# spthm/grace-devel

Measured on AMD Instinct MI355X. Metric: Mrays/s SPH column-density trace, 10^7 particles, higher is better.
Workload: dtype f32

## Files before the change

### grace-devel_amd/csrc/trace.hip

```cpp
#include "kernel_tables.hpp"
#include "trace_kernel.hpp"
#include "trace_plan.hpp"

#include <cmath>

using namespace grace_hip;

namespace grace_hip {

static_assert(GRACE_SPH_KERNEL_TABLE_ROWS == GRACE_SPH_KERNEL_WENDLAND_C6 + 1, "one table per built-in kernel");
__device__ double g_sph_kernel_tables[GRACE_SPH_KERNEL_TABLE_ROWS][N_TABLE] = GRACE_SPH_KERNEL_TABLES_INIT;
static const double k_sph_kernel_tables[GRACE_SPH_KERNEL_TABLE_ROWS][N_TABLE] = GRACE_SPH_KERNEL_TABLES_INIT;

static grace_status trace_state_destroy(Context& c)
{
    if (!c.trace) return GRACE_OK;
    TraceState& ts = *c.trace;
    GRACE_TRY(plan_release(ts));
    GRACE_TRY(scene_release(ts));
    GRACE_TRY(rays_release(ts));
    if (ts.hits.chunk_counts) GRACE_TRY_HIP(hipFree(ts.hits.chunk_counts));
    if (ts.custom_table) GRACE_TRY_HIP(hipFree(ts.custom_table));
    if (ts.status) GRACE_TRY_HIP(hipFree(ts.status));
    if (ts.ev0) GRACE_TRY_HIP(hipEventDestroy(ts.ev0));
// ... 231 lines not shown

template <int MODE, bool SPLIT, bool ALT = false>
void launch_walk(const int grid, const TraceArgs& args, hipStream_t stream)
{
    trace_kernel<MODE, SPLIT, ALT, false><<<grid, TRACE_BLOCK, 0, stream>>>(args);
    if constexpr (has_lattice(MODE))
        if (args.lat_dev) trace_kernel<MODE, SPLIT, ALT, true><<<grid, TRACE_BLOCK, 0, stream>>>(args);
}

template <int MODE>
grace_status dispatch(const TraceState& ts, const TraceArgs& a, const TraceBuffers& b, const LaunchPlan& p,
                      const int* kept, const size_t n_rays, hipStream_t stream)
{
    const int grid = ceil_div(size_t(p.n_packets) * p.split, TRACE_BLOCK / 64);
    const int* const plan_k_dev = a.plan_usable ? a.plan_split_dev : nullptr;
    auto combine = [&](const int k, const int* k_dev, const int* run_if) -> grace_status {
        const int g = ceil_div(n_rays * channels(MODE), 256);
        if constexpr (double_sums(MODE))
            combine_classes_kernel<double><<<g, 256, 0, stream>>>(a.partial_d, int(n_rays), k, k_dev, a.out_sums_d, run_if);
        else if constexpr (weighted(MODE))
            combine_channel_classes_kernel<<<g, 256, 0, stream>>>(a.partial, int(n_rays), channels(MODE), k, k_dev,
                                                                  a.out_sums, a.out_stride, run_if,
                                                                  a.plan_usable, plan_k_dev);
        else if constexpr (f4_sums(MODE))
            combine_classes_kernel<float><<<g, 256, 0, stream>>>(a.partial, int(n_rays), k, k_dev, a.out_sums, run_if,
                                                                 a.plan_usable, plan_k_dev);
        else return GRACE_OK;
        GRACE_CHECK_LAUNCH();
        return GRACE_OK;
    };
    if constexpr (class_split(MODE)) {
        auto walk = [&](auto alt_tag) -> grace_status {
            constexpr bool ALT = decltype(alt_tag)::value;
            if constexpr (has_lattice(MODE)) if (p.lat_split) {
                if (output(MODE) == OUT_COUNTS)
                    GRACE_TRY_HIP(hipMemsetAsync(a.out_counts, 0, n_rays * sizeof(int), stream));
                trace_kernel<MODE, false, ALT, false><<<grid, TRACE_BLOCK, 0, stream>>>(a);
                GRACE_CHECK_LAUNCH();
                TraceArgs a_lat = a;
                a_lat.split = p.lat_split; a_lat.split_dev = nullptr;
                trace_kernel<MODE, true, ALT, true><<<ceil_div(size_t(p.n_packets) * p.lat_split, TRACE_BLOCK / 64),
                                                      TRACE_BLOCK, 0, stream>>>(a_lat);
                GRACE_CHECK_LAUNCH();
                return combine(p.lat_split, nullptr, a.lat_dev);
            }
            if constexpr (f4_sums(MODE)) if (a.plan_usable) {
                GRACE_TRY(plan_record(ts, a, stream));
                const int grid_planned = a.plan_split_dev
                    ? ceil_div(size_t(p.n_packets) * planned_split(p.n_packets), TRACE_BLOCK / 64) : grid;
                GRACE_TRY(launch_planned(MODE, ALT, grid_planned, a, stream));
                if (p.split == 1) GRACE_TRY(combine(1, nullptr, reinterpret_cast<const int*>(a.plan_usable)));
            }
            if (p.split > 1) launch_walk<MODE, true, ALT>(grid, a, stream);
            else launch_walk<MODE, false, ALT>(grid, a, stream);
            return GRACE_OK;
        };
        if constexpr (f4_sums(MODE)) GRACE_TRY(p.fast_b ? walk(std::true_type()) : walk(std::false_type()));
        else GRACE_TRY(walk(std::false_type()));
    } else if constexpr (MODE == MODE_HITS) {
        if (p.hits_split) {
            const int* counts = kept;
            if (!kept) {
                TraceArgs c = a;
                c.chunk_counts = b.chunk_counts; c.out_counts = b.scratch_counts;
                GRACE_TRY_HIP(hipMemsetAsync(b.chunk_counts, 0, n_rays * size_t(p.hit_chunks) * 4, stream));
                GRACE_TRY_HIP(hipMemsetAsync(b.scratch_counts, 0, n_rays * 4, stream));
                launch_walk<MODE_COUNT, true>(grid, c, stream);
                GRACE_CHECK_LAUNCH();
                counts = b.chunk_counts;
            }
            hits_offsets_kernel<<<ceil_div(n_rays, 4), 256, 0, stream>>>(counts, a.offsets, int(n_rays),
                                                                         p.hit_chunks, b.chunk_off);
            GRACE_CHECK_LAUNCH();
            hits_plan_kernel<<<p.n_packets, MAX_HIT_CHUNKS, 0, stream>>>(counts, a.perm, int(n_rays),
                                                                         p.hit_chunks, b.pk_prefix, b.pk_total);
            GRACE_CHECK_LAUNCH();
            hits_assign_kernel<<<1, 1024, 0, stream>>>(b.pk_total, p.n_packets, p.n_packets * p.split, p.hit_chunks,
                                                       b.pk_first, b.pk_parts, b.n_wave_map,
                                                       ts.hits_stage_split ? 200000ull : 0ull);
            GRACE_CHECK_LAUNCH();
            hits_bounds_kernel<<<p.n_packets, 64, 0, stream>>>(b.pk_prefix, b.pk_total, b.pk_first, b.pk_parts,
                                                               p.hit_chunks, b.wave_map);
            GRACE_CHECK_LAUNCH();
            TraceArgs staged = a, direct = a;
            staged.stage_dev = direct.stage_dev = b.n_wave_map + 4;
            staged.stage_want = 1; direct.stage_want = 0;
            launch_walk<MODE, true, true>(grid, staged, stream);
            GRACE_CHECK_LAUNCH();
            launch_walk<MODE, true, false>(grid, direct, stream);
        } else if (p.n_packets >= 4096) {
            launch_walk<MODE, false, true>(grid, a, stream);
        } else {
            launch_walk<MODE, false, false>(grid, a, stream);
        }
    } else {
        launch_walk<MODE, false>(grid, a, stream);
    }
    GRACE_CHECK_LAUNCH();
    GRACE_TRY(stamps_report(MODE));
    if (p.split > 1) GRACE_TRY(combine(p.split, a.split_dev, nullptr));
    return GRACE_OK;
}

template <int MODE>
grace_status launch_trace(TraceArgs a, size_t n_rays, size_t n_spheres, size_t n_nodes,
                          hipStream_t stream, const Nested nested = Nested())
{
    GRACE_REQUIRE(a.rays && a.spheres && a.nodes && a.leaves && a.root, "trace: null pointer");
    GRACE_REQUIRE(n_rays < (size_t(1) << 31), "trace: bad ray count");
    GRACE_REQUIRE(n_nodes >= 1 && n_nodes < (size_t(1) << 30), "trace: bad node count");
    GRACE_REQUIRE(n_spheres > 0 && n_spheres < (size_t(1) << 31), "trace: bad primitive count");
    TraceState* ts_ptr = nullptr;
    GRACE_TRY(trace_state(&ts_ptr));
    TraceState& ts = *ts_ptr;
    GRACE_TRY(ensure_status(ts, stream));
    a.kernel_table = ts.kernel_table;
    const LaunchPlan p = plan_launch<MODE>(ts, a.keep_chunks, n_rays, n_spheres);
    const bool reuse_chunks = p.hits_split && ts.hits.valid && ts.hits.rays == a.rays
        && ts.hits.n_rays == n_rays && ts.hits.prims == static_cast<const void*>(a.spheres)
        && ts.hits.n_prims == n_spheres && ts.hits.n_chunks == p.hit_chunks;
    if (chunked(MODE)) ts.hits.valid = false;
    const size_t need = n_rays * size_t(p.hit_chunks);
    if (p.keep_chunks && ts.hits.capacity < need) {
        if (ts.hits.chunk_counts) { GRACE_TRY_HIP(hipDeviceSynchronize()); GRACE_TRY_HIP(hipFree(ts.hits.chunk_counts)); }
        ts.hits.chunk_counts = nullptr; ts.hits.capacity = 0;
        hipError_t e = hipMalloc(reinterpret_cast<void**>(&ts.hits.chunk_counts), need * sizeof(int));
        if (e != hipSuccess) return set_error(GRACE_OUT_OF_MEMORY, __FILE__, __LINE__, hipGetErrorString(e));
        ts.hits.capacity = need;
    }
    FrameGuard frame;
    TraceBuffers b;
    GRACE_TRY(use_records<MODE>(ts, a, b, frame, p, n_rays, n_spheres, n_nodes, stream, nested));
    if (nested.measure) return GRACE_OK;
    a.width = p.width; a.split = p.split; a.treelet = p.treelet; a.treelet_axis = p.treelet_axis;
    a.n_rays = int(n_rays); a.n_nodes = int(n_nodes); a.n_prims = int(n_spheres); a.status = ts.status;
    a.group_shift = group_shift(n_spheres); a.chunk_shift = p.hit_chunk_shift; a.n_chunks = p.hit_chunks;
    a.partial = b.partial; a.partial_d = b.partial_d;
    a.chunk_off = b.chunk_off; a.wave_map = b.wave_map; a.n_wave_map = b.n_wave_map;
    if (p.split > 1 && output(MODE) == OUT_COUNTS)
        GRACE_TRY_HIP(hipMemsetAsync(a.out_counts, 0, n_rays * sizeof(int), stream));
    if (p.keep_chunks && p.split > 1) {
        a.chunk_counts = ts.hits.chunk_counts;
        GRACE_TRY_HIP(hipMemsetAsync(ts.hits.chunk_counts, 0, n_rays * size_t(p.hit_chunks) * 4, stream));
        ts.hits.valid = true; ts.hits.rays = a.rays; ts.hits.n_rays = n_rays;
        ts.hits.prims = a.spheres; ts.hits.n_prims = n_spheres; ts.hits.n_chunks = p.hit_chunks;
    }
    ts.last_lat_dev = a.lat_dev; ts.last_lat_stream = stream;
    if constexpr (f4_sums(MODE)) {
        PacketPlan& pp = ts.plan;
        if (b.plan_eligible && !(pp.key == b.plan_key && (pp.valid || pp.dead)))
            GRACE_TRY(plan_fill(ts, b.plan_key, a, stream));
        ts.last_plan_ctl = nullptr;
        if (b.plan_eligible && pp.valid && pp.key == b.plan_key) {
            a.plan_entries = pp.entries; a.plan_spans = pp.spans; a.plan_counts = pp.counts;
            a.plan_usable = &pp.ctl->usable;
            ts.last_plan_ctl = pp.ctl; ts.last_plan_stream = stream;
        }
    }
    return timed(ts, stream, [&] {
        return dispatch<MODE>(ts, a, b, p, reuse_chunks ? ts.hits.chunk_counts : nullptr, n_rays, stream);
    });
}

TraceArgs trace_args(const void* d_rays, const void* d_prims, const int* d_nodes, const int* d_leaves,
                     const int* d_root)
{
    TraceArgs a = {};
    a.rays = static_cast<const float*>(d_rays);
    a.spheres = static_cast<const float4*>(d_prims);
    a.nodes = reinterpret_cast<const float4*>(d_nodes);
    a.leaves = reinterpret_cast<const int4*>(d_leaves);
    a.root = d_root;
    return a;
}

}

namespace grace_hip {
grace_status rays_invalidate_if_written(const void* d_written)
{
    Context* c = nullptr;
    GRACE_TRY(current_context(&c));
    if (!c->trace) return GRACE_OK;
    TraceState& ts = *c->trace;
    if (ts.cache_validation) return GRACE_OK;
    if (ts.rays.valid && d_written && d_written == static_cast<const void*>(ts.rays.key.rays)) return rays_release(ts);
    return GRACE_OK;
}

grace_status scene_invalidate_if_written(const void* d_written)
{
    Context* c = nullptr;
    GRACE_TRY(current_context(&c));
    if (!c->trace) return GRACE_OK;
    TraceState& ts = *c->trace;
    if (ts.cache_validation) return GRACE_OK;
    if (ts.scene.valid && d_written
        && (d_written == ts.scene.key.prims || d_written == ts.scene.key.nodes || d_written == ts.scene.key.leaves))
        return scene_release(ts);
    return GRACE_OK;
}

grace_status trace_nested_bytes(size_t n_rays, size_t n_spheres, size_t n_nodes, size_t* bytes)
{
    TraceArgs a = trace_args(bytes, bytes, reinterpret_cast<const int*>(bytes), reinterpret_cast<const int*>(bytes),
                             reinterpret_cast<const int*>(bytes));
    size_t counts = 0, hits = 0;
    GRACE_TRY(launch_trace<MODE_COUNT>(a, n_rays, n_spheres, n_nodes, nullptr, Nested{true, &counts}));
    GRACE_TRY(launch_trace<MODE_HITS>(a, n_rays, n_spheres, n_nodes, nullptr, Nested{true, &hits}));
    *bytes = counts > hits ? counts : hits;
    return GRACE_OK;
}

grace_status trace_hitcounts_nested(const void* d_rays, size_t n_rays, const float* d_spheres, size_t n_spheres,
                                    const int* d_nodes, size_t n_nodes, const int* d_leaves, const int* d_root,
                                    int* d_hit_counts, hipStream_t stream)
{
    TraceArgs a = trace_args(d_rays, d_spheres, d_nodes, d_leaves, d_root);
    a.out_counts = d_hit_counts;
    return launch_trace<MODE_COUNT>(a, n_rays, n_spheres, n_nodes, stream, Nested{true, nullptr});
}

grace_status trace_hits_nested(const void* d_rays, size_t n_rays, const float* d_spheres, size_t n_spheres,
                               const int* d_nodes, size_t n_nodes, const int* d_leaves, const int* d_root,
                               const int* d_ray_offsets, int* d_hit_indices, float* d_hit_integrals,
                               float* d_hit_distances, hipStream_t stream)
{
    TraceArgs a = trace_args(d_rays, d_spheres, d_nodes, d_leaves, d_root);
    a.offsets = d_ray_offsets;
    a.hit_idx = d_hit_indices;
    a.hit_integral = d_hit_integrals;
    a.hit_dist = d_hit_distances;
    return launch_trace<MODE_HITS>(a, n_rays, n_spheres, n_nodes, stream, Nested{true, nullptr});
}
}

extern "C" {

grace_status grace_trace_hitcounts_f4(const void* d_rays, size_t n_rays, const float* d_spheres,
                                      size_t n_spheres, const int* d_nodes, size_t n_nodes,
                                      const int* d_leaves, const int* d_root,
                                      int* d_hit_counts, grace_stream stream)
{
    if (n_rays == 0) return GRACE_OK;
    GRACE_REQUIRE(d_hit_counts, "trace_hitcounts: null output");
    TraceArgs a = trace_args(d_rays, d_spheres, d_nodes, d_leaves, d_root);
    a.out_counts = d_hit_counts;
    return launch_trace<MODE_COUNT>(a, n_rays, n_spheres, n_nodes, as_stream(stream));
}

grace_status grace_trace_hitcounts_keep_f4(const void* d_rays, size_t n_rays, const float* d_spheres,
                                           size_t n_spheres, const int* d_nodes, size_t n_nodes,
                                           const int* d_leaves, const int* d_root,
                                           int* d_hit_counts, grace_stream stream)
{
    if (n_rays == 0) return GRACE_OK;
    GRACE_REQUIRE(d_hit_counts, "trace_hitcounts: null output");
    TraceArgs a = trace_args(d_rays, d_spheres, d_nodes, d_leaves, d_root);
    a.out_counts = d_hit_counts;
    a.keep_chunks = true;
    return launch_trace<MODE_COUNT>(a, n_rays, n_spheres, n_nodes, as_stream(stream));
}

grace_status grace_trace_cumulative_f4(const void* d_rays, size_t n_rays, const float* d_spheres,
                                       size_t n_spheres, const int* d_nodes, size_t n_nodes,
                                       const int* d_leaves, const int* d_root,
                                       float* d_cumulated, grace_stream stream)
{
    if (n_rays == 0) return GRACE_OK;
    GRACE_REQUIRE(d_cumulated, "trace_cumulative: null output");
    TraceArgs a = trace_args(d_rays, d_spheres, d_nodes, d_leaves, d_root);
    a.out_sums = d_cumulated;
    return launch_trace<MODE_CUMULATIVE>(a, n_rays, n_spheres, n_nodes, as_stream(stream));
}

grace_status grace_trace_cumulative_weighted_f4(const void* d_rays, size_t n_rays, const float* d_spheres,
                                                size_t n_spheres, const int* d_nodes, size_t n_nodes,
                                                const int* d_leaves, const int* d_root,
                                                const float* d_weights, int n_channels, float* d_out,
                                                grace_stream stream)
{
    GRACE_REQUIRE(n_channels >= 1 && n_channels <= 64, "trace_cumulative_weighted: channels must be 1..64");
    if (n_rays == 0) return GRACE_OK;
    GRACE_REQUIRE(d_weights || n_spheres == 0, "trace_cumulative_weighted: null weights");
    GRACE_REQUIRE(d_out, "trace_cumulative_weighted: null output");
    GRACE_REQUIRE(n_rays * size_t(n_channels) < (size_t(1) << 31), "trace_cumulative_weighted: too many outputs");
    for (int g = 0; g < n_channels; g += MAX_LAUNCH_CHANNELS) {
        TraceArgs a = trace_args(d_rays, d_spheres, d_nodes, d_leaves, d_root);
        a.weights = d_weights + g;
        a.w_stride = n_channels;
        a.out_sums = d_out + g;
        a.out_stride = n_channels;
        const hipStream_t s = as_stream(stream);
        switch (n_channels - g < MAX_LAUNCH_CHANNELS ? n_channels - g : MAX_LAUNCH_CHANNELS) {
        case 1: GRACE_TRY(launch_trace<MODE_WCUM1>(a, n_rays, n_spheres, n_nodes, s)); break;
        case 2: GRACE_TRY(launch_trace<MODE_WCUM2>(a, n_rays, n_spheres, n_nodes, s)); break;
        case 3: GRACE_TRY(launch_trace<MODE_WCUM3>(a, n_rays, n_spheres, n_nodes, s)); break;
        default: GRACE_TRY(launch_trace<MODE_WCUM4>(a, n_rays, n_spheres, n_nodes, s)); break;
        }
    }
    return GRACE_OK;
}

grace_status grace_trace_hits_f4(const void* d_rays, size_t n_rays, const float* d_spheres,
                                 size_t n_spheres, const int* d_nodes, size_t n_nodes,
                                 const int* d_leaves, const int* d_root,
                                 const int* d_ray_offsets, int* d_hit_indices,
                                 float* d_hit_integrals, float* d_hit_distances,
                                 grace_stream stream)
// ... 97 lines not shown
                                     int* d_hit_indices, double* d_hit_integrals,
                                     double* d_hit_distances, grace_stream stream)
{
    if (n_rays == 0) return GRACE_OK;
    GRACE_REQUIRE(d_ray_offsets && d_hit_indices && d_hit_integrals && d_hit_distances,
                  "trace_hits (float4, double): null output");
    TraceArgs a = trace_args(d_rays, d_spheres, d_nodes, d_leaves, d_root);
    a.offsets = d_ray_offsets;
    a.hit_idx = d_hit_indices;
    a.hit_integral_d = d_hit_integrals;
    a.hit_dist_d = d_hit_distances;
    return launch_trace<MODE_HITS_F4D>(a, n_rays, n_spheres, n_nodes, as_stream(stream));
}

grace_status grace_trace_stats_f4(const void* d_rays, size_t n_rays, const float* d_spheres,
                                  size_t n_spheres, const int* d_nodes, size_t n_nodes,
                                  const int* d_leaves, const int* d_root,
                                  uint32_t* d_stats4, grace_stream stream)
{
    if (n_rays == 0) return GRACE_OK;
    GRACE_REQUIRE(d_stats4, "trace_stats: null output");
    TraceArgs a = trace_args(d_rays, d_spheres, d_nodes, d_leaves, d_root);
    a.stats = d_stats4;
    return launch_trace<MODE_STATS>(a, n_rays, n_spheres, n_nodes, as_stream(stream));
}

grace_status grace_hit_integrals_f32(const float* d_b2, const float* d_h, size_t n, float* d_out,
                                     grace_stream stream)
{
    GRACE_REQUIRE(n == 0 || (d_b2 && d_h && d_out), "hit_integrals: null pointer");
    if (n == 0) return GRACE_OK;
    TraceState* ts = nullptr;
    GRACE_TRY(trace_state(&ts));
    hit_integrals_kernel<<<stream_grid(n, 256), 256, 0, as_stream(stream)>>>(d_b2, d_h, n, d_out,
                                                                             ts->kernel_table);
    GRACE_CHECK_LAUNCH();
    return GRACE_OK;
}

grace_status grace_sph_kernel_table(int kind, double* h_out51)
{
    GRACE_REQUIRE(kind >= GRACE_SPH_KERNEL_CUBIC && kind <= GRACE_SPH_KERNEL_WENDLAND_C6,
                  "sph_kernel_table: kind must be a built-in GRACE_SPH_KERNEL_* (0..5)");
    GRACE_REQUIRE(h_out51, "sph_kernel_table: null output");
    for (int i = 0; i < N_TABLE; ++i) h_out51[i] = k_sph_kernel_tables[kind][i];
    return GRACE_OK;
}

#define GRACE_TRACE_STATE()                                                                      \
    TraceState* ts_ptr_ = nullptr;                                                               \
    GRACE_TRY(trace_state(&ts_ptr_));                                                            \
    TraceState& ts = *ts_ptr_

grace_status grace_trace_prepare_f4(const float* d_spheres, size_t n_spheres, const int* d_nodes,
                                    size_t n_nodes, const int* d_leaves, grace_stream stream)
{
    GRACE_TRACE_STATE();
    return scene_prepare(ts, PRIM_F4, d_spheres, n_spheres, d_nodes, n_nodes, d_leaves, as_stream(stream));
}

grace_status grace_trace_prepare_tri(const float* d_tris, size_t n_tris, const int* d_nodes,
                                     size_t n_nodes, const int* d_leaves, grace_stream stream)
{
    GRACE_TRACE_STATE();
    return scene_prepare(ts, PRIM_TRI, d_tris, n_tris, d_nodes, n_nodes, d_leaves, as_stream(stream));
}

grace_status grace_trace_prepare_rays(const void* d_rays, size_t n_rays, grace_stream stream)
{
    GRACE_TRACE_STATE();
    return rays_prepare(ts, static_cast<const float*>(d_rays), n_rays, as_stream(stream));
}

grace_status grace_trace_release_rays(void)
{
    GRACE_TRACE_STATE();
    GRACE_TRY(plan_release(ts));
    return rays_release(ts);
}

grace_status grace_trace_release(void)
{
    GRACE_TRACE_STATE();
    if (ts.hits.chunk_counts) {
        GRACE_TRY_HIP(hipDeviceSynchronize());
        GRACE_TRY_HIP(hipFree(ts.hits.chunk_counts));
    }
    ts.hits = HitsCache();
    GRACE_TRY(plan_release(ts));
    return scene_release(ts);
}

grace_status grace_trace_enable_timing(int enabled)
{
    GRACE_TRACE_STATE();
    ts.timing = enabled != 0;
    ts.ev_valid = false;
    return GRACE_OK;
}

grace_status grace_trace_last_kernel_ms(float* h_ms)
{
    GRACE_REQUIRE(h_ms, "null output");
    GRACE_TRACE_STATE();
    GRACE_REQUIRE(ts.timing && ts.ev_valid, "no timed traversal launch recorded");
    GRACE_TRY_HIP(hipEventSynchronize(ts.ev1));
    GRACE_TRY_HIP(hipEventElapsedTime(h_ms, ts.ev0, ts.ev1));
    return GRACE_OK;
}

grace_status grace_trace_last_lattice(int* h_lattice)
{
    GRACE_REQUIRE(h_lattice, "null output");
    *h_lattice = 0;
    GRACE_TRACE_STATE();
    if (ts.last_lat_dev) {
        GRACE_TRY_HIP(hipStreamSynchronize(ts.last_lat_stream));
        GRACE_TRY_HIP(hipMemcpy(h_lattice, ts.last_lat_dev, sizeof(int), hipMemcpyDeviceToHost));
    }
    return GRACE_OK;
}

grace_status grace_trace_last_plan_used(int* h_used)
{
    GRACE_REQUIRE(h_used, "null output");
    *h_used = 0;
    GRACE_TRACE_STATE();
    if (ts.last_plan_ctl) {
        PlanCtl h = {};
        GRACE_TRY_HIP(hipStreamSynchronize(ts.last_plan_stream));
        GRACE_TRY_HIP(hipMemcpy(&h, ts.last_plan_ctl, sizeof(h), hipMemcpyDeviceToHost));
        *h_used = h.usable != 0u ? 1 : 0;
    }
    return GRACE_OK;
}

grace_status grace_trace_plan_stats(unsigned long long* h_stats)
{
    GRACE_REQUIRE(h_stats, "null output");
    for (int k = 0; k < 7; ++k) h_stats[k] = 0;
    GRACE_TRACE_STATE();
    if (ts.last_plan_ctl) {
        PlanCtl h = {};
        GRACE_TRY_HIP(hipStreamSynchronize(ts.last_plan_stream));
        GRACE_TRY_HIP(hipMemcpy(&h, ts.last_plan_ctl, sizeof(h), hipMemcpyDeviceToHost));
        if (h.usable != 0u) {
            for (int k = 0; k < 6; ++k) h_stats[k] = h.stats[k];
            h_stats[6] = h.largest_round;
        }
    }
    return GRACE_OK;
}

grace_status grace_trace_set_plan(int on)
{
    GRACE_TRACE_STATE();
    ts.plan_on = on != 0;
    if (!ts.plan_on) GRACE_TRY(plan_release(ts));
    return GRACE_OK;
}

grace_status grace_trace_set_plan_budget(size_t bytes)
{
    GRACE_TRACE_STATE();
    ts.plan_budget = bytes;
    GRACE_TRY(plan_release(ts));
    return GRACE_OK;
}

grace_status grace_trace_plan_bytes(size_t* h_bytes)
{
    GRACE_REQUIRE(h_bytes, "null output");
    GRACE_TRACE_STATE();
    const PacketPlan& pp = ts.plan;
    *h_bytes = pp.valid ? (pp.n_entries + 4) * sizeof(uint4) + pp.n_lists * (sizeof(int) + sizeof(int2)) + sizeof(PlanCtl) : 0;
    return GRACE_OK;
}

grace_status grace_trace_set_packet_split(int waves_per_packet)
{
    GRACE_REQUIRE(waves_per_packet == -1 || waves_per_packet == 1 || waves_per_packet == 2
                      || waves_per_packet == 4 || waves_per_packet == 8,
                  "packet split must be 1, 2, 4, 8 or -1 (automatic)");
    GRACE_TRACE_STATE();
    ts.split = waves_per_packet;
    return GRACE_OK;
}

grace_status grace_trace_set_packet_width(int rays_per_packet)
{
    GRACE_REQUIRE(rays_per_packet == -1 || rays_per_packet == 16 || rays_per_packet == 32
                      || rays_per_packet == 64,
                  "packet width must be 16, 32, 64 or -1 (automatic)");
    GRACE_TRACE_STATE();
    ts.width = rays_per_packet;
    return GRACE_OK;
}

grace_status grace_trace_set_exact_integrals(int enabled)
{
    GRACE_TRACE_STATE();
    ts.exact_integrals = enabled != 0;
    return GRACE_OK;
}

grace_status grace_trace_set_sph_kernel(int kind)
{
    GRACE_REQUIRE(kind >= GRACE_SPH_KERNEL_CUBIC && kind <= GRACE_SPH_KERNEL_WENDLAND_C6,
                  "set_sph_kernel: kind must be a built-in GRACE_SPH_KERNEL_* (0..5); a custom table is "
                  "set with grace_trace_set_sph_kernel_table");
    GRACE_TRACE_STATE();
    ts.sph_kernel = kind;
    ts.kernel_table = ts.builtin_tables + kind * N_TABLE;
    return GRACE_OK;
}

grace_status grace_trace_set_sph_kernel_table(const double* h_table, int n)
{
    GRACE_REQUIRE(h_table && n == N_TABLE, "set_sph_kernel_table: the table must hold 51 values");
    for (int i = 0; i < N_TABLE; ++i)
        GRACE_REQUIRE(std::isfinite(h_table[i]) && h_table[i] >= 0.0,
                      "set_sph_kernel_table: every value must be finite and >= 0");
    GRACE_REQUIRE(h_table[N_TABLE - 1] == 0.0, "set_sph_kernel_table: the last value (b = H) must be 0");
    GRACE_TRACE_STATE();
    GRACE_TRY_HIP(hipDeviceSynchronize());
    if (!ts.custom_table)
        GRACE_TRY_HIP(hipMalloc(reinterpret_cast<void**>(&ts.custom_table), N_TABLE * sizeof(double)));
    GRACE_TRY_HIP(hipMemcpy(ts.custom_table, h_table, N_TABLE * sizeof(double), hipMemcpyHostToDevice));
    for (int i = 0; i < N_TABLE; ++i) ts.custom_host[i] = h_table[i];
    ts.sph_kernel = GRACE_SPH_KERNEL_CUSTOM;
    ts.kernel_table = ts.custom_table;
    return GRACE_OK;
}

grace_status grace_trace_get_sph_kernel(int* h_kind, double* h_table51)
{
    GRACE_TRACE_STATE();
    if (h_kind) *h_kind = ts.sph_kernel;
    if (h_table51) {
        const double* t = ts.sph_kernel == GRACE_SPH_KERNEL_CUSTOM ? ts.custom_host
                                                                   : k_sph_kernel_tables[ts.sph_kernel];
        for (int i = 0; i < N_TABLE; ++i) h_table51[i] = t[i];
    }
    return GRACE_OK;
}

grace_status grace_trace_set_treelet_size(int max_primitives)
{
    GRACE_REQUIRE(max_primitives >= -1, "treelet size must be >= 0 (or -1 for automatic)");
    GRACE_TRACE_STATE();
    ts.treelet = max_primitives;
    return GRACE_OK;
}

grace_status grace_trace_set_ray_reorder(int enabled)
{
    GRACE_TRACE_STATE();
    ts.ray_reorder = enabled != 0;
    return GRACE_OK;
}

grace_status grace_trace_set_cache_validation(int enabled)
{
    GRACE_TRACE_STATE();
    ts.cache_validation = enabled != 0;
    return GRACE_OK;
}

grace_status grace_trace_set_cache_auto(int enabled)
{
    GRACE_TRACE_STATE();
    ts.cache_auto = enabled != 0;
    if (!ts.cache_auto) {
        if ((ts.scene.valid && !ts.scene.pinned) || (ts.rays.valid && !ts.rays.pinned)) GRACE_TRY(plan_release(ts));
        if (ts.scene.valid && !ts.scene.pinned) GRACE_TRY(scene_release(ts));
        if (ts.rays.valid && !ts.rays.pinned) GRACE_TRY(rays_release(ts));
        ts.scene.seen = SceneKey();
        ts.rays.seen = RayKey();
    }
    return GRACE_OK;
}

grace_status grace_trace_set_lattice_split(int waves_per_packet)
{
    GRACE_REQUIRE(waves_per_packet == 0 || waves_per_packet == 2 || waves_per_packet == 4
                      || waves_per_packet == 8,
                  "lattice split must be 0 (one wave per packet), 2, 4 or 8");
    GRACE_TRACE_STATE();
    ts.lat_split = waves_per_packet;
    return GRACE_OK;
}

grace_status grace_trace_set_hits_staging(int enabled)
{
    GRACE_TRACE_STATE();
    ts.hits_stage_split = enabled != 0;
    return GRACE_OK;
}

grace_status grace_trace_status(grace_stream stream)
{
    GRACE_TRACE_STATE();
    if (!ts.status) return GRACE_OK;
    int h = 0;
    GRACE_TRY_HIP(hipMemcpyAsync(&h, ts.status, sizeof(int), hipMemcpyDeviceToHost,
                                 as_stream(stream)));
    GRACE_TRY_HIP(hipStreamSynchronize(as_stream(stream)));
    if (h != 0) {
        GRACE_TRY_HIP(hipMemsetAsync(ts.status, 0, sizeof(int), as_stream(stream)));
        if (h == GRACE_INVALID_ARGUMENT)
            return set_error(GRACE_INVALID_ARGUMENT, __FILE__, __LINE__,
                             "range_neighbours: a row of d_offsets does not have the length of its list");
        return set_error(GRACE_STACK_OVERFLOW, __FILE__, __LINE__,
                         "trace: packet stack (128 entries) exhausted");
    }
    return GRACE_OK;
}

}
```

### grace-devel_amd/csrc/trace_coherence.hip

```cpp
#include "trace_state.hpp"

using namespace grace_hip;

namespace {

__device__ __forceinline__ uint32_t f2ord_u(float f)
{
    const uint32_t u = __float_as_uint(f);
    return (u & 0x80000000u) ? ~u : (u | 0x80000000u);
}

__device__ __forceinline__ float ord2f_u(uint32_t u)
{
    return __uint_as_float((u & 0x80000000u) ? (u & 0x7fffffffu) : ~u);
}

__global__ void ray_ext_init_kernel(uint32_t* __restrict__ ext16)
{
    if (threadIdx.x < 16) ext16[threadIdx.x] = threadIdx.x < 6 ? 0xFFFFFFFFu : 0u;
}

__global__ __launch_bounds__(1024) void ray_extents_kernel(const float* __restrict__ rays, int n,
                                                          uint32_t* __restrict__ ext12,
                                                          const uint32_t* __restrict__ run_if)
// ... 14 lines not shown
        len_hi = fmaxf(len_hi, r[6]);
    }
#pragma unroll
    for (int off = 32; off > 0; off >>= 1) len_hi = fmaxf(len_hi, __shfl_xor(len_hi, off));
#pragma unroll
    for (int k = 0; k < 6; ++k) {
#pragma unroll
        for (int off = 32; off > 0; off >>= 1) {
            lo[k] = fminf(lo[k], __shfl_xor(lo[k], off));
            hi[k] = fmaxf(hi[k], __shfl_xor(hi[k], off));
        }
    }
    __shared__ float s_lo[16][6], s_hi[16][6], s_len[16];
    const int wave = threadIdx.x >> 6;
    if ((threadIdx.x & 63) == 0) {
#pragma unroll
        for (int k = 0; k < 6; ++k) { s_lo[wave][k] = lo[k]; s_hi[wave][k] = hi[k]; }
        s_len[wave] = len_hi;
    }
    __syncthreads();
    const int n_waves = int(blockDim.x >> 6);
    if (threadIdx.x < 6) {
        const int k = threadIdx.x;
        float l = s_lo[0][k], h = s_hi[0][k];
        for (int w = 1; w < n_waves; ++w) { l = fminf(l, s_lo[w][k]); h = fmaxf(h, s_hi[w][k]); }
        atomicMin(&ext12[k], f2ord_u(l));
        atomicMax(&ext12[6 + k], f2ord_u(h));
    } else if (threadIdx.x == 6) {
        float l = s_len[0];
        for (int w = 1; w < n_waves; ++w) l = fmaxf(l, s_len[w]);
        if (l > -INFINITY) atomicMax(&ext12[15], f2ord_u(l));
    }
}

__device__ int choose_split(const uint32_t* __restrict__ ext12, int n_packets, int launched_arg, bool lattice)
{
    const bool one_direction = ext12[0] == ext12[6] && ext12[1] == ext12[7] && ext12[2] == ext12[8];
    const int launched = launched_arg & 0xFF;
    const int budget = (launched_arg & SPLIT_WIDE_BUDGET) ? 32768 : 16384;
    int k = launched;
    if (one_direction && !lattice) {
        k = 1;
        while (k < launched && n_packets * k < 8192) k *= 2;
        if (k < launched && n_packets >= 6144 && n_packets * k * 2 <= budget) k *= 2;
    } else if (!lattice) {
        k = 1;
        while (k < launched && n_packets * k < 16384) k *= 2;
    }
    return k;
}

__device__ __forceinline__ uint32_t hilbert2d_15(uint32_t x, uint32_t y)
{
    uint32_t d = 0;
    for (uint32_t s = 1u << 14; s > 0; s >>= 1) {
        const uint32_t rx = (x & s) ? 1u : 0u, ry = (y & s) ? 1u : 0u;
        d = (d << 2) | ((3u * rx) ^ ry);
        if (ry == 0) {
            if (rx) { x = 32767u - x; y = 32767u - y; }
            const uint32_t t = x; x = y; y = t;
        }
    }
    return d;
}

__global__ __launch_bounds__(256) void ray_lattice_kernel(const float* __restrict__ rays, int n,
                                                          const uint32_t* __restrict__ ext12,
                                                          uint32_t* __restrict__ flag,
                                                          const uint32_t* __restrict__ run_if)
{
    if (run_if && *run_if == 0u) return;
    int dims[2] = { 0, 0 }, nvar = 0;
    float lo[2] = { 0.f, 0.f }, span[2] = { 0.f, 0.f };
    for (int k = 5; k >= 0; --k) {
        const float l = ord2f_u(ext12[k]), sp = ord2f_u(ext12[6 + k]) - l;
        if (sp > 0.f && sp < INFINITY) {
            if (nvar < 2) { dims[nvar] = k; lo[nvar] = l; span[nvar] = sp; }
            ++nvar;
        }
    }
    bool fit = nvar == 2 && n >= 64 && (n & (n - 1)) == 0;
    float m1 = 0.f, m2 = 0.f;
    if (fit) {
        int log_n = 0;
        while ((1 << log_n) < n) ++log_n;
        fit = false;
        const float ratio = span[0] / span[1];
        for (int a = 3; a <= log_n - 3; ++a) {
            const float c1 = float((1 << a) - 1), c2 = float((1 << (log_n - a)) - 1);
            if (fabsf(c1 / c2 - ratio) <= 1e-3f * ratio) { fit = true; m1 = c1; m2 = c2; break; }
        }
    }
    if (!fit) {
        if (blockIdx.x == 0 && threadIdx.x == 0) atomicOr(flag, 1u);
        return;
    }
    const float s1 = m1 / span[0], s2 = m2 / span[1];
    bool off = false;
    for (int i = blockIdx.x * blockDim.x + threadIdx.x; i < n; i += gridDim.x * blockDim.x) {
        const float* r = rays + 7 * size_t(i);
        const float u1 = (r[dims[0]] - lo[0]) * s1, u2 = (r[dims[1]] - lo[1]) * s2;
        off = off || !(fabsf(u1 - rintf(u1)) <= 0.01f) || !(fabsf(u2 - rintf(u2)) <= 0.01f);
    }
    if (__builtin_amdgcn_ballot_w64(off) != 0ull && (threadIdx.x & 63) == 0) atomicOr(flag, 1u);
}

__device__ void choose_variants(const uint32_t* __restrict__ ext12, int n, const float4* __restrict__ scene_min,
                                uint32_t* __restrict__ lat_flag, int split_packets, int split_launched,
                                int* __restrict__ split_dev)
{
    if (lat_flag) {
        int n_dir = 0;
        bool one_dir = true;
        float e1 = 0.f, e2 = 0.f;
        for (int k = 0; k < 3; ++k) {
            const float dl = ord2f_u(ext12[k]), dh = ord2f_u(ext12[6 + k]);
            one_dir = one_dir && dl == dh;
            n_dir += dl != 0.f ? 1 : 0;
            const float e = ord2f_u(ext12[9 + k]) - ord2f_u(ext12[3 + k]);
            if (e > e1) { e2 = e1; e1 = e; } else if (e > e2) e2 = e;
        }
        const float spacing2 = e1 * e2 / float(n);
        const float r2_min = scene_min->x;
        bool lat = one_dir && n_dir == 1 && spacing2 > 0.f && r2_min < 2.0f * spacing2;
        if (!lat && e1 == 0.f && ext12[15] != 0u) {
            const float len = ord2f_u(ext12[15]);
            if (len > 0.f && len < INFINITY) lat = r2_min < 2.0f * (12.566371f * len * len / float(n));
        }
        *lat_flag = lat ? 1u : 0u;
    }
    if (split_dev)
        *split_dev = choose_split(ext12, split_packets, split_launched, lat_flag ? *lat_flag != 0u : false);
}

__global__ void choose_variants_kernel(const uint32_t* __restrict__ ext12, int n, const float4* __restrict__ scene_min,
                                       uint32_t* __restrict__ lat_flag, int split_packets, int split_launched,
                                       int* __restrict__ split_dev, const PlanGate gate,
                                       int* __restrict__ plan_split_dev)
{
    if (lat_flag || split_dev)
        choose_variants(ext12, n, scene_min, lat_flag, split_packets, split_launched, split_dev);
    if (plan_split_dev) *plan_split_dev = planned_split(split_packets);
    if (gate.ctl) {
        PlanCtl& pc = *gate.ctl;
        const bool stale = pc.sig[0] != gate.scene->sig[0] || pc.sig[1] != gate.scene->sig[1]
            || pc.sig[2] != gate.rays->sig[0] || pc.sig[3] != gate.rays->sig[1];
        pc.record = stale ? 1u : 0u;
        if (stale) {
            pc.unusable = 0u; pc.usable = 1u;
            pc.sig[0] = gate.scene->sig[0]; pc.sig[1] = gate.scene->sig[1];
            pc.sig[2] = gate.rays->sig[0]; pc.sig[3] = gate.rays->sig[1];
            for (int k = 0; k < 6; ++k) pc.stats[k] = 0ull;
            pc.largest_round = 0u;
        }
    }
}

__global__ __launch_bounds__(256) void ray_keys_kernel(const float* __restrict__ rays, int n,
                                                       const uint32_t* __restrict__ ext12,
                                                       uint32_t* __restrict__ keys,
                                                       const float4* __restrict__ scene_min,
                                                       uint32_t* __restrict__ lat_flag,
                                                       int split_packets, int split_launched,
                                                       int* __restrict__ split_dev,
                                                       const uint32_t* __restrict__ not_grid,
                                                       const uint32_t* __restrict__ run_if)
{
    if (run_if && *run_if == 0u) return;
    const bool z_order_2d = not_grid && *not_grid == 0u;
    if (blockIdx.x == 0 && threadIdx.x == 0)
        choose_variants(ext12, n, scene_min, lat_flag, split_packets, split_launched, split_dev);
    float lo[6], scale[6], span[6];
    int nvar = 0;
    float span_d = 0.f, span_o = 0.f;
#pragma unroll
    for (int k = 0; k < 6; ++k) {
        lo[k] = ord2f_u(ext12[k]);
        span[k] = ord2f_u(ext12[6 + k]) - lo[k];
        const bool varies = span[k] > 0.f && span[k] < INFINITY;
        if (varies) { if (k < 3) span_d = fmaxf(span_d, span[k]); else span_o = fmaxf(span_o, span[k]); }
    }
#pragma unroll
    for (int k = 0; k < 6; ++k) {
        const bool varies = span[k] > 0.f && span[k] < INFINITY;
        scale[k] = varies ? 1.0f / (k < 3 ? span_d : span_o) : 0.f;
        nvar += varies ? 1 : 0;
    }
    const int bits = nvar ? min(15, 30 / nvar) : 0;
    const float qmax = float((1 << bits) - 1);
    const bool pencil = scale[3] == 0.f && scale[4] == 0.f && scale[5] == 0.f && nvar > 0;
    for (int i = blockIdx.x * blockDim.x + threadIdx.x; i < n; i += gridDim.x * blockDim.x) {
        const float* r = rays + 7 * size_t(i);
        if (pencil) {
            const float l1 = fabsf(r[0]) + fabsf(r[1]) + fabsf(r[2]);
            float u = r[0] / l1, v = r[1] / l1;
            if (r[2] < 0.f) {
                const float fu = (1.f - fabsf(v)) * (u >= 0.f ? 1.f : -1.f);
                const float fv = (1.f - fabsf(u)) * (v >= 0.f ? 1.f : -1.f);
                u = fu; v = fv;
            }
            const uint32_t qu = uint32_t(fminf(32767.f, fmaxf(0.f, (u * 0.5f + 0.5f) * 32767.f + 0.5f)));
            const uint32_t qv = uint32_t(fminf(32767.f, fmaxf(0.f, (v * 0.5f + 0.5f) * 32767.f + 0.5f)));
            keys[i] = hilbert2d_15(qu, qv);
            continue;
        }
        uint32_t q[6];
#pragma unroll
        for (int k = 0; k < 6; ++k) q[k] = uint32_t(fminf(qmax, (r[k] - lo[k]) * scale[k] * qmax + 0.5f));
#ifndef GRACE_MORTON2D
        if (nvar == 2 && !z_order_2d) {
            uint32_t xy[2] = {0, 0};
            int m = 0;
#pragma unroll
            for (int k = 5; k >= 0; --k)
                if (scale[k] > 0.f) { if (m < 2) xy[m] = q[k]; ++m; }
            keys[i] = hilbert2d_15(xy[1], xy[0]);
            continue;
        }
#endif
        uint32_t key = 0;
        for (int b = bits - 1; b >= 0; --b) {
#pragma unroll
            for (int k = 5; k >= 0; --k)
                if (scale[k] > 0.f) key = (key << 1) | ((q[k] >> b) & 1u);
        }
        keys[i] = key << (30 - bits * nvar);
    }
}

}

namespace grace_hip {

grace_status launch_choose_variants(const uint32_t* ext12, int n, const float4* scene_min, uint32_t* lat_flag,
                                    int split_packets, int split_launched, int* split_dev, hipStream_t stream,
                                    const PlanGate* gate, int* plan_split_dev)
{
    choose_variants_kernel<<<1, 1, 0, stream>>>(ext12, n, scene_min, lat_flag, split_packets, split_launched,
                                                split_dev, gate ? *gate : PlanGate(), plan_split_dev);
    GRACE_CHECK_LAUNCH();
    return GRACE_OK;
}

static grace_status rays_free_buffers(RayOrder& ro)
{
    if (ro.perm || ro.ext || ro.ctl) GRACE_TRY_HIP(hipDeviceSynchronize());
    if (ro.perm) GRACE_TRY_HIP(hipFree(ro.perm));
    if (ro.ext) GRACE_TRY_HIP(hipFree(ro.ext));
    if (ro.ctl) GRACE_TRY_HIP(hipFree(ro.ctl));
    ro.perm = nullptr; ro.ext = nullptr; ro.ctl = nullptr;
    ro.valid = false;
    ro.pinned = false;
    return GRACE_OK;
}

grace_status rays_release(TraceState& ts)
{
    GRACE_TRY(rays_free_buffers(ts.rays));
    ts.rays = RayOrder();
    return GRACE_OK;
}

grace_status rays_cache_alloc(TraceState& ts, const RayKey& key)
{
    RayOrder& ro = ts.rays;
    GRACE_TRY(rays_free_buffers(ro));
    if (hipMalloc(reinterpret_cast<void**>(&ro.perm), key.n * 4) != hipSuccess
        || hipMalloc(reinterpret_cast<void**>(&ro.ext), 64) != hipSuccess
        || hipMalloc(reinterpret_cast<void**>(&ro.ctl), sizeof(CacheCtl)) != hipSuccess) {
        (void)hipGetLastError();
        (void)rays_free_buffers(ro);
        return set_error(GRACE_OUT_OF_MEMORY, __FILE__, __LINE__, "ray order cache: out of device memory");
    }
    ro.key = key;
    ro.gen = ++ts.cache_gen;
    return GRACE_OK;
}

grace_status ray_order(const float* d_rays, size_t n_rays, uint32_t* ext, uint32_t* keys, uint32_t* perm,
                       const float4* scene_min, uint32_t* lat_flag, int n_packets, int split, int* split_dev,
                       hipStream_t stream, const uint32_t* run_if)
{
    if (!run_if) {
        ray_ext_init_kernel<<<1, 64, 0, stream>>>(ext);
        GRACE_CHECK_LAUNCH();
    }
    const int grid_small = stream_grid(n_rays, 256, 4) < 1024 ? stream_grid(n_rays, 256, 4) : 1024;
    const int grid_ext = stream_grid(n_rays, 1024, 4) < 128 ? stream_grid(n_rays, 1024, 4) : 128;
    ray_extents_kernel<<<grid_ext, 1024, 0, stream>>>(d_rays, int(n_rays), ext, run_if);
    GRACE_CHECK_LAUNCH();
    ray_lattice_kernel<<<grid_small, 256, 0, stream>>>(d_rays, int(n_rays), ext, ext + 14, run_if);
    GRACE_CHECK_LAUNCH();
    ray_keys_kernel<<<stream_grid(n_rays, 256), 256, 0, stream>>>(d_rays, int(n_rays), ext, keys, scene_min,
                                                                 lat_flag, n_packets, split, split_dev, ext + 14,
                                                                 run_if);
    GRACE_CHECK_LAUNCH();
    const size_t packets64 = ceil_div(n_rays, size_t(64));
    int want_bits = 2;
    while ((size_t(1) << (want_bits - 2)) < packets64 && want_bits < 30) ++want_bits;
    want_bits = ((want_bits + 7) / 8) * 8;
    const int begin_bit = want_bits >= 30 ? 0 : 30 - want_bits;
    return sort_pairs_u32_nested(keys, nullptr, n_rays, 0, begin_bit, 30, perm, stream, run_if);
}

grace_status rays_prepare(TraceState& ts, const float* d_rays, size_t n_rays, hipStream_t stream)
{
// ... 31 lines not shown
```

### grace-devel_amd/csrc/trace_kernel.hpp

```cpp
#pragma once

#include "trace_diag.hpp"
#include "trace_packet.hpp"
#include "trace_state.hpp"

#include <type_traits>

namespace {

using namespace grace_hip;

__device__ __forceinline__ bool any_lane(bool p) { return __builtin_amdgcn_ballot_w64(p) != 0ull; }

__device__ __forceinline__ int imin(int a, int b) { return a < b ? a : b; }
__device__ __forceinline__ int imax(int a, int b) { return a > b ? a : b; }

__device__ __forceinline__ void aabbs_hit(const float ix, const float iy, const float iz,
                                          const float ox, const float oy, const float oz,
                                          const float len, const float4 L, const float4 R,
                                          const float4 Z, bool& hit_l, bool& hit_r)
{
    const float bx_L = (L.x - ox) * ix, tx_L = (L.y - ox) * ix;
    const float by_L = (L.z - oy) * iy, ty_L = (L.w - oy) * iy;
    const float bz_L = (Z.x - oz) * iz, tz_L = (Z.y - oz) * iz;
// ... 45 lines not shown
    integral *= ir2;
    return integral;
}

__device__ __forceinline__ float hit_integral_fast(const float b2, const float ir50,
                                                   const float2* lutf)
{
    const float b = __builtin_amdgcn_sqrtf(b2) * ir50;
    const float2 y = lutf[static_cast<int>(b)];
    return __builtin_fmaf(y.y, b, y.x);
}

__device__ __forceinline__ bool tri_intersect(const double ddx, const double ddy, const double ddz,
                                              const float ox, const float oy, const float oz,
                                              const double* __restrict__ tri, float* t_out)
{
    const double vx = tri[0], vy = tri[1], vz = tri[2];
    const double e1x = tri[3], e1y = tri[4], e1z = tri[5];
    const double e2x = tri[6], e2y = tri[7], e2z = tri[8];
    const float Px = float(ddy * e2z - ddz * e2y);
    const float Py = float(ddz * e2x - ddx * e2z);
    const float Pz = float(ddx * e2y - ddy * e2x);
    const float det = float((e1x * double(Px) + e1y * double(Py)) + e1z * double(Pz));
    bool reject = det < 1E-14f;
    const float inv_det = 1.0f / det;
    const float OVx = ox - float(vx), OVy = oy - float(vy), OVz = oz - float(vz);
    const double dOVx = OVx, dOVy = OVy, dOVz = OVz;
    const float u = float(((dOVx * double(Px) + dOVy * double(Py)) + dOVz * double(Pz)) * double(inv_det));
    reject = reject || (u < 0.f || u > 1.f);
    const float Qx = float(dOVy * e1z - dOVz * e1y);
    const float Qy = float(dOVz * e1x - dOVx * e1z);
    const float Qz = float(dOVx * e1y - dOVy * e1x);
    const float v = float(((ddx * double(Qx) + ddy * double(Qy)) + ddz * double(Qz)) * double(inv_det));
    reject = reject || (v < 0.f || u + v > 1.f);
    *t_out = float(((e2x * double(Qx) + e2y * double(Qy)) + e2z * double(Qz)) * double(inv_det));
    return !reject;
}

__global__ __launch_bounds__(256) void hit_integrals_kernel(const float* __restrict__ b2,
                                                            const float* __restrict__ h, size_t n,
                                                            float* __restrict__ out,
                                                            const double* __restrict__ table)
{
    __shared__ double2 s_lut[N_TABLE];
    if (threadIdx.x < N_TABLE) {
        const double y0 = table[threadIdx.x];
        const double y1 = threadIdx.x + 1 < N_TABLE ? table[threadIdx.x + 1] : y0;
        s_lut[threadIdx.x] = make_double2(y0, y1 - y0);
    }
    __syncthreads();
    for (size_t i = blockIdx.x * size_t(blockDim.x) + threadIdx.x; i < n;
         i += size_t(gridDim.x) * blockDim.x) {
        const float ir = 1.f / h[i];
        out[i] = hit_integral(b2[i], ir, ir * ir, s_lut);
    }
}

__device__ __forceinline__ bool beam_may_hit(const float4 s, const Beam& bm,
                                             const float margin = 3.814697265625e-06f )
{
    float p2_lo = 0.f, p2_hi = 0.f, t_lo = 0.f, t_hi = 0.f;
    const float c[3] = { s.x, s.y, s.z };
#pragma unroll
    for (int k = 0; k < 3; ++k) {
        const float plo = c[k] - bm.ohi[k], phi = c[k] - bm.olo[k];
        const float a2 = plo * plo, b2 = phi * phi;
        p2_hi += fmaxf(a2, b2);
        p2_lo += (plo <= 0.f && phi >= 0.f) ? 0.f : fminf(a2, b2);
        const float q0 = plo * bm.dlo[k], q1 = plo * bm.dhi[k];
        const float q2 = phi * bm.dlo[k], q3 = phi * bm.dhi[k];
        t_lo += fminf(fminf(q0, q1), fminf(q2, q3));
        t_hi += fmaxf(fmaxf(q0, q1), fmaxf(q2, q3));
    }
    const float t2_hi = fmaxf(t_lo * t_lo, t_hi * t_hi);
    const float b2_lo = p2_lo - t2_hi - margin * p2_hi;
    return !(b2_lo >= s.w);
}

struct Pencil {
    float ox, oy, oz;
    float ax, ay, az;
    float sin_t, cos_t;
    float nx[4], ny[4], nz[4];
};

__device__ __forceinline__ bool pencil_may_hit(const float4 s, const Pencil& pc)
{
    const float vx = s.x - pc.ox, vy = s.y - pc.oy, vz = s.z - pc.oz;
    const float d2 = __builtin_fmaf(vx, vx, __builtin_fmaf(vy, vy, vz * vz));
    const float va = __builtin_fmaf(vx, pc.ax, __builtin_fmaf(vy, pc.ay, vz * pc.az));
    const float inv = __builtin_amdgcn_rsqf(d2);
    const float sin_a = fminf(1.0f, __builtin_amdgcn_sqrtf(s.w) * inv * 1.00001f);
    const float cos_a = __builtin_amdgcn_sqrtf(fmaxf(0.0f, __builtin_fmaf(-sin_a, sin_a, 1.0f)));
    const float cos_limit = __builtin_fmaf(pc.cos_t, cos_a, -pc.sin_t * sin_a) - 1e-5f;
    const float h = __builtin_amdgcn_sqrtf(s.w) * 1.00001f + 1e-6f * __builtin_amdgcn_sqrtf(d2);
    float out = -1.0f;
#pragma unroll
    for (int k = 0; k < 4; ++k)
        out = fmaxf(out, __builtin_fmaf(vx, pc.nx[k], __builtin_fmaf(vy, pc.ny[k], vz * pc.nz[k])) - h);
    return !(d2 > s.w * 1.00001f) || (!(va * inv < cos_limit) && !(out > 0.0f));
}

template <int AX, bool FUSED = false>
__device__ __forceinline__ bool axis_beam_may_hit(const float4 s, const Beam& bm)
{
    constexpr int D1 = AX == 0 ? 1 : 0, D2 = AX == 2 ? 1 : 2;
    const float s1 = AX == 0 ? s.y : s.x;
    const float s2 = AX == 2 ? s.y : s.z;
    const float q1 = s1 - __builtin_amdgcn_fmed3f(s1, bm.olo[D1], bm.ohi[D1]);
    const float q2 = s2 - __builtin_amdgcn_fmed3f(s2, bm.olo[D2], bm.ohi[D2]);
    const float b2_lo = FUSED ? __builtin_fmaf(q1, q1, q2 * q2) : q1 * q1 + q2 * q2;
    return !(b2_lo >= s.w);
}

__device__ __forceinline__ float4 cluster_sphere(const float4 blo, const float4 bhi)
{
    const float cx = 0.5f * (blo.x + bhi.x), cy = 0.5f * (blo.y + bhi.y), cz = 0.5f * (blo.z + bhi.z);
    const float ex = bhi.x - cx, ey = bhi.y - cy, ez = bhi.z - cz;
    const float fx = cx - blo.x, fy = cy - blo.y, fz = cz - blo.z;
    const float rx = fmaxf(ex, fx), ry = fmaxf(ey, fy), rz = fmaxf(ez, fz);
    return make_float4(cx, cy, cz, (rx * rx + ry * ry + rz * rz) * 1.001f);
}

template <int AX>
__device__ __forceinline__ bool cluster_may_hit(const float4 blo, const float4 bhi, const Beam& bm,
                                                const Pencil* pc)
{
    if constexpr (AX >= 0) {
        constexpr int D1 = AX == 0 ? 1 : 0, D2 = AX == 2 ? 1 : 2;
        const float lo1 = AX == 0 ? blo.y : blo.x, hi1 = AX == 0 ? bhi.y : bhi.x;
        const float lo2 = AX == 2 ? blo.y : blo.z, hi2 = AX == 2 ? bhi.y : bhi.z;
        return !(lo1 > bm.ohi[D1]) && !(hi1 < bm.olo[D1]) && !(lo2 > bm.ohi[D2]) && !(hi2 < bm.olo[D2]);
    } else if constexpr (AX == -2) {
        const float lx = blo.x - pc->ox, ly = blo.y - pc->oy, lz = blo.z - pc->oz;
        const float hx = bhi.x - pc->ox, hy = bhi.y - pc->oy, hz = bhi.z - pc->oz;
        const float scale = fmaxf(fmaxf(fmaxf(fabsf(lx), fabsf(hx)), fmaxf(fabsf(ly), fabsf(hy))),
                                  fmaxf(fabsf(lz), fabsf(hz)));
        const float slack = 1e-5f * scale;
        float worst = -1.0f;
#pragma unroll
        for (int k = 0; k < 4; ++k) {
            const float m = fminf(pc->nx[k] * lx, pc->nx[k] * hx) + fminf(pc->ny[k] * ly, pc->ny[k] * hy)
                + fminf(pc->nz[k] * lz, pc->nz[k] * hz);
            worst = fmaxf(worst, m);
        }
        const float front = fmaxf(pc->ax * lx, pc->ax * hx) + fmaxf(pc->ay * ly, pc->ay * hy)
            + fmaxf(pc->az * lz, pc->az * hz);
        return !(worst > slack) && !(front < -slack) && pencil_may_hit(cluster_sphere(blo, bhi), *pc);
    } else {
        return beam_may_hit(cluster_sphere(blo, bhi), bm, 1.52587890625e-05f );
    }
}

typedef uint32_t plan_u32x4 __attribute__((ext_vector_type(4)));
typedef int plan_i32x2 __attribute__((ext_vector_type(2)));
template <typename T>
__device__ __forceinline__ const __attribute__((address_space(4))) T* plan_const(const void* p)
{
    return (const __attribute__((address_space(4))) T*)(uintptr_t)p;
}

template <int N>
struct WeightedB {
    float x, y;
    float w[N + 1];
    __device__ WeightedB(const float2 b) : x(b.x), y(b.y), w{} {}
};

template <int MODE, bool SPLIT, bool ALT = false, bool LAT = false, bool PLANNED = false>
__global__ __launch_bounds__(TRACE_BLOCK, !f4_class_split(MODE) ? 1
                                          : weighted(MODE) ? (channels(MODE) == 1 ? 6 : 7 - channels(MODE))
                                          : (SPLIT ? 8 : 6))
void trace_kernel(const TraceArgs a)
{
    static_assert(!ALT || f4_integrals(MODE), "no alternative path for this mode");
    static_assert(!LAT || has_lattice(MODE), "no lattice cull for this mode");
    static_assert(!PLANNED || (SPLIT && !LAT && f4_sums(MODE)), "planned: class-split column densities only");
    if constexpr (PLANNED) {
        if (*plan_const<uint32_t>(a.plan_usable) == 0u) return;
    } else if (has_lattice(MODE)) {
        if (a.plan_usable && *a.plan_usable != 0u) return;
        if (a.lat_dev ? (*a.lat_dev != 0) != LAT : LAT) return;
        if (a.stage_dev && *a.stage_dev != a.stage_want) return;
    }
    constexpr bool FAST = ALT && f4_sums(MODE);
    constexpr bool WEIGHTED = weighted(MODE);
    constexpr int NW = channels(MODE), WP = WEIGHTED ? (NW + 1) / 2 : 0;
    using BRec = std::conditional_t<WEIGHTED, WeightedB<NW>, float2>;
    __shared__ double2 s_lut[FAST ? 1 : N_TABLE];
    constexpr int LUTF_N = 256;
    __shared__ float2 s_lutf[FAST ? LUTF_N : 1];
    constexpr bool D4 = primitive(MODE) == PRIM_D4, F4D = primitive(MODE) == PRIM_F4D;
    constexpr bool LDS_TILE = primitive(MODE) == PRIM_F4;
    __shared__ __align__(16) float2 s_tile[LDS_TILE ? TRACE_BLOCK / 64 : 1][LDS_TILE ? 3 + WP : 1][LDS_TILE ? 66 : 1];
    __shared__ double s_tile_d[D4 ? TRACE_BLOCK / 64 : 1][D4 ? 64 : 1][D4 ? 6 : 1];
    __shared__ float4 s_tile_f[F4D ? TRACE_BLOCK / 64 : 1][F4D ? 64 : 1][F4D ? 2 : 1];
    const int lane = threadIdx.x & 63;
    static_assert(!SPLIT || class_split(MODE) || MODE == MODE_HITS, "triangle and stats walks do not split");
    constexpr bool RANGE_SPLIT = SPLIT && MODE == MODE_HITS;
    const int split_ordinary = !SPLIT ? 1 : (!RANGE_SPLIT && a.split_dev) ? *a.split_dev : a.split;
    int split_planned = 0;
    if constexpr (PLANNED)
        if (a.plan_split_dev) split_planned = *plan_const<int>(a.plan_split_dev);
    const int split = PLANNED && split_planned > 0 ? split_planned : split_ordinary;
    const int n_packets = (a.n_rays + a.width - 1) / a.width;
    const int nb = (n_packets * split + TRACE_BLOCK / 64 - 1) / (TRACE_BLOCK / 64);
    const int q = nb >> 3, r8 = nb & 7, xcd = blockIdx.x & 7, slot = blockIdx.x >> 3;
    if (slot >= q + (xcd < r8 ? 1 : 0)) return;
    const int vblock = (xcd < r8 ? xcd * (q + 1) : r8 * (q + 1) + (xcd - r8) * q) + slot;
    const int wave_id = __builtin_amdgcn_readfirstlane(vblock * (TRACE_BLOCK / 64)
                                                       + (threadIdx.x >> 6));
    if (integrates(MODE)) {
        if (FAST) {
            static_assert(TRACE_BLOCK >= 256, "one table entry per thread");
            float2 e = make_float2(0.f, 0.f);
            if (threadIdx.x < N_TABLE - 1) {
                const double y0 = a.kernel_table[threadIdx.x], dy = a.kernel_table[threadIdx.x + 1] - y0;
                e = make_float2(float(y0 - double(threadIdx.x) * dy), float(dy));
            }
            if (threadIdx.x < LUTF_N) s_lutf[threadIdx.x] = e;
        } else if (threadIdx.x < N_TABLE) {
            const int i0 = threadIdx.x;
            const double y0 = a.kernel_table[i0];
            const double y1 = i0 + 1 < N_TABLE ? a.kernel_table[i0 + 1] : y0;
            s_lut[threadIdx.x] = make_double2(y0, y1 - y0);
        }
        __syncthreads();
    }
    int packet = wave_id / split, part = wave_id - packet * split;
    int prim_lo = 0, prim_hi = 0x7fffffff;
    if (RANGE_SPLIT) {
        if (wave_id >= *a.n_wave_map) return;
        const int4 wm = a.wave_map[wave_id];
        packet = wm.x; part = 0;
        prim_lo = wm.y << a.chunk_shift;
        prim_hi = wm.z << a.chunk_shift;
        if (prim_lo >= prim_hi) return;
    }
    const int first_ray = packet * a.width;
    if (first_ray >= a.n_rays) return;
    const int classes_per_part = SUM_CLASSES / split;
    const int own_lo = part * classes_per_part, own_hi = own_lo + classes_per_part;
    auto owns_granule = [&](const int g) {
        if (RANGE_SPLIT) { const int p = g << GRANULE_SHIFT; return p >= prim_lo && p < prim_hi; }
        const int c = g & (SUM_CLASSES - 1);
        return c >= own_lo && c < own_hi;
    };
    auto foreign_range = [&](const int first, const int count) {
        if (RANGE_SPLIT) return first + count <= prim_lo || first >= prim_hi;
        const int g0 = first >> GRANULE_SHIFT, g1 = (first + count - 1) >> GRANULE_SHIFT;
        return g1 - g0 <= 1 && !owns_granule(g0) && !owns_granule(g1);
    };
    const PacketRay ray = load_packet_ray(a, first_ray, lane);
    const bool valid = ray.valid;
    const int ray_index = ray.index;
    const float dx = ray.dx, dy = ray.dy, dz = ray.dz;
    const float ox = ray.ox, oy = ray.oy, oz = ray.oz;
    const float len = ray.len;
    const float ix = 1.f / dx, iy = 1.f / dy, iz = 1.f / dz;
    const Beam beam = packet_beam(ray);
    int axis = -1;
    if (!ordered(MODE)) axis = packet_axis(dx, dy, dz);
    __shared__ Pencil s_pencil[TRACE_BLOCK / 64];
    Pencil pencil;
    bool is_pencil = false;
    if (!PLANNED && axis < 0 && MODE != MODE_STATS && beam.olo[0] == beam.ohi[0] && beam.olo[1] == beam.ohi[1]
        && beam.olo[2] == beam.ohi[2]) {
        float sx = dx, sy = dy, sz = dz;
#pragma unroll
        for (int off = 32; off > 0; off >>= 1) {
            sx += __shfl_xor(sx, off); sy += __shfl_xor(sy, off); sz += __shfl_xor(sz, off);
        }
        const float inv = 1.0f / sqrtf(sx * sx + sy * sy + sz * sz);
        const float ax = sx * inv, ay = sy * inv, az = sz * inv;
        const float cx = ay * dz - az * dy, cy = az * dx - ax * dz, cz = ax * dy - ay * dx;
        const float sin_t = wave_max(sqrtf(cx * cx + cy * cy + cz * cz)) + 2e-6f;
        const float cos_min = wave_min(ax * dx + ay * dy + az * dz);
        if (cos_min > 0.5f && sin_t < 0.8660254f) {
            is_pencil = true;
            pencil.ox = beam.olo[0]; pencil.oy = beam.olo[1]; pencil.oz = beam.olo[2];
            pencil.ax = ax; pencil.ay = ay; pencil.az = az;
            pencil.sin_t = sin_t;
            pencil.cos_t = sqrtf(1.0f - sin_t * sin_t);
            float ux, uy, uz;
            if (fabsf(ax) <= fabsf(ay) && fabsf(ax) <= fabsf(az)) { ux = 0.f; uy = -az; uz = ay; }
            else if (fabsf(ay) <= fabsf(az)) { ux = az; uy = 0.f; uz = -ax; }
            else { ux = -ay; uy = ax; uz = 0.f; }
            const float un = 1.0f / sqrtf(ux * ux + uy * uy + uz * uz);
            ux *= un; uy *= un; uz *= un;
            const float vx = ay * uz - az * uy, vy = az * ux - ax * uz, vz = ax * uy - ay * ux;
            const float da_ = ax * dx + ay * dy + az * dz;
            const float tu = (ux * dx + uy * dy + uz * dz) / da_, tv = (vx * dx + vy * dy + vz * dz) / da_;
            const float m = 4e-6f;
            const float tu_lo = wave_min(tu) - m, tu_hi = wave_max(tu) + m;
            const float tv_lo = wave_min(tv) - m, tv_hi = wave_max(tv) + m;
            auto plane = [&](int k, float cu, float cv, float ca) {
                float px = cu * ux + cv * vx + ca * ax, py = cu * uy + cv * vy + ca * ay,
                      pz = cu * uz + cv * vz + ca * az;
                const float pn = 1.0f / sqrtf(px * px + py * py + pz * pz);
                pencil.nx[k] = px * pn; pencil.ny[k] = py * pn; pencil.nz[k] = pz * pn;
            };
            plane(0, 1.f, 0.f, -tu_hi);
            plane(1, -1.f, 0.f, tu_lo);
            plane(2, 0.f, 1.f, -tv_hi);
            plane(3, 0.f, -1.f, tv_lo);
            if (lane == 0) s_pencil[threadIdx.x >> 6] = pencil;
        }
    }
    const AxisRay ar = axis_ray(axis, ray);
    const float oa = ar.oa, da = ar.da, noda = ar.noda, o1 = ar.o1, o2 = ar.o2;
    float noda_lo = 0.f, noda_hi = 0.f, len_lo = 0.f, da0 = 0.f;
    bool same_sense = false;
    if (axis >= 0) axis_extremes(ar, len, noda_lo, noda_hi, len_lo, da0, same_sense);
    const float fat_r2 = FAST && axis >= 0 ? fat_radius2(axis, beam) : INFINITY;
    const int treelet = axis >= 0 ? a.treelet_axis : a.treelet;
    constexpr bool LATTICE = LAT;
    __shared__ float s_lat[LATTICE ? TRACE_BLOCK / 64 : 1][2][8];
    __shared__ float s_lat_r2[LATTICE ? TRACE_BLOCK / 64 : 1];
    if (LATTICE && lane == 0) s_lat_r2[threadIdx.x >> 6] = 0.f;
    if (LATTICE && axis >= 0) {
        bool ok;
        float cell2;
        build_origin_lattice(o1, o2, lane, s_lat, ok, cell2);
        if (lane == 0) s_lat_r2[threadIdx.x >> 6] = ok ? cell2 : 0.f;
    }

    int count = 0;
    constexpr bool CHUNKED = SPLIT && chunked(MODE);
    int cur_chunk = -1;
    int count_at_chunk = 0;
    float sum = 0.f;
    float wsum[NW] = {};
    constexpr bool CLASSES_F = f4_sums(MODE), CLASSES_D = double_sums(MODE);
    constexpr bool CLASSES = output(MODE) == OUT_SUMS || WEIGHTED;
    __shared__ float s_class[CLASSES_F ? TRACE_BLOCK / 64 : 1][CLASSES_F ? SUM_CLASSES * NW : 1][CLASSES_F ? 64 : 1];
    __shared__ double s_class_d[CLASSES_D ? TRACE_BLOCK / 64 : 1][CLASSES_D ? SUM_CLASSES : 1][CLASSES_D ? 64 : 1];
    const int wv_acc = threadIdx.x >> 6;
    if (CLASSES_F) {
#pragma unroll
        for (int c = 0; c < SUM_CLASSES * NW; ++c) s_class[wv_acc][c][lane] = 0.f;
    }
    if (CLASSES_D) {
#pragma unroll
        for (int c = 0; c < SUM_CLASSES; ++c) s_class_d[wv_acc][c][lane] = 0.0;
    }
    double sum_d = 0.0;
    int cur_granule = -1;
// ... 12 lines not shown
        cur_granule = prim >> GRANULE_SHIFT;
        cur_granule_end = (cur_granule + 1) << GRANULE_SHIFT;
        cur_owned = !SPLIT || owns_granule(cur_granule);
        if constexpr (WEIGHTED) {
#pragma unroll
            for (int c = 0; c < NW; ++c) wsum[c] = s_class[wv_acc][(cur_granule & (SUM_CLASSES - 1)) * NW + c][lane];
        } else {
        if (CLASSES_D) sum_d = s_class_d[wv_acc][cur_granule & (SUM_CLASSES - 1)][lane];
        else sum = s_class[wv_acc][cur_granule & (SUM_CLASSES - 1)][lane];
        }
    };
    int write_at = 0;
    auto leave_chunk = [&]() {
        if (MODE == MODE_COUNT && cur_chunk >= 0 && valid && count != count_at_chunk)
            atomicAdd(&a.chunk_counts[size_t(ray_index) * a.n_chunks + cur_chunk],
                      count - count_at_chunk);
        count_at_chunk = count;
    };
    int tri_data = -1;
    float tri_tmin = len * (1.f + 0.000001f);
    const double ddx = dx, ddy = dy, ddz = dz;
    if (output(MODE) == OUT_HITS) write_at = a.offsets[ray_index];
    const double rdx = dx, rdy = dy, rdz = dz;
    constexpr int HIT_CAP = 8;
    constexpr bool STAGE_HITS = ALT && MODE == MODE_HITS;
    __shared__ float s_hits[STAGE_HITS ? TRACE_BLOCK / 64 : 1][STAGE_HITS ? 3 : 1]
                           [STAGE_HITS ? HIT_CAP : 1][STAGE_HITS ? 65 : 1];
    int staged = 0;
    auto drain_hits = [&]() {
        const int wvh = threadIdx.x >> 6;
        constexpr int RAYS_PER_PASS = 64 / HIT_CAP;
        const int g = lane / HIT_CAP, e = lane % HIT_CAP;
#pragma unroll 1
        for (int pass = 0; pass < HIT_CAP; ++pass) {
            const int src = pass * RAYS_PER_PASS + g;
            const int n_src = __shfl(staged, src);
            const int first = __shfl(write_at - staged, src);
            if (e < n_src) {
                a.hit_idx[first + e] = __float_as_int(s_hits[wvh][0][e][src]);
                a.hit_integral[first + e] = s_hits[wvh][STAGE_HITS ? 1 : 0][e][src];
                a.hit_dist[first + e] = s_hits[wvh][STAGE_HITS ? 2 : 0][e][src];
            }
        }
        staged = 0;
    };
    auto enter_chunk = [&](const int chunk) {
        leave_chunk();
        cur_chunk = chunk;
        if (MODE == MODE_HITS) {
            if (STAGE_HITS && __builtin_amdgcn_ballot_w64(staged != 0) != 0ull) drain_hits();
            write_at = a.chunk_off[size_t(ray_index) * a.n_chunks + chunk];
        }
    };
    uint32_t st_nodes = 0, st_leaves = 0, st_tested = 0;

    int stk0 = 0, stk1 = 0;
    int ml0 = 0, mh0 = 0, ml1 = 0, mh1 = 0;
    int sp = -1;
    int junk = 0;
    bool overflow = false;

    auto push = [&](const int value, const unsigned long long alive) {
        if (sp >= 127) { overflow = true; return; }
        ++sp;
        if (sp < 64) {
            const bool me = lane == sp;
            stk0 = me ? value : stk0;
            if (MODE == MODE_STATS) {
                ml0 = me ? int(uint32_t(alive)) : ml0;
                mh0 = me ? int(uint32_t(alive >> 32)) : mh0;
            }
        } else {
            const bool me = lane == sp - 64;
            stk1 = me ? value : stk1;
            if (MODE == MODE_STATS) {
                ml1 = me ? int(uint32_t(alive)) : ml1;
                mh1 = me ? int(uint32_t(alive >> 32)) : mh1;
            }
        }
    };

    constexpr bool FLAT_OK = class_split(MODE);
    bool flat = FLAT_OK && !PLANNED && (axis >= 0 || is_pencil);
    int groups_kept = 0;
    const float4* const group_boxes = a.C + 2 * ((size_t(a.n_prims) + 63) >> 6) + 1;
    const int covered = FLAT_OK ? min(__float_as_int(group_boxes[-1].y), a.n_prims) : 0;
    if (covered < 0) flat = false;
    const int n_groups = FLAT_OK ? int((size_t(max(covered, 0)) + (size_t(1) << a.group_shift) - 1) >> a.group_shift) : 0;
    unsigned long long group_mask = 0ull;
    int group_next = 0;
    __shared__ unsigned long long s_group_mask[FLAT_OK && !PLANNED ? TRACE_BLOCK / 64 : 1][FLAT_OK && !PLANNED ? 64 : 1];
    if (flat && axis < 0) {
        const int wvg = threadIdx.x >> 6;
        for (int g0 = 0; g0 < n_groups; g0 += 128) {
            float4 lo[2], hi[2];
#pragma unroll
            for (int k = 0; k < 2; ++k) {
                const int gj = min(g0 + 64 * k + lane, n_groups - 1);
                lo[k] = group_boxes[2 * size_t(gj)];
                hi[k] = group_boxes[2 * size_t(gj) + 1];
            }
#pragma unroll
            for (int k = 0; k < 2; ++k) {
                const int gk = g0 + 64 * k;
                if (gk < n_groups) {
                    const bool may = cluster_may_hit<-2>(lo[k], hi[k], beam, &s_pencil[wvg]);
                    const int n_g = n_groups - gk;
                    const unsigned long long m = __builtin_amdgcn_ballot_w64(may)
                        & (n_g >= 64 ? ~0ull : ((1ull << n_g) - 1ull));
                    if (lane == 0) s_group_mask[wvg][gk >> 6] = m;
                    groups_kept += __builtin_popcountll(m);
                }
            }
        }
    } else if (flat) {
        const int d1 = axis == 0 ? 1 : 0, d2 = axis == 2 ? 1 : 2;
        const float flat_lo1 = d1 == 0 ? beam.olo[0] : beam.olo[1], flat_hi1 = d1 == 0 ? beam.ohi[0] : beam.ohi[1];
        const float flat_lo2 = d2 == 1 ? beam.olo[1] : beam.olo[2], flat_hi2 = d2 == 1 ? beam.ohi[1] : beam.ohi[2];
        const float oa = axis == 0 ? ox : axis == 1 ? oy : oz;
        const float da = axis == 0 ? dx : axis == 1 ? dy : dz;
        const float ea = oa + da * len;
        const float flat_alo = wave_min(fminf(oa, ea));
        const float flat_ahi = wave_max(fmaxf(oa, ea));
        const int wvg = threadIdx.x >> 6;
        auto group_test = [&](const float4 glo, const float4 ghi, const int g0) {
            const float l1 = axis == 0 ? glo.y : glo.x, h1 = axis == 0 ? ghi.y : ghi.x;
            const float l2 = axis == 2 ? glo.y : glo.z, h2 = axis == 2 ? ghi.y : ghi.z;
            const float la = axis == 0 ? glo.x : axis == 1 ? glo.y : glo.z;
            const float ha = axis == 0 ? ghi.x : axis == 1 ? ghi.y : ghi.z;
            const bool may = !(l1 > flat_hi1) && !(h1 < flat_lo1) && !(l2 > flat_hi2) && !(h2 < flat_lo2)
                && !(la > flat_ahi) && !(ha < flat_alo);
            const int n_g = n_groups - g0;
            const unsigned long long m = __builtin_amdgcn_ballot_w64(may)
                & (n_g >= 64 ? ~0ull : n_g <= 0 ? 0ull : ((1ull << n_g) - 1ull));
            if (lane == 0) s_group_mask[wvg][g0 >> 6] = m;
            groups_kept += __builtin_popcountll(m);
        };
        for (int g0 = 0; g0 < n_groups; g0 += 256) {
            float4 lo[4], hi[4];
#pragma unroll
            for (int k = 0; k < 4; ++k) {
                const int gj = min(g0 + 64 * k + lane, n_groups - 1);
                lo[k] = group_boxes[2 * size_t(gj)];
                hi[k] = group_boxes[2 * size_t(gj) + 1];
            }
#pragma unroll
            for (int k = 0; k < 4; ++k)
                if (g0 + 64 * k < n_groups) group_test(lo[k], hi[k], g0 + 64 * k);
        }
    }
    constexpr int FLAT_MAX_GROUPS = 256;
    if (flat && groups_kept > FLAT_MAX_GROUPS) flat = false;
    if (!flat && !PLANNED) push(*a.root, ~0ull);
    const __attribute__((address_space(4))) plan_u32x4* plan_at = nullptr;
    int plan_n = 0, plan_cls = own_lo;
    (void)plan_at; (void)plan_n; (void)plan_cls;
    unsigned long long st_walk = 0, st_cluster = 0, st_cull = 0, st_surv = 0, st_rounds = 0, st_nsurv = 0;
    const unsigned long long st_begin = STAMP_NOW();
    (void)st_walk; (void)st_cluster; (void)st_cull; (void)st_surv; (void)st_rounds; (void)st_nsurv; (void)st_begin;

    for (;;) {
        const unsigned long long st_t0 = STAMP_NOW(); (void)st_t0;
        int sweep_first = 0, sweep_count = 0;
        bool sweep = false;
        if constexpr (PLANNED) {
            if (plan_cls >= own_hi) break;
            const int list = packet * SUM_CLASSES + plan_cls++;
            plan_n = plan_const<int>(a.plan_counts)[list];
            if (plan_n <= 0) continue;
            plan_at = plan_const<plan_u32x4>(a.plan_entries) + plan_const<plan_i32x2>(a.plan_spans)[list].x;
            enter_granule((plan_cls - 1) << GRANULE_SHIFT);
            sweep = true; sweep_count = a.n_prims;
        } else if (flat) {
            while (group_mask == 0ull && group_next < n_groups) {
                group_mask = s_group_mask[threadIdx.x >> 6][group_next >> 6];
                group_mask = (unsigned long long)uint32_t(__builtin_amdgcn_readfirstlane(int(uint32_t(group_mask))))
                    | ((unsigned long long)uint32_t(__builtin_amdgcn_readfirstlane(int(uint32_t(group_mask >> 32)))) << 32);
                group_next += 64;
            }
            if (group_mask == 0ull) break;
            const int g = group_next - 64 + __builtin_ctzll(group_mask);
            group_mask &= group_mask - 1ull;
            sweep_first = g << a.group_shift;
            sweep_count = min(1 << a.group_shift, covered - sweep_first);
            if (SPLIT) {
                bool mine = false;
                for (int gr = sweep_first >> GRANULE_SHIFT; gr <= (sweep_first + sweep_count - 1) >> GRANULE_SHIFT
                         && gr < (sweep_first >> GRANULE_SHIFT) + SUM_CLASSES; ++gr)
                    mine = mine || owns_granule(gr);
                if (!mine) continue;
            }
            sweep = true;
        } else {
        if (sp < 0) break;
        int idx;
        unsigned long long alive_mask = ~0ull;
        if (sp < 64) {
            idx = __builtin_amdgcn_readlane(stk0, sp);
            if (MODE == MODE_STATS)
                alive_mask = (unsigned long long)uint32_t(__builtin_amdgcn_readlane(ml0, sp))
                    | ((unsigned long long)uint32_t(__builtin_amdgcn_readlane(mh0, sp)) << 32);
        } else {
            idx = __builtin_amdgcn_readlane(stk1, sp - 64);
            if (MODE == MODE_STATS)
                alive_mask = (unsigned long long)uint32_t(__builtin_amdgcn_readlane(ml1, sp - 64))
                    | ((unsigned long long)uint32_t(__builtin_amdgcn_readlane(mh1, sp - 64)) << 32);
        }
        --sp;
        const bool alive = (alive_mask >> lane) & 1ull;

        if (idx < a.n_nodes) {
            const float4* np = a.nodes + 4 * size_t(idx);
            const float4 n0 = np[0];
            const float4 L = np[1];
            const float4 R = np[2];
            const float4 Z = np[3];
            int2 span = make_int2(0, 0x7fffffff);
#ifdef GRACE_PACKET_STATS
            if (treelet > 0) span = a.node_prims[idx];
#else
            if (MODE != MODE_STATS && (treelet > 0 || SPLIT)) span = a.node_prims[idx];
#endif
            if (SPLIT && foreign_range(span.x, span.y)) continue;
            if (span.y <= treelet) {
                sweep = true; sweep_first = span.x; sweep_count = span.y;
            } else {
            bool hit_l, hit_r;
            if constexpr (fp64(MODE) || MODE == MODE_TRI) {
                auto widen = [](const float4 b) {
                    const float s0 = (fabsf(b.x) + fabsf(b.y)) * 4.76837158203125e-07f;
                    const float s1 = (fabsf(b.z) + fabsf(b.w)) * 4.76837158203125e-07f;
                    return make_float4(b.x - s0, b.y + s0, b.z - s1, b.w + s1);
                };
                aabbs_hit(ix, iy, iz, ox, oy, oz, len, widen(L), widen(R), widen(Z), hit_l, hit_r);
            } else {
                aabbs_hit(ix, iy, iz, ox, oy, oz, len, L, R, Z, hit_l, hit_r);
            }
            const unsigned long long vote_r = __builtin_amdgcn_ballot_w64(hit_r);
            const unsigned long long vote_l = __builtin_amdgcn_ballot_w64(hit_l);
#ifdef GRACE_PACKET_STATS
#else
            if (MODE == MODE_STATS && alive) ++st_nodes;
#endif
            if (vote_r) push(__float_as_int(n0.y),
                             MODE == MODE_STATS ? __builtin_amdgcn_ballot_w64(hit_r && alive) : 0ull);
            if (vote_l) push(__float_as_int(n0.x),
                             MODE == MODE_STATS ? __builtin_amdgcn_ballot_w64(hit_l && alive) : 0ull);
            }
        } else {
            const int4 lf = a.leaves[idx - a.n_nodes];
            if (SPLIT && foreign_range(lf.x, lf.y)) continue;
            sweep = true; sweep_first = lf.x; sweep_count = lf.y;
#ifndef GRACE_PACKET_STATS
            if (MODE == MODE_STATS && alive) { ++st_leaves; st_tested += uint32_t(lf.y); }
#endif
        }
        }
        STAMP_ADD(st_walk, st_t0);
        if (sweep) {
            const int2 leaf = make_int2(sweep_first, sweep_count);
            int warm = 0;
            if (sp >= 0) {
                const int nxt = sp < 64 ? __builtin_amdgcn_readlane(stk0, sp)
                                        : __builtin_amdgcn_readlane(stk1, sp - 64);
                warm = nxt < a.n_nodes
                    ? reinterpret_cast<const int*>(a.nodes)[16 * size_t(nxt)]
                    : reinterpret_cast<const int*>(a.leaves)[4 * size_t(nxt - a.n_nodes)];
            }
            auto sweep_range = [&](auto ax_tag) {
                constexpr int AX = decltype(ax_tag)::value;
            constexpr bool NEED_B = f4_integrals(MODE);
            constexpr bool LEAN4 = FAST && AX >= 0;
            const int wv = threadIdx.x >> 6;
            float4* const tile4 = reinterpret_cast<float4*>(&s_tile[wv][0][0]);
            const int r_lo = leaf.x, r_hi = leaf.x + leaf.y;
            const int c_first = r_lo >> 6, c_last = (r_hi - 1) >> 6;
            double4 mined_next = make_double4(0., 0., 0., 0.);
            float mw_next[NW] = {};
            auto load_cluster = [&](const int c, float4& m4, float2& m2) {
                const int pj = PLANNED ? int(min(uint32_t(c << 6) + uint32_t(lane), uint32_t(r_hi - 1)))
                                       : min(max((c << 6) + lane, r_lo), r_hi - 1);
                m4 = a.A[pj];
                if (LDS_TILE && NEED_B) m2 = a.B[pj];
                if (D4) mined_next = reinterpret_cast<const double4*>(a.spheres_d)[pj];
                if (F4D) {
                    const float4 f = a.spheres[pj];
                    mined_next = make_double4(f.x, f.y, f.z, f.w);
                }
                if constexpr (WEIGHTED) {
#pragma unroll
                    for (int c = 0; c < NW; ++c) mw_next[c] = a.weights[size_t(pj) * a.w_stride + c];
                }
            };
            for (int cg = c_first; cg <= (PLANNED ? c_first : c_last); cg += 64) {
                const unsigned long long st_t1 = STAMP_NOW(); (void)st_t1;
                unsigned long long cmask = 1ull;
                unsigned long long small_mask = ~0ull;
                if (!PLANNED && c_last != c_first) {
                    const int cj = min(cg + lane, c_last);
                    const float4 blo = a.C[2 * size_t(cj)], bhi = a.C[2 * size_t(cj) + 1];
                    const bool c_may = cluster_may_hit<AX>(blo, bhi, beam, &s_pencil[wv]);
                    if (LATTICE && AX >= 0) small_mask = __builtin_amdgcn_ballot_w64(blo.w < s_lat_r2[wv]);
                    const int n_c = min(64, c_last - cg + 1);
                    cmask = __builtin_amdgcn_ballot_w64(c_may)
                        & (n_c >= 64 ? ~0ull : ((1ull << n_c) - 1ull));
                    if (SPLIT) cmask &= __builtin_amdgcn_ballot_w64(owns_granule(cj >> (GRANULE_SHIFT - 6)));
#ifdef GRACE_PACKET_STATS
                    if (MODE == MODE_STATS) st_leaves += 1;
#endif
                }
                STAMP_ADD(st_cluster, st_t1);
                if (cmask == 0ull) continue;
                int cnext = cg + __builtin_ctzll(cmask);
                cmask &= cmask - 1ull;
                plan_u32x4 e0 = { 0u, 0u, 0u, 0u }, e1 = e0, e2 = e0, e3 = e0;
                int plan_i = 0;
                (void)plan_i;
                if constexpr (PLANNED) { e0 = plan_at[0]; e1 = plan_at[1]; e2 = plan_at[2]; e3 = plan_at[3]; }
                float4 mine_next;
                float2 mineb_next = make_float2(0.f, 0.f);
                int round_n_next = 0;
                uint32_t round_bits_next = 0u;
                (void)round_n_next; (void)round_bits_next;
                auto gather_round = [&]() {
                    if constexpr (PLANNED) {
                        float* const idx = &s_tile[wv][0][0].x;
                        int p = 0;
                        round_bits_next = e0.w;
                        auto take = [&](const plan_u32x4 ent) {
                            const uint32_t m_lo = uint32_t(__builtin_amdgcn_readfirstlane(int(ent.y)));
                            const uint32_t m_hi = uint32_t(__builtin_amdgcn_readfirstlane(int(ent.z)));
                            const unsigned long long m = (unsigned long long)m_lo | ((unsigned long long)m_hi << 32);
                            const int n_e = __builtin_popcountll(m);
                            if (p + n_e > 64) return false;
                            if (__builtin_amdgcn_inverse_ballot_w64(m))
                                idx[p + int(__builtin_amdgcn_mbcnt_hi(m_hi, __builtin_amdgcn_mbcnt_lo(m_lo, 0u)))] =
                                    __uint_as_float((uint32_t(__builtin_amdgcn_readfirstlane(int(ent.x))) << 6) + uint32_t(lane));
                            p += n_e;
                            ++plan_i;
                            return (uint32_t(__builtin_amdgcn_readfirstlane(int(ent.w))) & 4u) == 0u && plan_i < plan_n;
                        };
                        while (take(e0) && take(e1) && take(e2) && take(e3)) {
                            e0 = plan_at[plan_i]; e1 = plan_at[plan_i + 1]; e2 = plan_at[plan_i + 2]; e3 = plan_at[plan_i + 3];
                        }
                        e0 = plan_at[plan_i]; e1 = plan_at[plan_i + 1]; e2 = plan_at[plan_i + 2]; e3 = plan_at[plan_i + 3];
                        round_n_next = p;
                        const int pj = int(min(__float_as_uint(idx[lane]), uint32_t(r_hi - 1)));
                        mine_next = a.A[pj];
                        if (NEED_B) mineb_next = a.B[pj];
                        if constexpr (WEIGHTED) {
#pragma unroll
                            for (int c = 0; c < NW; ++c) mw_next[c] = a.weights[size_t(pj) * a.w_stride + c];
                        }
                    }
                };
                if constexpr (PLANNED) gather_round();
                else load_cluster(cnext, mine_next, mineb_next);
                for (;;) {
                    const unsigned long long st_t2 = STAMP_NOW(); (void)st_t2;
                    const int pbase = cnext << 6;
                    const float4 mine = mine_next;
                    const float2 mineb = mineb_next;
                    const double4 mined = mined_next;
                    float mw[NW];
                    if constexpr (WEIGHTED) {
#pragma unroll
                        for (int c = 0; c < NW; ++c) mw[c] = mw_next[c];
                    }
                    bool more = cmask != 0ull;
                    const int round_n = round_n_next;
                    const uint32_t round_bits = round_bits_next;
                    (void)round_n; (void)round_bits;
                    if constexpr (PLANNED) {
                        more = plan_i < plan_n;
                        if (more) gather_round();
                    } else if (more) {
                        cnext = cg + __builtin_ctzll(cmask);
                        cmask &= cmask - 1ull;
                        load_cluster(cnext, mine_next, mineb_next);
                    }
                    const int lo_bit = max(r_lo - pbase, 0), hi_bit = min(r_hi - pbase, 64);
                    const unsigned long long m_mask =
                        (hi_bit >= 64 ? ~0ull : ((1ull << hi_bit) - 1ull)) & (~0ull << lo_bit);
                bool may_hit = false;
                if constexpr (PLANNED) { }
                else if constexpr (AX >= 0) may_hit = axis_beam_may_hit<AX, FAST>(mine, beam);
                else if constexpr (AX == -2) may_hit = pencil_may_hit(mine, s_pencil[wv]);
                else may_hit = beam_may_hit(mine, beam);
                unsigned long long rest = PLANNED
                    ? (round_n >= 64 ? ~0ull : ((1ull << round_n) - 1ull))
                    : (__builtin_amdgcn_ballot_w64(may_hit) & m_mask);
                bool keep = __builtin_amdgcn_inverse_ballot_w64(rest);
                bool lean_round = PLANNED && (__builtin_amdgcn_readfirstlane(int(round_bits)) & 1) != 0;
                if constexpr (!PLANNED && AX >= 0 && f4_class_split(MODE)) {
                    const float sa = AX == 0 ? mine.x : AX == 1 ? mine.y : mine.z;
                    const unsigned long long inside =
                        __builtin_amdgcn_ballot_w64(__builtin_fmaf(sa, da0, noda_lo) >= 0.0f)
                        & __builtin_amdgcn_ballot_w64(__builtin_fmaf(sa, da0, noda_hi) < len_lo);
                    lean_round = same_sense & ((rest & ~inside) == 0ull);
                }
                bool fat_round = PLANNED && (__builtin_amdgcn_readfirstlane(int(round_bits)) & 2) != 0;
                if constexpr (LEAN4 && !PLANNED)
                    fat_round = (rest & ~__builtin_amdgcn_ballot_w64(mine.w >= fat_r2)) == 0ull;
                if constexpr (LATTICE && AX >= 0) {
                    if (((small_mask >> ((pbase >> 6) - cg)) & 1ull) && rest != 0ull
                        && __builtin_amdgcn_ballot_w64(keep && mine.w < s_lat_r2[wv]) != 0ull) {
                        const float s1 = AX == 0 ? mine.y : mine.x;
                        const float s2 = AX == 2 ? mine.y : mine.z;
                        float q1 = INFINITY, q2 = INFINITY;
#pragma unroll 1
                        for (int k = 0; k < 8; ++k) {
                            q1 = fminf(q1, fabsf(s1 - s_lat[wv][0][k]));
                            q2 = fminf(q2, fabsf(s2 - s_lat[wv][1][k]));
                        }
                        const float nan_if_nan = (s1 + s2) * 0.0f;
                        const float b2_lo = (FAST ? __builtin_fmaf(q1, q1, q2 * q2) : q1 * q1 + q2 * q2) + nan_if_nan;
                        keep = keep && !(b2_lo >= mine.w);
                        rest = __builtin_amdgcn_ballot_w64(keep);
                    }
                }
#ifdef GRACE_PACKET_STATS
                if (MODE == MODE_STATS) { st_tested += __builtin_popcountll(rest); }
#endif
                constexpr bool COMPACT = f4_class_split(MODE);
                bool skip_round = rest == 0ull;
                if (!PLANNED && !skip_round && (CLASSES || SPLIT)) {
                    const int pf = pbase + __builtin_ctzll(rest);
                    if (CLASSES && pf >= cur_granule_end) enter_granule(pf);
                    if (SPLIT && !(CLASSES ? cur_owned : owns_granule(pf >> GRANULE_SHIFT)))
                        skip_round = true;
                    else if (CHUNKED && (MODE == MODE_HITS || a.chunk_counts) && (pf >> a.chunk_shift) != cur_chunk)
                        enter_chunk(pf >> a.chunk_shift);
                }
                if (!skip_round) {
                if (LDS_TILE) {
                    const int slot = PLANNED ? lane : COMPACT
                        ? int(__builtin_amdgcn_mbcnt_hi(uint32_t(rest >> 32),
                                                        __builtin_amdgcn_mbcnt_lo(uint32_t(rest), 0u)))
                        : lane;
                    float sw[NW + 3] = {};
                    if constexpr (WEIGHTED) {
#pragma unroll
                        for (int c = 0; c < NW; ++c) sw[c] = FAST ? mw[c] * mineb.y : mw[c];
                    }
                    if (LEAN4 && lean_round) {
                        const float s1 = AX == 0 ? mine.y : mine.x;
                        const float s2 = AX == 2 ? mine.y : mine.z;
                        if constexpr (WEIGHTED) {
                            if (keep) tile4[slot] = make_float4(s1, s2, mineb.x, sw[0]);
                            if (NW > 1 && keep) tile4[66 + slot] = make_float4(sw[1], sw[2], sw[3], 0.f);
                        } else {
                        if (keep) tile4[slot] = make_float4(s1, s2, mineb.x, mineb.y);
                        }
                    } else if (!COMPACT || keep) {
                        s_tile[wv][0][slot] = make_float2(mine.x, mine.y);
                        s_tile[wv][LDS_TILE ? 1 : 0][slot] = make_float2(mine.z, mine.w);
                        if (NEED_B) s_tile[wv][LDS_TILE ? 2 : 0][slot] = mineb;
                        if constexpr (WEIGHTED) {
#pragma unroll
                            for (int p = 0; p < WP; ++p) s_tile[wv][3 + p][slot] = make_float2(sw[2 * p], sw[2 * p + 1]);
                        }
                    }
                }
                if (D4) {
                    double* t = s_tile_d[wv][lane];
                    const double ir = 1.f / mined.w;
                    t[0] = mined.x; t[1] = mined.y; t[2] = mined.z;
                    t[3] = mined.w * mined.w;
                    t[4] = ir; t[5] = ir * ir;
                }
                if (F4D) {
                    const float4 f = make_float4(float(mined.x), float(mined.y), float(mined.z), float(mined.w));
                    const float ir = 1.f / f.w;
                    s_tile_f[wv][lane][0] = make_float4(f.x, f.y, f.z, f.w * f.w);
                    s_tile_f[wv][lane][F4D ? 1 : 0] = make_float4(ir, ir * ir, 0.f, 0.f);
                }
                const unsigned long long todo = rest;
                STAMP_ADD(st_cull, st_t2);
                const unsigned long long st_t3 = STAMP_NOW(); (void)st_t3;
#ifdef GRACE_STAMPS
                st_rounds += 1; st_nsurv += __builtin_popcountll(todo);
#endif
                auto process = [&](auto lean_tag, const float4 s, const BRec sb, const int jj) {
                    constexpr bool LEAN = decltype(lean_tag)::value;
                    if constexpr (D4) {
                        const double* sp = s_tile_d[wv][jj - pbase];
                        const double sx = sp[0], sy = sp[1], sz = sp[2], sw2 = sp[3];
                        double dot_p, b2;
                        if (AX >= 0) {
                            const double sa = AX == 0 ? sx : AX == 1 ? sy : sz;
                            const double s1 = AX == 0 ? sy : sx;
                            const double s2 = AX == 2 ? sy : sz;
                            const double q1 = s1 - double(o1), q2 = s2 - double(o2);
                            dot_p = (sa - double(oa)) * double(da);
                            b2 = q1 * q1 + q2 * q2;
                        } else {
                            const double px = sx - ox, py = sy - oy, pz = sz - oz;
                            dot_p = px * rdx + py * rdy + pz * rdz;
                            const double bx = px - dot_p * rdx, by = py - dot_p * rdy, bz = pz - dot_p * rdz;
                            b2 = bx * bx + by * by + bz * bz;
                        }
                        const bool hit = !(b2 >= sw2) && !(dot_p < 0.0f) && !(dot_p >= len);
                        if (output(MODE) == OUT_COUNTS) {
                            count += hit ? 1 : 0;
                        } else if (hit) {
                            const double ir = sp[4];
                            double x = (N_TABLE - 1) * (sqrt(b2) * ir);
                            int x_idx = static_cast<int>(x);
                            if (x_idx >= N_TABLE - 1) { x = double(N_TABLE - 1); x_idx = N_TABLE - 2; }
                            const double2 y = s_lut[x_idx];
                            double integral = __builtin_fma(x - x_idx, y.y, y.x);
                            integral *= sp[5];
                            if (output(MODE) == OUT_SUMS) {
                                sum_d += integral;
                            } else if (valid) {
                                a.hit_idx[write_at] = jj;
                                a.hit_integral_d[write_at] = integral;
                                a.hit_dist_d[write_at] = dot_p;
                                ++write_at;
                            }
                        }
                    } else if constexpr (F4D) {
                        const float4 r0 = s_tile_f[wv][jj - pbase][0], r1 = s_tile_f[wv][jj - pbase][F4D ? 1 : 0];
                        double dot_p, b2;
                        if (AX >= 0) {
                            const float sa = AX == 0 ? r0.x : AX == 1 ? r0.y : r0.z;
                            const float s1 = AX == 0 ? r0.y : r0.x;
                            const float s2 = AX == 2 ? r0.y : r0.z;
                            const double q1 = s1 - o1, q2 = s2 - o2;
                            dot_p = double(sa - oa) * double(da);
                            b2 = q1 * q1 + q2 * q2;
                        } else {
                            const double px = r0.x - ox, py = r0.y - oy, pz = r0.z - oz;
                            dot_p = px * rdx + py * rdy + pz * rdz;
                            const double bx = px - dot_p * rdx, by = py - dot_p * rdy, bz = pz - dot_p * rdz;
                            b2 = bx * bx + by * by + bz * bz;
                        }
                        const bool hit = !(b2 >= double(r0.w)) && !(dot_p < 0.0f) && !(dot_p >= len);
                        if (output(MODE) == OUT_COUNTS) {
                            count += hit ? 1 : 0;
                        } else if (hit && output(MODE) == OUT_SUMS) {
                            const float b = float((N_TABLE - 1) * (sqrt(b2) * double(r1.x)));
                            int x_idx = static_cast<int>(b);
                            float t = b - static_cast<float>(x_idx);
                            if (x_idx >= N_TABLE - 1) { t = 1.0f; x_idx = N_TABLE - 2; }
                            const double2 y = s_lut[x_idx];
                            float integral = static_cast<float>(__builtin_fma(double(t), y.y, y.x));
                            integral *= r1.y;
                            sum_d += integral;
                        } else if (hit && valid) {
                            const double ir = r1.x;
                            double x = (N_TABLE - 1) * (sqrt(b2) * ir);
                            int x_idx = static_cast<int>(x);
                            if (x_idx >= N_TABLE - 1) { x = double(N_TABLE - 1); x_idx = N_TABLE - 2; }
                            const double2 y = s_lut[x_idx];
                            double integral = __builtin_fma(x - x_idx, y.y, y.x);
                            integral *= ir * ir;
                            a.hit_idx[write_at] = jj;
                            a.hit_integral_d[write_at] = integral;
                            a.hit_dist_d[write_at] = dot_p;
                            ++write_at;
                        }
                    } else if (MODE == MODE_TRI) {
                        float t;
                        if (tri_intersect(ddx, ddy, ddz, ox, oy, oz, a.T64 + 9 * size_t(jj), &t)) {
                            if (t <= tri_tmin && t >= 1E-14f) {
                                tri_tmin = t;
                                tri_data = jj;
                            }
                        }
                    } else {
                        float b2, dot_p;
                        if (AX >= 0) {
                            const float sa = AX == 0 ? s.x : AX == 1 ? s.y : s.z;
                            const float s1 = AX == 0 ? s.y : s.x;
                            const float s2 = AX == 2 ? s.y : s.z;
                            const float q1 = s1 - o1, q2 = s2 - o2;
                            dot_p = LEAN ? 0.0f : __builtin_fmaf(sa, da, noda);
                            b2 = FAST ? __builtin_fmaf(q1, q1, q2 * q2) : q1 * q1 + q2 * q2;
                        } else {
                            const float px = s.x - ox, py = s.y - oy, pz = s.z - oz;
                            dot_p = px * dx + py * dy + pz * dz;
                            const float bx = px - dot_p * dx;
                            const float by = py - dot_p * dy;
                            const float bz = pz - dot_p * dz;
                            b2 = FAST ? __builtin_fmaf(bx, bx, __builtin_fmaf(by, by, bz * bz))
                                      : bx * bx + by * by + bz * bz;
                        }
                        if constexpr (FAST && LEAN) {
                            const float b = fminf(__builtin_amdgcn_sqrtf(b2) * sb.x, float(N_TABLE - 1));
                            const float2 y = s_lutf[static_cast<int>(b)];
                            if constexpr (WEIGHTED) {
                                const float t = __builtin_fmaf(y.y, b, y.x);
#pragma unroll
                                for (int c = 0; c < NW; ++c) wsum[c] = __builtin_fmaf(t, sb.w[c], wsum[c]);
                            } else {
                                sum = __builtin_fmaf(__builtin_fmaf(y.y, b, y.x), sb.y, sum);
                            }
                            return;
                        }
                        const bool hit = LEAN ? !(b2 >= s.w)
                                              : !(b2 >= s.w) && !(dot_p < 0.0f) && !(dot_p >= len);
#ifdef GRACE_PACKET_STATS
                        if (MODE == MODE_STATS && __builtin_amdgcn_ballot_w64(hit) != 0ull) ++st_nodes;
#endif
                        if (!integrates(MODE)) {
                            count += hit ? 1 : 0;
                        } else if (hit) {
                            const float w = FAST ? hit_integral_fast(b2, sb.x, s_lutf)
                                                 : hit_integral(b2, sb.x, sb.y, s_lut);
                            if constexpr (WEIGHTED) {
#pragma unroll
                                for (int c = 0; c < NW; ++c)
                                    wsum[c] = FAST ? __builtin_fmaf(w, sb.w[c], wsum[c]) : wsum[c] + sb.w[c] * w;
                            } else {
                            if (FAST) {
                                sum = __builtin_fmaf(w, sb.y, sum);
                            } else if (MODE == MODE_CUMULATIVE) {
                                sum += w;
                            } else if (valid && !STAGE_HITS) {
                                a.hit_idx[write_at] = jj;
                                a.hit_integral[write_at] = w;
                                a.hit_dist[write_at] = dot_p;
                                ++write_at;
                            } else if (valid) {
                                const int wvh = threadIdx.x >> 6;
                                s_hits[wvh][0][staged][lane] = __int_as_float(jj);
                                s_hits[wvh][STAGE_HITS ? 1 : 0][staged][lane] = w;
                                s_hits[wvh][STAGE_HITS ? 2 : 0][staged][lane] = dot_p;
                                ++staged;
                                ++write_at;
                            }
                            }
                        }
                        if (STAGE_HITS && __builtin_amdgcn_ballot_w64(staged == HIT_CAP) != 0ull)
                            drain_hits();
                    }
                };
                auto fetch = [&](unsigned long long& td, int& k, float4& c, BRec& cb, int& jj) {
                    int at;
                    if (COMPACT) {
                        at = k++;
                        jj = 0;
                    } else {
                        at = __builtin_ctzll(td);
                        td = (td & ~(1ull << at)) | 0x8000000000000000ull;
                        jj = min(pbase + at, r_hi - 1);
                    }
                    if (LDS_TILE) {
                        const float2 xy = s_tile[wv][0][at];
                        const float2 zw = s_tile[wv][LDS_TILE ? 1 : 0][at];
                        c = make_float4(xy.x, xy.y, zw.x, zw.y);
                        if constexpr (WEIGHTED) {
                            const float2 b = s_tile[wv][2][at];
                            cb.x = b.x; cb.y = b.y;
#pragma unroll
                            for (int p = 0; p < WP; ++p) {
                                const float2 wp = s_tile[wv][3 + p][at];
                                cb.w[2 * p] = wp.x;
                                cb.w[2 * p + 1] = wp.y;
                            }
                        } else {
                        if (NEED_B) cb = s_tile[wv][LDS_TILE ? 2 : 0][at];
                        }
                        __builtin_amdgcn_sched_barrier(0);
                    } else if (!fp64(MODE)) {
                        c = a.A[jj];
                    }
                };
                auto run = [&](auto lean_tag) {
                    float4 c0, c1, c2;
                    BRec b0 = make_float2(0.f, 0.f), b1 = b0, b2 = b0;
                    int j0, j1 = 0, j2 = 0;
                    int left = __builtin_popcountll(todo);
                    unsigned long long td = todo | 0x8000000000000000ull;
                    int k = 0;
                    fetch(td, k, c0, b0, j0);
                    fetch(td, k, c1, b1, j1);
                    for (;;) {
                        fetch(td, k, c2, b2, j2);
                        process(lean_tag, c0, b0, j0);
                        if (--left == 0) break;
                        fetch(td, k, c0, b0, j0);
                        process(lean_tag, c1, b1, j1);
                        if (--left == 0) break;
                        fetch(td, k, c1, b1, j1);
                        process(lean_tag, c2, b2, j2);
                        if (--left == 0) break;
                    }
                };
                auto run_lean4 = [&](auto fat_tag) {
                    constexpr bool FAT = decltype(fat_tag)::value;
                    float4 c0, c1, c2;
                    int left = __builtin_popcountll(todo);
                    const float4* t4 = tile4;
                    if constexpr (WEIGHTED && NW > 1) {
                        float4 x0, x1;
                        auto procw = [&](const float4 c, const float4 x) {
                            const float q1 = c.x - o1, q2 = c.y - o2;
                            float b = __builtin_amdgcn_sqrtf(__builtin_fmaf(q1, q1, q2 * q2)) * c.z;
                            if (!FAT) b = fminf(b, float(N_TABLE - 1));
                            const float2 y = s_lutf[static_cast<int>(b)];
                            const float t = __builtin_fmaf(y.y, b, y.x);
                            const float xw[4] = { c.w, x.x, x.y, x.z };
#pragma unroll
                            for (int ch = 0; ch < NW; ++ch) wsum[ch] = __builtin_fmaf(t, xw[ch], wsum[ch]);
                        };
                        c0 = t4[0]; x0 = t4[66]; __builtin_amdgcn_sched_barrier(0);
                        for (;;) {
                            c1 = t4[1]; x1 = t4[67]; __builtin_amdgcn_sched_barrier(0);
                            procw(c0, x0);
                            if (--left == 0) break;
                            c0 = t4[2]; x0 = t4[68]; __builtin_amdgcn_sched_barrier(0);
                            procw(c1, x1);
                            if (--left == 0) break;
                            t4 += 2;
                        }
                        return;
                    }
                    auto proc = [&](const float4 c) {
                        const float q1 = c.x - o1, q2 = c.y - o2;
                        float b = __builtin_amdgcn_sqrtf(__builtin_fmaf(q1, q1, q2 * q2)) * c.z;
                        if (!FAT) b = fminf(b, float(N_TABLE - 1));
                        const float2 y = s_lutf[static_cast<int>(b)];
                        if constexpr (WEIGHTED) wsum[0] = __builtin_fmaf(__builtin_fmaf(y.y, b, y.x), c.w, wsum[0]);
                        else sum = __builtin_fmaf(__builtin_fmaf(y.y, b, y.x), c.w, sum);
                    };
                    c0 = t4[0]; __builtin_amdgcn_sched_barrier(0);
                    c1 = t4[1]; __builtin_amdgcn_sched_barrier(0);
                    for (;;) {
                        c2 = t4[2]; __builtin_amdgcn_sched_barrier(0);
                        proc(c0);
                        if (--left == 0) break;
                        c0 = t4[3]; __builtin_amdgcn_sched_barrier(0);
                        proc(c1);
                        if (--left == 0) break;
                        c1 = t4[4]; __builtin_amdgcn_sched_barrier(0);
                        proc(c2);
                        if (--left == 0) break;
                        t4 += 3;
                    }
                };
                if constexpr (LEAN4) {
                    if (lean_round) {
                        if (fat_round) run_lean4(std::true_type());
                        else run_lean4(std::false_type());
                    } else run(std::false_type());
                } else {
                    if (lean_round) run(std::true_type());
                    else run(std::false_type());
                }
                STAMP_ADD(st_surv, st_t3);
                }
                    if (!more) break;
                }
            }
            };
            switch (axis) {
            case 0: sweep_range(std::integral_constant<int, 0>()); break;
            case 1: sweep_range(std::integral_constant<int, 1>()); break;
            case 2: sweep_range(std::integral_constant<int, 2>()); break;
            default:
                if constexpr (!PLANNED) {
                    if (is_pencil) sweep_range(std::integral_constant<int, -2>());
                    else sweep_range(std::integral_constant<int, -1>());
                }
                break;
            }
            junk |= warm;
        }
    }

#ifdef GRACE_STAMPS
    if (lane == 0) {
        atomicAdd(&g_stamp_acc[0], __builtin_amdgcn_s_memtime() - st_begin);
        atomicAdd(&g_stamp_acc[1], st_walk); atomicAdd(&g_stamp_acc[2], st_cluster);
        atomicAdd(&g_stamp_acc[3], st_cull); atomicAdd(&g_stamp_acc[4], st_surv);
        atomicAdd(&g_stamp_acc[5], st_rounds); atomicAdd(&g_stamp_acc[6], st_nsurv);
        atomicAdd(&g_stamp_acc[7], 1ull);
        {
            const unsigned slot = atomicAdd(&g_stamp_n, 1u) & 0xffffu;
            g_stamp_log[slot][0] = st_begin; g_stamp_log[slot][1] = __builtin_amdgcn_s_memtime();
            g_stamp_log[slot][2] = st_nsurv; g_stamp_log[slot][3] = st_walk;
        }
    }
#endif
    if (STAGE_HITS) drain_hits();
    if (CHUNKED && MODE == MODE_COUNT && a.chunk_counts) leave_chunk();
    if ((overflow || junk < 0) && lane == 0) *a.status = GRACE_STACK_OVERFLOW;
    if (!valid) return;
    if (output(MODE) == OUT_COUNTS) {
        if (!SPLIT) a.out_counts[ray_index] = count;
        else if (count) atomicAdd(&a.out_counts[ray_index], count);
    }
    if (MODE == MODE_TRI) a.out_counts[ray_index] = tri_data;
    if (double_sums(MODE)) {
        if (cur_granule >= 0) s_class_d[wv_acc][cur_granule & (SUM_CLASSES - 1)][lane] = sum_d;
        const int c_lo = SPLIT ? own_lo : 0, c_n = SPLIT ? classes_per_part : SUM_CLASSES;
        for (int w = 1; w < c_n; w *= 2)
            for (int c = c_lo; c < c_lo + c_n; c += 2 * w) {
                const double x = s_class_d[wv_acc][c][lane], y = s_class_d[wv_acc][c + w][lane];
                s_class_d[wv_acc][c][lane] = x + y;
            }
        if (!SPLIT) a.out_sums_d[ray_index] = s_class_d[wv_acc][0][lane];
        else a.partial_d[size_t(ray_index) * split + part] = s_class_d[wv_acc][c_lo][lane];
    }
    if (MODE == MODE_CUMULATIVE) {
        if (cur_granule >= 0) s_class[wv_acc][cur_granule & (SUM_CLASSES - 1)][lane] = sum;
        float t[SUM_CLASSES];
#pragma unroll
        for (int c = 0; c < SUM_CLASSES; ++c) t[c] = s_class[wv_acc][c][lane];
        float result = 0.f;
        if (!SPLIT) {
#pragma unroll
            for (int w = 1; w < SUM_CLASSES; w *= 2)
#pragma unroll
                for (int c = 0; c < SUM_CLASSES; c += 2 * w) t[c] = t[c] + t[c + w];
            result = t[0];
            a.out_sums[ray_index] = result;
        } else {
            for (int w = 1; w < classes_per_part; w *= 2)
                for (int c = own_lo; c < own_hi; c += 2 * w) {
                    const float x = s_class[wv_acc][c][lane], y = s_class[wv_acc][c + w][lane];
                    s_class[wv_acc][c][lane] = x + y;
                }
            a.partial[size_t(ray_index) * split + part] = s_class[wv_acc][own_lo][lane];
        }
    }
    if constexpr (WEIGHTED) {
        if (cur_granule >= 0) {
#pragma unroll
            for (int c = 0; c < NW; ++c) s_class[wv_acc][(cur_granule & (SUM_CLASSES - 1)) * NW + c][lane] = wsum[c];
        }
#pragma unroll
        for (int ch = 0; ch < NW; ++ch) {
            if (!SPLIT) {
                float t[SUM_CLASSES];
#pragma unroll
                for (int c = 0; c < SUM_CLASSES; ++c) t[c] = s_class[wv_acc][c * NW + ch][lane];
#pragma unroll
                for (int w = 1; w < SUM_CLASSES; w *= 2)
#pragma unroll
                    for (int c = 0; c < SUM_CLASSES; c += 2 * w) t[c] = t[c] + t[c + w];
                a.out_sums[size_t(ray_index) * a.out_stride + ch] = t[0];
            } else {
                for (int w = 1; w < classes_per_part; w *= 2)
                    for (int c = own_lo; c < own_hi; c += 2 * w) {
// ... 15 lines not shown
```

### grace-devel_amd/csrc/trace_planned.hip

```cpp
#include "trace_kernel.hpp"

#include <vector>

using namespace grace_hip;

namespace {

struct PlanRef {
    uint4* entries;
    const int2* spans;
    int* counts;
    PlanCtl* ctl;
    int force;
};

template <bool FUSED>
__global__ __launch_bounds__(TRACE_BLOCK) void plan_record_kernel(const TraceArgs a, const PlanRef pl)
{
    __shared__ float s_lat[TRACE_BLOCK / 64][2][8];
    if (pl.spans && !pl.force && pl.ctl->record == 0u) return;
    const int lane = threadIdx.x & 63, wv = threadIdx.x >> 6;
    const int n_packets = (a.n_rays + a.width - 1) / a.width;
    const int packet = blockIdx.x * (TRACE_BLOCK / 64) + wv;
    if (packet >= n_packets) return;
    const PacketRay ray = load_packet_ray(a, packet * a.width, lane);
    const int axis = packet_axis(ray.dx, ray.dy, ray.dz);
    const float4* const group_boxes = a.C + 2 * ((size_t(a.n_prims) + 63) >> 6) + 1;
    const int covered = min(__float_as_int(group_boxes[-1].y), a.n_prims);
    int cnt = 0;
    int round_n = 0, round_bits = 0;
    int t_surv = 0, t_rounds = 0, t_full = 0, t_cap = 0, t_flag = 0, t_max = 0;
    bool failed = axis < 0 || covered < 0;
    if (!failed) {
        const AxisRay ar = axis_ray(axis, ray);
        float noda_lo, noda_hi, len_lo, da0;
        bool same_sense;
        axis_extremes(ar, ray.len, noda_lo, noda_hi, len_lo, da0, same_sense);
        const float lo1 = wave_min(ar.o1), hi1 = wave_max(ar.o1), lo2 = wave_min(ar.o2), hi2 = wave_max(ar.o2);
        const float ea = ar.oa + ar.da * ray.len;
        const float alo = wave_min(fminf(ar.oa, ea)), ahi = wave_max(fmaxf(ar.oa, ea));
        const float fat_r2 = fat_radius2(hi1 - lo1, hi2 - lo2);
        bool lat_ok;
        float cell2;
        build_origin_lattice(ar.o1, ar.o2, lane, s_lat, lat_ok, cell2);
        const float lat_r2 = lat_ok ? cell2 : 0.f;

        auto box_may_hit = [&](const float4 blo, const float4 bhi, const bool along) {
            const float l1 = axis == 0 ? blo.y : blo.x, h1 = axis == 0 ? bhi.y : bhi.x;
            const float l2 = axis == 2 ? blo.y : blo.z, h2 = axis == 2 ? bhi.y : bhi.z;
            const float la = axis == 0 ? blo.x : axis == 1 ? blo.y : blo.z;
            const float ha = axis == 0 ? bhi.x : axis == 1 ? bhi.y : bhi.z;
            return !(l1 > hi1) && !(h1 < lo1) && !(l2 > hi2) && !(h2 < lo2)
                && (!along || (!(la > ahi) && !(ha < alo)));
        };
        const int n_groups = int((size_t(covered) + (size_t(1) << a.group_shift) - 1) >> a.group_shift);
        for (int g0 = 0; g0 < n_groups; g0 += 64) {
            const int gj = min(g0 + lane, n_groups - 1);
            const bool g_may = box_may_hit(group_boxes[2 * size_t(gj)], group_boxes[2 * size_t(gj) + 1], true);
            const int n_g = min(64, n_groups - g0);
            unsigned long long gmask = __builtin_amdgcn_ballot_w64(g_may) & (n_g >= 64 ? ~0ull : ((1ull << n_g) - 1ull));
            while (gmask != 0ull) {
                const int g = g0 + __builtin_ctzll(gmask);
                gmask &= gmask - 1ull;
                const int r_lo = g << a.group_shift;
                const int r_hi = r_lo + min(1 << a.group_shift, covered - r_lo);
                const int c_first = r_lo >> 6, c_last = (r_hi - 1) >> 6;
                for (int cg = c_first; cg <= c_last; cg += 64) {
                    const int cj = min(cg + lane, c_last);
                    const bool c_may = box_may_hit(a.C[2 * size_t(cj)], a.C[2 * size_t(cj) + 1], false);
                    const int n_c = min(64, c_last - cg + 1);
                    unsigned long long cmask = __builtin_amdgcn_ballot_w64(c_may)
                        & (n_c >= 64 ? ~0ull : ((1ull << n_c) - 1ull));
                    while (cmask != 0ull) {
                        const int c = cg + __builtin_ctzll(cmask);
                        cmask &= cmask - 1ull;
                        const int pbase = c << 6;
                        const int pj = min(max(pbase + lane, r_lo), r_hi - 1);
                        const float4 mine = a.A[pj];
                        const int lo_bit = max(r_lo - pbase, 0), hi_bit = min(r_hi - pbase, 64);
                        const unsigned long long m_mask =
                            (hi_bit >= 64 ? ~0ull : ((1ull << hi_bit) - 1ull)) & (~0ull << lo_bit);
                        const float s1 = axis == 0 ? mine.y : mine.x;
                        const float s2 = axis == 2 ? mine.y : mine.z;
                        const float sa = axis == 0 ? mine.x : axis == 1 ? mine.y : mine.z;
                        const float q1 = s1 - __builtin_amdgcn_fmed3f(s1, lo1, hi1);
                        const float q2 = s2 - __builtin_amdgcn_fmed3f(s2, lo2, hi2);
                        const float b2_lo = FUSED ? __builtin_fmaf(q1, q1, q2 * q2) : q1 * q1 + q2 * q2;
                        bool keep = !(b2_lo >= mine.w);
                        unsigned long long rest = __builtin_amdgcn_ballot_w64(keep) & m_mask;
                        keep = __builtin_amdgcn_inverse_ballot_w64(rest);
                        if (rest != 0ull && __builtin_amdgcn_ballot_w64(keep && mine.w < lat_r2) != 0ull) {
                            float p1 = INFINITY, p2 = INFINITY;
                            for (int k = 0; k < 8; ++k) {
                                p1 = fminf(p1, fabsf(s1 - s_lat[wv][0][k]));
                                p2 = fminf(p2, fabsf(s2 - s_lat[wv][1][k]));
                            }
                            const float nan_if_nan = (s1 + s2) * 0.0f;
                            const float l2 = (FUSED ? __builtin_fmaf(p1, p1, p2 * p2) : p1 * p1 + p2 * p2) + nan_if_nan;
                            keep = keep && !(l2 >= mine.w);
                            rest = __builtin_amdgcn_ballot_w64(keep);
                        }
                        if (rest == 0ull) continue;
                        const unsigned long long inside =
                            __builtin_amdgcn_ballot_w64(__builtin_fmaf(sa, da0, noda_lo) >= 0.0f)
                            & __builtin_amdgcn_ballot_w64(__builtin_fmaf(sa, da0, noda_hi) < len_lo);
                        const bool lean = same_sense && (rest & ~inside) == 0ull;
                        const bool fat = FUSED && (rest & ~__builtin_amdgcn_ballot_w64(mine.w >= fat_r2)) == 0ull;
                        const int cls = (c >> (GRANULE_SHIFT - 6)) & (SUM_CLASSES - 1);
                        const int n = __builtin_amdgcn_readlane(cnt, cls);
                        const int bits = (lean ? 1 : 0) | (fat ? 2 : 0);
                        const int n_surv = __builtin_popcountll(rest);
                        const int open_n = __builtin_amdgcn_readlane(round_n, cls);
                        const int open_bits = __builtin_amdgcn_readlane(round_bits, cls);
                        const bool close_cap = n > 0 && open_n + n_surv > 64;
                        const bool close_flag = n > 0 && !close_cap && open_bits != bits;
                        const bool close = close_cap || close_flag;
                        if (pl.spans) {
                            const int2 span = pl.spans[packet * SUM_CLASSES + cls];
                            if (n < span.y) {
                                if (lane == 0) {
                                    if (close) pl.entries[size_t(span.x) + n - 1].w = uint32_t(open_bits) | PLAN_ROUND_END;
                                    pl.entries[size_t(span.x) + n] =
                                        make_uint4(uint32_t(c), uint32_t(rest), uint32_t(rest >> 32), uint32_t(bits));
                                }
                            } else {
                                failed = true;
                            }
                        }
                        if (lane == cls) {
                            if (close) {
                                t_rounds += 1; t_full += open_n == 64 ? 1 : 0;
                                t_cap += close_cap ? 1 : 0; t_flag += close_flag ? 1 : 0;
                                t_max = max(t_max, open_n);
                                round_n = 0;
                            }
                            round_n += n_surv; round_bits = bits;
                            t_surv += n_surv;
                            cnt += 1;
                        }
                    }
                }
            }
        }
    }
    if (failed) {
        cnt = 0;
        if (lane == 0) { pl.ctl->unusable = 1u; pl.ctl->usable = 0u; }
    }
    if (lane < SUM_CLASSES) pl.counts[packet * SUM_CLASSES + lane] = cnt;
    if (pl.spans && !failed) {
        for (int cls = 0; cls < SUM_CLASSES; ++cls) {
            const int n = __builtin_amdgcn_readlane(cnt, cls);
            const int open_bits = __builtin_amdgcn_readlane(round_bits, cls);
            if (n > 0 && lane == 0)
                pl.entries[size_t(pl.spans[packet * SUM_CLASSES + cls].x) + n - 1].w = uint32_t(open_bits) | PLAN_ROUND_END;
        }
        if (lane < SUM_CLASSES && cnt > 0) {
            t_rounds += 1; t_full += round_n == 64 ? 1 : 0;
            t_max = max(t_max, round_n);
        }
        if (lane >= SUM_CLASSES) cnt = 0;
        int tally[6] = { cnt, t_surv, t_rounds, t_full, t_cap, t_flag };
#pragma unroll
        for (int off = 1; off < SUM_CLASSES; off <<= 1) {
#pragma unroll
            for (int k = 0; k < 6; ++k) tally[k] += __shfl_xor(tally[k], off);
            t_max = max(t_max, __shfl_xor(t_max, off));
        }
        if (lane == 0) {
#pragma unroll
            for (int k = 0; k < 6; ++k)
                if (tally[k]) atomicAdd(&pl.ctl->stats[k], (unsigned long long)tally[k]);
            atomicMax(&pl.ctl->largest_round, uint32_t(t_max));
        }
    }
}

grace_status launch_record(const bool fast, const TraceArgs& a, const PlanRef& pl, hipStream_t stream)
{
    const int n_packets = (a.n_rays + a.width - 1) / a.width;
    const int grid = ceil_div(size_t(n_packets), size_t(TRACE_BLOCK / 64));
    if (fast) plan_record_kernel<true><<<grid, TRACE_BLOCK, 0, stream>>>(a, pl);
    else plan_record_kernel<false><<<grid, TRACE_BLOCK, 0, stream>>>(a, pl);
    GRACE_CHECK_LAUNCH();
    return GRACE_OK;
}

grace_status plan_free_buffers(PacketPlan& pp)
{
    void* bufs[] = { pp.entries, pp.spans, pp.counts, pp.ctl };
    bool any = false;
    for (void* b : bufs) any = any || b;
    if (any) GRACE_TRY_HIP(hipDeviceSynchronize());
    for (void* b : bufs)
        if (b) GRACE_TRY_HIP(hipFree(b));
    pp.entries = nullptr; pp.spans = nullptr; pp.counts = nullptr; pp.ctl = nullptr;
    pp.valid = false;
    pp.n_lists = pp.n_entries = pp.recorded = 0;
    return GRACE_OK;
}

}

namespace grace_hip {

grace_status plan_release(TraceState& ts)
{
    GRACE_TRY(plan_free_buffers(ts.plan));
    ts.plan = PacketPlan();
    ts.last_plan_ctl = nullptr;
    return GRACE_OK;
}

grace_status plan_fill(TraceState& ts, const PlanKey& key, const TraceArgs& a, hipStream_t stream)
{
    PacketPlan& pp = ts.plan;
    GRACE_TRY(plan_free_buffers(pp));
    ts.last_plan_ctl = nullptr;
    pp.key = key;
    pp.dead = true;
    const int n_packets = (a.n_rays + a.width - 1) / a.width;
    const size_t n_lists = size_t(n_packets) * SUM_CLASSES;
    auto alloc = [&](auto*& ptr, const size_t bytes) {
        if (hipMalloc(reinterpret_cast<void**>(&ptr), bytes) == hipSuccess) return true;
        (void)hipGetLastError();
        ptr = nullptr;
        return false;
    };
    if (n_lists * (sizeof(int) + sizeof(int2)) > ts.plan_budget) return GRACE_OK;
    if (!alloc(pp.counts, n_lists * sizeof(int)) || !alloc(pp.spans, n_lists * sizeof(int2))
        || !alloc(pp.ctl, sizeof(PlanCtl)))
        return plan_free_buffers(pp);
    GRACE_TRY_HIP(hipMemsetAsync(pp.ctl, 0, sizeof(PlanCtl), stream));
    GRACE_TRY(launch_record(key.fast, a, PlanRef{ nullptr, nullptr, pp.counts, pp.ctl, 1 }, stream));
    std::vector<int> counts(n_lists);
    PlanCtl seen = {};
    GRACE_TRY_HIP(hipMemcpyAsync(counts.data(), pp.counts, n_lists * sizeof(int), hipMemcpyDeviceToHost, stream));
    GRACE_TRY_HIP(hipMemcpyAsync(&seen, pp.ctl, sizeof(seen), hipMemcpyDeviceToHost, stream));
    GRACE_TRY_HIP(hipStreamSynchronize(stream));
    if (seen.unusable) return plan_free_buffers(pp);
    std::vector<int2> spans(n_lists);
    size_t total = 0, used = 0;
    for (size_t l = 0; l < n_lists; ++l) {
        const size_t room = size_t(counts[l]) + size_t(counts[l]) / 8 + 2;
        spans[l] = make_int2(int(total), int(room));
        total += room;
        used += size_t(counts[l]);
        if (total >= (size_t(1) << 31)) return plan_free_buffers(pp);
    }
    const size_t bytes = (total + 4) * sizeof(uint4) + n_lists * (sizeof(int) + sizeof(int2));
    if (bytes > ts.plan_budget || !alloc(pp.entries, (total + 4) * sizeof(uint4))) return plan_free_buffers(pp);
    GRACE_TRY_HIP(hipMemcpy(pp.spans, spans.data(), n_lists * sizeof(int2), hipMemcpyHostToDevice));
    GRACE_TRY_HIP(hipMemsetAsync(pp.entries + total, 0, 4 * sizeof(uint4), stream));
    pp.n_lists = n_lists; pp.n_entries = total; pp.recorded = used;
    GRACE_TRY_HIP(hipMemsetD32Async(reinterpret_cast<hipDeviceptr_t>(&pp.ctl->usable), 1, 1, stream));
    GRACE_TRY_HIP(hipMemcpyAsync(&pp.ctl->sig[0], ts.scene.ctl->sig, 16, hipMemcpyDeviceToDevice, stream));
    GRACE_TRY_HIP(hipMemcpyAsync(&pp.ctl->sig[2], ts.rays.ctl->sig, 16, hipMemcpyDeviceToDevice, stream));
    GRACE_TRY(launch_record(key.fast, a, PlanRef{ pp.entries, pp.spans, pp.counts, pp.ctl, 1 }, stream));
    pp.valid = true;
    pp.dead = false;
    return GRACE_OK;
}

grace_status plan_record(const TraceState& ts, const TraceArgs& a, hipStream_t stream)
{
    const PacketPlan& pp = ts.plan;
    return launch_record(pp.key.fast, a, PlanRef{ pp.entries, pp.spans, pp.counts, pp.ctl, 0 }, stream);
}

grace_status launch_planned(const int mode, const bool fast, const int grid, const TraceArgs& a, hipStream_t stream)
{
    auto go = [&](auto mode_tag) {
        constexpr int MODE = decltype(mode_tag)::value;
        if (fast) trace_kernel<MODE, true, true, false, true><<<grid, TRACE_BLOCK, 0, stream>>>(a);
        else trace_kernel<MODE, true, false, false, true><<<grid, TRACE_BLOCK, 0, stream>>>(a);
    };
    switch (mode) {
    case MODE_CUMULATIVE: go(std::integral_constant<int, MODE_CUMULATIVE>()); break;
    case MODE_WCUM1: go(std::integral_constant<int, MODE_WCUM1>()); break;
    case MODE_WCUM2: go(std::integral_constant<int, MODE_WCUM2>()); break;
    case MODE_WCUM3: go(std::integral_constant<int, MODE_WCUM3>()); break;
    case MODE_WCUM4: go(std::integral_constant<int, MODE_WCUM4>()); break;
    default: return set_error(GRACE_INVALID_ARGUMENT, __FILE__, __LINE__, "no planned kernel for this mode");
    }
    GRACE_CHECK_LAUNCH();
    return GRACE_OK;
}

}
```

### grace-devel_amd/csrc/trace_state.hpp

```cpp
#pragma once

#include "common.hpp"

namespace grace_hip {

constexpr int TRACE_BLOCK = 256;
constexpr int N_TABLE = 51;
constexpr int SPLIT_WIDE_BUDGET = 0x100;

inline int group_shift(size_t n_prims)
{
    int s = 12;
    while (((n_prims + (size_t(1) << s) - 1) >> s) > 4096) ++s;
    return s;
}
inline size_t group_count(size_t n_prims)
{
    const int s = group_shift(n_prims);
    return (n_prims + (size_t(1) << s) - 1) >> s;
}
inline size_t cluster_record_count(size_t n_prims)
{
    return 2 * ((n_prims + 63) / 64) + 1 + 2 * group_count(n_prims);
}
constexpr int MAX_HIT_CHUNKS = 256;
constexpr int SUM_CLASSES = 8;
constexpr int GRANULE_SHIFT = 10;


enum { MODE_COUNT = 0, MODE_CUMULATIVE = 1, MODE_HITS = 2, MODE_STATS = 3, MODE_TRI = 4,
       MODE_COUNT_D4 = 5, MODE_CUM_D4 = 6, MODE_HITS_D4 = 7,
       MODE_COUNT_F4D = 8, MODE_CUM_F4D = 9, MODE_HITS_F4D = 10,
       MODE_WCUM1 = 11, MODE_WCUM2 = 12, MODE_WCUM3 = 13, MODE_WCUM4 = 14 };

enum Primitive { PRIM_F4 = 0,
                 PRIM_TRI = 1,
                 PRIM_D4 = 2,
                 PRIM_F4D = 3 };
enum Output { OUT_COUNTS, OUT_SUMS, OUT_HITS, OUT_STATS, OUT_CLOSEST,
              OUT_WSUMS };

struct ModeParts { Primitive prim; Output out; int channels = 1; };
constexpr ModeParts mode_parts(const int mode)
{
    switch (mode) {
    case MODE_COUNT:      return { PRIM_F4, OUT_COUNTS };
    case MODE_CUMULATIVE: return { PRIM_F4, OUT_SUMS };
    case MODE_HITS:       return { PRIM_F4, OUT_HITS };
    case MODE_STATS:      return { PRIM_F4, OUT_STATS };
    case MODE_TRI:        return { PRIM_TRI, OUT_CLOSEST };
    case MODE_COUNT_D4:   return { PRIM_D4, OUT_COUNTS };
    case MODE_CUM_D4:     return { PRIM_D4, OUT_SUMS };
    case MODE_HITS_D4:    return { PRIM_D4, OUT_HITS };
    case MODE_COUNT_F4D:  return { PRIM_F4D, OUT_COUNTS };
    case MODE_CUM_F4D:    return { PRIM_F4D, OUT_SUMS };
    case MODE_HITS_F4D:   return { PRIM_F4D, OUT_HITS };
    case MODE_WCUM1:      return { PRIM_F4, OUT_WSUMS, 1 };
    case MODE_WCUM2:      return { PRIM_F4, OUT_WSUMS, 2 };
    case MODE_WCUM3:      return { PRIM_F4, OUT_WSUMS, 3 };
    case MODE_WCUM4:      return { PRIM_F4, OUT_WSUMS, 4 };
    }
    __builtin_unreachable();
}
constexpr Primitive primitive(const int mode) { return mode_parts(mode).prim; }
constexpr Output output(const int mode) { return mode_parts(mode).out; }
constexpr int channels(const int mode) { return mode_parts(mode).channels; }
constexpr int MAX_LAUNCH_CHANNELS = 4;
constexpr bool weighted(const int mode) { return output(mode) == OUT_WSUMS; }

constexpr bool fp64(const int mode) { return primitive(mode) == PRIM_D4 || primitive(mode) == PRIM_F4D; }
constexpr bool class_split(const int mode)
{
    return output(mode) == OUT_COUNTS || output(mode) == OUT_SUMS || output(mode) == OUT_WSUMS;
}
constexpr bool f4_class_split(const int mode) { return class_split(mode) && primitive(mode) == PRIM_F4; }
constexpr bool f4_sums(const int mode)
{
    return primitive(mode) == PRIM_F4 && (output(mode) == OUT_SUMS || output(mode) == OUT_WSUMS);
}
constexpr bool double_sums(const int mode) { return output(mode) == OUT_SUMS && fp64(mode); }
constexpr bool ordered(const int mode) { return output(mode) == OUT_HITS || output(mode) == OUT_CLOSEST; }
constexpr bool integrates(const int mode)
{
    return output(mode) == OUT_SUMS || output(mode) == OUT_WSUMS || output(mode) == OUT_HITS;
}
constexpr bool f4_integrals(const int mode) { return integrates(mode) && primitive(mode) == PRIM_F4; }
constexpr bool has_lattice(const int mode) { return primitive(mode) == PRIM_F4 && output(mode) != OUT_STATS; }
constexpr bool chunked(const int mode)
{
    return primitive(mode) == PRIM_F4 && (output(mode) == OUT_COUNTS || output(mode) == OUT_HITS);
}

struct TraceArgs {
    const float* rays;
    const uint32_t* perm;
    int n_rays;
    const float4* spheres;
    const int2* node_prims;
    int treelet;
    int treelet_axis;
    const float4* A;
    const float2* B;
    int group_shift;
    const float4* C;
    const double* T64;
    const double* spheres_d;
    double* out_sums_d;
    double* hit_integral_d;
    double* hit_dist_d;
    int split;
    int n_prims;
    float* partial;
    double* partial_d;
    const int* split_dev;
    const int* lat_dev;
    const int* stage_dev;
    int stage_want;
    int* chunk_counts;
    const int* chunk_off;
    const int4* wave_map;
    const int* n_wave_map;
    bool keep_chunks;
    int chunk_shift, n_chunks;
    int width;
    const float4* nodes;
    int n_nodes;
    const int4* leaves;
    const int* root;
    int* out_counts;
    float* out_sums;
    const int* offsets;
    int* hit_idx;
    float* hit_integral;
    float* hit_dist;
    uint32_t* stats;
    int* status;
    const float* weights;
    int w_stride;
    int out_stride;
    const double* kernel_table;
    const uint4* plan_entries;
    const int2* plan_spans;
    const int* plan_counts;
    const uint32_t* plan_usable;
    const int* plan_split_dev;
};


struct CacheCtl {
    unsigned long long sig[2];
    uint32_t stale;
    uint32_t pad;
};

struct SceneKey {
    Primitive kind = PRIM_F4;
    const void* prims = nullptr; const void* nodes = nullptr; const void* leaves = nullptr;
    size_t n_prims = 0, n_nodes = 0;
    bool operator==(const SceneKey& o) const
    {
        return kind == o.kind && prims == o.prims && nodes == o.nodes && leaves == o.leaves
            && n_prims == o.n_prims && n_nodes == o.n_nodes;
    }
};

struct Scene {
    bool valid = false;
    SceneKey key;
    SceneKey seen;
    float4* A = nullptr; float2* B1 = nullptr; float2* B50 = nullptr; double* T64 = nullptr;
    int2* node_prims = nullptr; float4* C = nullptr;
    CacheCtl* ctl = nullptr;
    bool pinned = false;
    unsigned long long gen = 0;
};

struct RayKey {
    const float* rays = nullptr;
    size_t n = 0;
    bool operator==(const RayKey& o) const { return rays == o.rays && n == o.n; }
};

struct RayOrder {
    bool valid = false;
    RayKey key, seen;
    uint32_t* perm = nullptr;
    uint32_t* ext = nullptr;
    CacheCtl* ctl = nullptr;
    bool pinned = false;
    unsigned long long gen = 0;
};

struct PlanCtl {
    uint32_t record;
    uint32_t unusable;
    uint32_t usable;
    uint32_t largest_round;
    unsigned long long sig[4];
    unsigned long long stats[6];
};
constexpr uint32_t PLAN_ROUND_END = 4u;
constexpr int PLAN_FORMAT = 2;

struct PlanKey {
    int format = PLAN_FORMAT;
    bool fast = false;
    int group_shift = 0, width = 0;
    bool reorder = false;
    size_t n_rays = 0, n_prims = 0;
    unsigned long long scene_gen = 0, rays_gen = 0;
    bool operator==(const PlanKey& o) const
    {
        return format == o.format && fast == o.fast && group_shift == o.group_shift && width == o.width && reorder == o.reorder
            && n_rays == o.n_rays && n_prims == o.n_prims && scene_gen == o.scene_gen && rays_gen == o.rays_gen;
    }
};

struct PacketPlan {
    bool valid = false;
    bool dead = false;
    PlanKey key;
    uint4* entries = nullptr;
    int2* spans = nullptr;
    int* counts = nullptr;
    PlanCtl* ctl = nullptr;
    size_t n_lists = 0, n_entries = 0;
    size_t recorded = 0;
};

struct PlanGate {
    const CacheCtl* scene = nullptr;
    const CacheCtl* rays = nullptr;
    PlanCtl* ctl = nullptr;
};

__host__ __device__ inline int planned_split(const int n_packets)
{
    return n_packets <= 8192 ? SUM_CLASSES : SUM_CLASSES / 2;
}

struct HitsCache {
    int* chunk_counts = nullptr;
    size_t capacity = 0;
    bool valid = false;
    const void* rays = nullptr; const void* prims = nullptr;
    size_t n_rays = 0, n_prims = 0;
    int n_chunks = 0;
};

struct TraceState {
    int* status = nullptr;
    const int* last_lat_dev = nullptr;
    hipStream_t last_lat_stream = nullptr;
    bool timing = false;
    hipEvent_t ev0 = nullptr, ev1 = nullptr;
    bool ev_valid = false;
    bool ray_reorder = true;
    int treelet = -1;
    int split = -1;
    int lat_split = 4;
    int width = -1;
    bool exact_integrals = false;
    bool hits_stage_split = true;
    bool cache_validation = true;
    bool cache_auto = true;
    int sph_kernel = 0;
    const double* builtin_tables = nullptr;
    const double* kernel_table = nullptr;
    double* custom_table = nullptr;
    double custom_host[N_TABLE] = {};
    bool plan_on = true;
    size_t plan_budget = size_t(512) << 20;
    Scene scene;
    RayOrder rays;
    HitsCache hits;
    unsigned long long cache_gen = 0;
    PacketPlan plan;
    const PlanCtl* last_plan_ctl = nullptr;
    hipStream_t last_plan_stream = nullptr;
};

grace_status trace_state(TraceState** out);

inline grace_status ensure_status(TraceState& ts, hipStream_t stream)
{
    if (!ts.status) {
        GRACE_TRY_HIP(hipMalloc(reinterpret_cast<void**>(&ts.status), sizeof(int)));
        GRACE_TRY_HIP(hipMemsetAsync(ts.status, 0, sizeof(int), stream));
    }
    return GRACE_OK;
}

template <typename Launches>
grace_status timed(TraceState& ts, hipStream_t stream, Launches launches)
{
    if (ts.timing) {
        if (!ts.ev0) { GRACE_TRY_HIP(hipEventCreate(&ts.ev0)); GRACE_TRY_HIP(hipEventCreate(&ts.ev1)); }
        GRACE_TRY_HIP(hipEventRecord(ts.ev0, stream));
    }
    GRACE_TRY(launches());
    if (ts.timing) {
        GRACE_TRY_HIP(hipEventRecord(ts.ev1, stream));
        ts.ev_valid = true;
    }
    return GRACE_OK;
}

size_t sig_partial_words();
struct SigRequest {
    const void* prims = nullptr; size_t prims_bytes = 0;
    const void* nodes = nullptr; size_t nodes_bytes = 0;
    const void* leaves = nullptr; size_t leaves_bytes = 0;
    CacheCtl* scene_ctl = nullptr; bool scene_force = false;
    const void* rays = nullptr; size_t rays_bytes = 0;
    CacheCtl* rays_ctl = nullptr; bool rays_force = false;
    uint32_t* rays_ext = nullptr;
};
grace_status launch_signatures(const SigRequest& rq, unsigned long long* partial, hipStream_t stream);

grace_status scene_release(TraceState& ts);
grace_status scene_cache_alloc(TraceState& ts, const SceneKey& key);
grace_status scene_fill(Primitive kind, const void* prims, size_t n_prims, const float4* nodes,
                        size_t n_nodes, const int4* leaves, float4* A, float2* B1, float2* B50,
                        double* T64, int2* node_prims, float4* C, hipStream_t stream,
                        const uint32_t* run_if = nullptr);
grace_status scene_prepare(TraceState& ts, Primitive kind, const void* prims, size_t n_prims,
                           const int* d_nodes, size_t n_nodes, const int* d_leaves, hipStream_t stream);

grace_status rays_release(TraceState& ts);
grace_status rays_cache_alloc(TraceState& ts, const RayKey& key);
grace_status ray_order(const float* d_rays, size_t n_rays, uint32_t* ext, uint32_t* keys, uint32_t* perm,
                       const float4* scene_min, uint32_t* lat_flag, int n_packets, int split, int* split_dev,
                       hipStream_t stream, const uint32_t* run_if = nullptr);
grace_status rays_prepare(TraceState& ts, const float* d_rays, size_t n_rays, hipStream_t stream);
grace_status launch_choose_variants(const uint32_t* ext12, int n, const float4* scene_min, uint32_t* lat_flag,
                                    int split_packets, int split_launched, int* split_dev, hipStream_t stream,
                                    const PlanGate* gate = nullptr, int* plan_split_dev = nullptr);

grace_status plan_release(TraceState& ts);
grace_status plan_fill(TraceState& ts, const PlanKey& key, const TraceArgs& a, hipStream_t stream);
grace_status plan_record(const TraceState& ts, const TraceArgs& a, hipStream_t stream);
grace_status launch_planned(int mode, bool fast, int grid, const TraceArgs& a, hipStream_t stream);

}
```

### grace-devel_amd/grace_hip/__init__.py

```python
import collections
import ctypes as C
import os

import numpy as np
import torch

_HERE = os.path.dirname(os.path.abspath(__file__))
LIB_PATH = os.path.join(os.path.dirname(_HERE), "lib", "libgrace_hip.so")

if not os.path.exists(LIB_PATH):
    raise ImportError(
        "libgrace_hip.so is not built (%s). Run __graft_entry__.build() or "
        "`make -C grace-devel_amd`. There is no CPU fallback." % LIB_PATH)

_lib = C.CDLL(LIB_PATH)
_lib.grace_last_error.restype = C.c_char_p
_lib.grace_version.restype = C.c_int

GRACE_OK = 0
GRACE_INVALID_ARGUMENT = 1
GRACE_HIP_ERROR = 2
GRACE_OUT_OF_MEMORY = 3
GRACE_STACK_OVERFLOW = 4

# ... 187 lines not shown
def build_ALBVH(tree, prims, deltas, prim_kind=PRIM_SPHERE_F4, delta_comp=COMP_LESS):
    n = len(prims)
    assert tree.leaves.shape[0] >= n and len(deltas) == n + 1
    if deltas.dtype not in _DELTA_CODES:
        raise ValueError("deltas must be float32/float64 or 32/64-bit XOR deltas")
    n_leaves = C.c_size_t(0)
    _check(_lib.grace_albvh_build_ex(C.c_int(prim_kind), _ptr(prims), C.c_size_t(n),
                                     C.c_int(_DELTA_CODES[deltas.dtype]), _ptr(deltas), C.c_int(delta_comp),
                                     C.c_int(tree.max_per_leaf), _ptr(tree.nodes), _ptr(tree.leaves),
                                     _ptr(tree.root_index), C.byref(n_leaves), _stream()))
    tree.leaves = tree.leaves[: n_leaves.value]
    tree.nodes = tree.nodes[: n_leaves.value - 1]
    return tree


def min_max_components(data, n_comp, first=0):
    code = {torch.float32: 0, torch.float64: 1, torch.int32: 2}[data.dtype]
    assert data.dim() == 2 and data.is_contiguous() and first + n_comp <= data.shape[1]
    npdt = {0: np.float32, 1: np.float64, 2: np.int32}[code]
    lo = np.zeros(n_comp, npdt); hi = np.zeros(n_comp, npdt)
    elem = data.element_size()
    _check(_lib.grace_minmax_components(C.c_void_p(data.data_ptr() + first * elem), C.c_size_t(len(data)),
                                        C.c_int(code), C.c_int(n_comp), C.c_size_t(data.shape[1] * elem),
                                        lo.ctypes.data_as(C.c_void_p), hi.ctypes.data_as(C.c_void_p), _stream()))
    return lo, hi


def build_tree(spheres, tree, low=None, high=None, want_perm=False):
    deltas = torch.empty(len(spheres) + 1, dtype=torch.float32, device=spheres.device)
    keys = torch.empty(len(spheres), dtype=torch.int32, device=spheres.device)
    morton_keys_sph(spheres, keys, low, high)
    perm = sort_by_key(keys, spheres, 0, 30, want_perm=want_perm)
    euclidean_deltas_sph(spheres, deltas)
    ALBVH_sph(spheres, deltas, tree)
    return (tree, perm) if want_perm else tree


def _check_rays(rays):
    _rays(rays)
    if len(rays) % 32 != 0:
        raise ValueError("Number of rays must be a multiple of the warp size (32).")


def _trace_args(rays, spheres, tree):
    return (_ptr(rays), C.c_size_t(len(rays)), _ptr(_spheres(spheres)), C.c_size_t(len(spheres)),
            _ptr(tree.nodes), C.c_size_t(tree.n_nodes), _ptr(tree.leaves), _ptr(tree.root_index))


def hit_integrals(b2, h):
    out = torch.empty_like(b2)
    _check(_lib.grace_hit_integrals_f32(_ptr(b2), _ptr(h), C.c_size_t(len(b2)), _ptr(out), _stream()))
    return out


def enable_kernel_timing(enabled=True):
    _check(_lib.grace_trace_enable_timing(C.c_int(1 if enabled else 0)))


def last_kernel_ms():
    ms = C.c_float(0)
    _check(_lib.grace_trace_last_kernel_ms(C.byref(ms)))
    return ms.value


def last_lattice():
    v = C.c_int(0)
    _check(_lib.grace_trace_last_lattice(C.byref(v)))
    return v.value


def set_packet_split(k):
    _check(_lib.grace_trace_set_packet_split(C.c_int(int(k))))


def set_packet_width(w):
    _check(_lib.grace_trace_set_packet_width(C.c_int(int(w))))


def set_exact_integrals(enabled):
    _check(_lib.grace_trace_set_exact_integrals(C.c_int(1 if enabled else 0)))


SPH_KERNELS = ("cubic", "quartic", "quintic", "wendland_c2", "wendland_c4", "wendland_c6")
SPH_KERNEL_CUSTOM = -1


def _kernel_kind(name):
    if name not in SPH_KERNELS:
        raise ValueError("unknown SPH kernel %r (one of %s)" % (name, ", ".join(SPH_KERNELS)))
    return SPH_KERNELS.index(name)


def sph_kernel_table(name):
    out = (C.c_double * N_TABLE)()
    _check(_lib.grace_sph_kernel_table(C.c_int(_kernel_kind(name)), out))
    return np.array(out, np.float64)


def set_sph_kernel(kernel):
    if isinstance(kernel, str):
        _check(_lib.grace_trace_set_sph_kernel(C.c_int(_kernel_kind(kernel))))
        return
    t = np.asarray(kernel)
    if t.dtype.kind not in "fiu" or t.ndim != 1:
        raise ValueError("an SPH kernel table must be a 1-D array of 51 numbers")
    t = np.ascontiguousarray(t, dtype=np.float64)
    _check(_lib.grace_trace_set_sph_kernel_table(t.ctypes.data_as(C.POINTER(C.c_double)), C.c_int(len(t))))


def sph_kernel():
    kind = C.c_int(0)
    out = (C.c_double * N_TABLE)()
    _check(_lib.grace_trace_get_sph_kernel(C.byref(kind), out))
    name = "custom" if kind.value == SPH_KERNEL_CUSTOM else SPH_KERNELS[kind.value]
    return name, np.array(out, np.float64)


def set_cache_validation(enabled):
    _check(_lib.grace_trace_set_cache_validation(C.c_int(1 if enabled else 0)))


def set_cache_auto(enabled):
    _check(_lib.grace_trace_set_cache_auto(C.c_int(1 if enabled else 0)))


def set_plan(enabled):
    _check(_lib.grace_trace_set_plan(C.c_int(1 if enabled else 0)))


def set_plan_budget(n_bytes):
    _check(_lib.grace_trace_set_plan_budget(C.c_size_t(int(n_bytes))))


def plan_bytes():
    v = C.c_size_t(0)
    _check(_lib.grace_trace_plan_bytes(C.byref(v)))
    return v.value


def last_plan_used():
    v = C.c_int(0)
    _check(_lib.grace_trace_last_plan_used(C.byref(v)))
    return v.value


PlanStats = collections.namedtuple(
    "PlanStats", "entries survivors rounds full_rounds closed_by_capacity closed_by_flags largest_round")


def plan_stats():
    v = (C.c_ulonglong * 7)()
    _check(_lib.grace_trace_plan_stats(v))
    return PlanStats(*[int(x) for x in v])


def set_lattice_split(k):
    _check(_lib.grace_trace_set_lattice_split(C.c_int(k)))


def set_hits_staging(enabled):
    _check(_lib.grace_trace_set_hits_staging(C.c_int(1 if enabled else 0)))


class Context:

    def __init__(self):
        self._h = C.c_void_p(0)
        _check(_lib.grace_context_create(C.byref(self._h)))

    def make_current(self):
        _check(_lib.grace_context_set_current(self._h))

    @staticmethod
    def reset_current():
        _check(_lib.grace_context_set_current(C.c_void_p(0)))

    def destroy(self):
        if self._h:
            _check(_lib.grace_context_destroy(self._h))
            self._h = C.c_void_p(0)

    def __enter__(self):
        self.make_current()
        return self

    def __exit__(self, *exc):
        Context.reset_current()
        self.destroy()
        return False


def set_treelet_size(n):
    _check(_lib.grace_trace_set_treelet_size(C.c_int(int(n))))


def set_ray_reorder(enabled):
    _check(_lib.grace_trace_set_ray_reorder(C.c_int(1 if enabled else 0)))


def trace_status():
    _check(_lib.grace_trace_status(_stream()))


_prepared = {}


def trace_prepare(spheres, tree):
    _check(_lib.grace_trace_prepare_f4(_ptr(_spheres(spheres)), C.c_size_t(len(spheres)),
                                       _ptr(tree.nodes), C.c_size_t(tree.n_nodes),
                                       _ptr(tree.leaves), _stream()))
    _prepared["scene"] = (spheres, tree.nodes, tree.leaves)


def trace_prepare_tri(tris, tree):
    _check(_lib.grace_trace_prepare_tri(_ptr(_tris(tris)), C.c_size_t(len(tris)),
                                        _ptr(tree.nodes), C.c_size_t(tree.n_nodes),
                                        _ptr(tree.leaves), _stream()))
    _prepared["scene"] = (tris, tree.nodes, tree.leaves)


def trace_prepare_rays(rays):
    _check(_lib.grace_trace_prepare_rays(_ptr(_rays(rays)), C.c_size_t(len(rays)), _stream()))
    _prepared["rays"] = rays


def trace_release_rays():
    _check(_lib.grace_trace_release_rays())
    _prepared.pop("rays", None)


def trace_release():
    _check(_lib.grace_trace_release())
    _prepared.pop("scene", None)


def _trace_hitcounts_keep(rays, spheres, tree, hit_counts, real=torch.float32):
    _check_rays(rays)
    fn = _lib.grace_trace_hitcounts_f4_f64 if real == torch.float64 else _lib.grace_trace_hitcounts_keep_f4
    _check(fn(*_trace_args(rays, spheres, tree), _ptr(hit_counts), _stream()))
    return hit_counts


def _real_of(real):
    assert real in (torch.float32, torch.float64), "real: torch.float32 or torch.float64"
    return real


def trace_hitcounts_f4_f64(rays, spheres, tree, hit_counts, check=False):
    _check_rays(rays)
    assert hit_counts.dtype == torch.int32 and len(hit_counts) == len(rays)
    _check(_lib.grace_trace_hitcounts_f4_f64(*_trace_args(rays, spheres, tree), _ptr(hit_counts), _stream()))
    if check:
        trace_status()
    return hit_counts


def trace_hitcounts_sph(rays, spheres, tree, hit_counts, check=False):
    _check_rays(rays)
    assert hit_counts.dtype == torch.int32 and len(hit_counts) == len(rays)
    _check(_lib.grace_trace_hitcounts_f4(*_trace_args(rays, spheres, tree), _ptr(hit_counts),
                                         _stream()))
    if check:
        trace_status()
    return hit_counts


def trace_cumulative_sph(rays, spheres, tree, cumulated, check=False):
    _check_rays(rays)
    assert cumulated.dtype in (torch.float32, torch.float64) and len(cumulated) == len(rays)
    fn = _lib.grace_trace_cumulative_f4_f64 if cumulated.dtype == torch.float64 else _lib.grace_trace_cumulative_f4
    _check(fn(*_trace_args(rays, spheres, tree), _ptr(cumulated), _stream()))
    if check:
        trace_status()
    return cumulated


def trace_cumulative_weighted_sph(rays, spheres, tree, weights, out=None, check=False):
    _check_rays(rays)
    if weights.dtype != torch.float32:
        raise ValueError("weights must be float32")
    if weights.dim() not in (1, 2) or weights.shape[0] != len(spheres):
        raise ValueError("weights must have shape [n_spheres] or [n_spheres, C]")
    n_ch = 1 if weights.dim() == 1 else weights.shape[1]
    if not 1 <= n_ch <= 64:
        raise ValueError("weights must have 1..64 channels")
    shape = (len(rays),) if weights.dim() == 1 else (len(rays), n_ch)
    if out is None:
        out = torch.empty(shape, dtype=torch.float32, device=rays.device)
    if out.dtype != torch.float32 or tuple(out.shape) != shape:
        raise ValueError("out must be float32 of shape %s" % (shape,))
    _check(_lib.grace_trace_cumulative_weighted_f4(*_trace_args(rays, spheres, tree), _ptr(weights),
                                                   C.c_int(n_ch), _ptr(out), _stream()))
    if check:
        trace_status()
    return out


def trace_emission_absorption_sph(rays, spheres, tree, emission, absorption, out=None, tau=None,
                                  check=False):
    _check_rays(rays)
    if emission.dtype != torch.float32 or absorption.dtype != torch.float32:
        raise ValueError("emission and absorption must be float32")
    if emission.dim() not in (1, 2) or emission.shape[0] != len(spheres):
        raise ValueError("emission must have shape [n_spheres] or [n_spheres, C]")
    if tuple(absorption.shape) != (len(spheres),):
        raise ValueError("absorption must have shape [n_spheres]")
# ... 1002 lines not shown
```

### include/grace_hip.h

```cpp
#ifndef GRACE_HIP_H
#define GRACE_HIP_H

#include <stddef.h>
#include <stdint.h>

#ifdef __cplusplus
extern "C" {
#endif

typedef enum grace_status {
    GRACE_OK = 0,
    GRACE_INVALID_ARGUMENT = 1,
    GRACE_HIP_ERROR = 2,
    GRACE_OUT_OF_MEMORY = 3,
    GRACE_STACK_OVERFLOW = 4
} grace_status;

typedef void* grace_stream;

int grace_version(void);
const char* grace_last_error(void);

grace_status grace_device_malloc(void** d_ptr, size_t bytes);
grace_status grace_device_free(void* d_ptr);
// ... 65 lines not shown
grace_status grace_sort_last_stats(grace_sort_stats* h_stats);

grace_status grace_deltas_euclid_f4(const float* d_spheres, size_t n, float* d_deltas,
                                    grace_stream stream);
grace_status grace_deltas_area_f4(const float* d_spheres, size_t n, float* d_deltas,
                                  grace_stream stream);
grace_status grace_deltas_xor_u32(const uint32_t* d_keys, size_t n, uint32_t* d_deltas,
                                  grace_stream stream);
grace_status grace_deltas_xor_u64(const uint64_t* d_keys, size_t n, uint64_t* d_deltas,
                                  grace_stream stream);

grace_status grace_albvh_build_f4(const float* d_spheres, size_t n, const float* d_deltas,
                                  int max_per_leaf, int* d_nodes, int* d_leaves, int* d_root,
                                  size_t* h_n_leaves, grace_stream stream);
grace_status grace_albvh_build_f4_u32(const float* d_spheres, size_t n, const uint32_t* d_deltas,
                                      int max_per_leaf, int* d_nodes, int* d_leaves,
                                      int* d_root, size_t* h_n_leaves, grace_stream stream);

grace_status grace_centroid_bounds_tri(const float* d_tris, size_t n, float* h_bot, float* h_top,
                                       grace_stream stream);
grace_status grace_morton_keys30_tri(const float* d_tris, size_t n, const float* h_bot,
                                     const float* h_top, uint32_t* d_keys, grace_stream stream);
grace_status grace_albvh_build_tri_u32(const float* d_tris, size_t n, const uint32_t* d_deltas,
                                       int max_per_leaf, int* d_nodes, int* d_leaves, int* d_root,
                                       size_t* h_n_leaves, grace_stream stream);

enum { GRACE_PRIM_SPHERE_F4 = 0, GRACE_PRIM_TRIANGLE = 1, GRACE_PRIM_SPHERE_D4 = 2, GRACE_PRIM_BOX = 3 };
enum { GRACE_DELTA_F32 = 0, GRACE_DELTA_F64 = 1, GRACE_DELTA_U32 = 2, GRACE_DELTA_U64 = 3 };
enum { GRACE_COMP_LESS = 0, GRACE_COMP_GREATER = 1 };
grace_status grace_albvh_build_ex(int prim_kind, const void* d_prims, size_t n, int delta_type,
                                  const void* d_deltas, int delta_comp, int max_per_leaf,
                                  int* d_nodes, int* d_leaves, int* d_root, size_t* h_n_leaves,
                                  grace_stream stream);

grace_status grace_albvh_enable_timing(int enabled);
grace_status grace_albvh_last_phase_ms(float* h_leaves_ms, float* h_nodes_ms);
grace_status grace_trace_closest_tri(const void* d_rays, size_t n_rays, const float* d_tris,
                                     size_t n_tris, const int* d_nodes, size_t n_nodes,
                                     const int* d_leaves, const int* d_root, int* d_closest,
                                     grace_stream stream);

grace_status grace_trace_hitcounts_f4(const void* d_rays, size_t n_rays, const float* d_spheres,
                                      size_t n_spheres, const int* d_nodes, size_t n_nodes,
                                      const int* d_leaves, const int* d_root,
                                      int* d_hit_counts, grace_stream stream);
grace_status grace_trace_hitcounts_keep_f4(const void* d_rays, size_t n_rays, const float* d_spheres,
                                           size_t n_spheres, const int* d_nodes, size_t n_nodes,
                                           const int* d_leaves, const int* d_root,
                                           int* d_hit_counts, grace_stream stream);
grace_status grace_trace_cumulative_f4(const void* d_rays, size_t n_rays, const float* d_spheres,
                                       size_t n_spheres, const int* d_nodes, size_t n_nodes,
                                       const int* d_leaves, const int* d_root,
                                       float* d_cumulated, grace_stream stream);
grace_status grace_trace_cumulative_weighted_f4(const void* d_rays, size_t n_rays, const float* d_spheres,
                                                size_t n_spheres, const int* d_nodes, size_t n_nodes,
                                                const int* d_leaves, const int* d_root,
                                                const float* d_weights, int n_channels, float* d_out,
                                                grace_stream stream);
grace_status grace_trace_emission_absorption_f4(const void* d_rays, size_t n_rays, const float* d_spheres,
                                                size_t n_spheres, const int* d_nodes, size_t n_nodes,
                                                const int* d_leaves, const int* d_root,
                                                const float* d_emission, int n_channels,
                                                const float* d_absorption, float* d_out, float* d_tau,
                                                grace_stream stream);
grace_status grace_trace_absorption_deposit_f4(const void* d_rays, size_t n_rays, const float* d_spheres,
                                               size_t n_spheres, const int* d_nodes, size_t n_nodes,
                                               const int* d_leaves, const int* d_root,
                                               const float* d_luminosity, const float* d_absorption,
                                               int n_channels, double* d_deposit, float* d_transmitted,
                                               double* d_quantum, grace_stream stream);
typedef struct grace_spectrum_grid {
    double v0;
    double dv;
    int    n_bins;
    int    periodic;
    double hubble;
} grace_spectrum_grid;
grace_status grace_trace_spectra_f4(const void* d_rays, size_t n_rays, const float* d_spheres,
                                    size_t n_spheres, const int* d_nodes, size_t n_nodes,
                                    const int* d_leaves, const int* d_root,
                                    const float* d_amount, const float* d_width, const float* d_velocity,
                                    int n_channels, const grace_spectrum_grid* grid, float* d_tau,
                                    float* d_column, grace_stream stream);
grace_status grace_trace_set_ordered_budget(size_t bytes);
grace_status grace_trace_ordered_limits(int* wave_max_hits, int* block_max_hits);
typedef struct grace_ordered_stats {
    unsigned long long batches;
    unsigned long long total_hits;
    unsigned long long rays_wave, rays_block, rays_global;
    unsigned long long budget_bytes, frame_bytes;
    float ms_count, ms_trace, ms_composite;
} grace_ordered_stats;
grace_status grace_trace_ordered_enable_stats(int enabled);
grace_status grace_trace_ordered_last_stats(grace_ordered_stats* h_stats);
grace_status grace_trace_hits_f4(const void* d_rays, size_t n_rays, const float* d_spheres,
                                 size_t n_spheres, const int* d_nodes, size_t n_nodes,
                                 const int* d_leaves, const int* d_root,
                                 const int* d_ray_offsets, int* d_hit_indices,
                                 float* d_hit_integrals, float* d_hit_distances,
                                 grace_stream stream);
grace_status grace_trace_stats_f4(const void* d_rays, size_t n_rays, const float* d_spheres,
                                  size_t n_spheres, const int* d_nodes, size_t n_nodes,
                                  const int* d_leaves, const int* d_root,
                                  uint32_t* d_stats4, grace_stream stream);

grace_status grace_hit_integrals_f32(const float* d_b2, const float* d_h, size_t n, float* d_out,
                                     grace_stream stream);

grace_status grace_trace_set_ray_reorder(int enabled);

grace_status grace_trace_enable_timing(int enabled);
grace_status grace_trace_last_kernel_ms(float* h_ms);

grace_status grace_trace_last_lattice(int* h_lattice);

grace_status grace_trace_set_packet_split(int waves_per_packet);

grace_status grace_trace_set_packet_width(int rays_per_packet);

grace_status grace_trace_set_exact_integrals(int enabled);

#define GRACE_SPH_KERNEL_CUSTOM      (-1)
#define GRACE_SPH_KERNEL_CUBIC       0
#define GRACE_SPH_KERNEL_QUARTIC     1
#define GRACE_SPH_KERNEL_QUINTIC     2
#define GRACE_SPH_KERNEL_WENDLAND_C2 3
#define GRACE_SPH_KERNEL_WENDLAND_C4 4
#define GRACE_SPH_KERNEL_WENDLAND_C6 5
grace_status grace_trace_set_sph_kernel(int kind);
grace_status grace_trace_set_sph_kernel_table(const double* h_table, int n);
grace_status grace_trace_get_sph_kernel(int* h_kind, double* h_table51);
grace_status grace_sph_kernel_table(int kind, double* h_out51);

grace_status grace_trace_set_treelet_size(int max_primitives);

grace_status grace_trace_set_lattice_split(int waves_per_packet);
grace_status grace_trace_set_hits_staging(int enabled);

grace_status grace_trace_prepare_f4(const float* d_spheres, size_t n_spheres, const int* d_nodes,
                                    size_t n_nodes, const int* d_leaves, grace_stream stream);
grace_status grace_trace_prepare_tri(const float* d_tris, size_t n_tris, const int* d_nodes,
                                     size_t n_nodes, const int* d_leaves, grace_stream stream);
grace_status grace_trace_release(void);
grace_status grace_trace_prepare_rays(const void* d_rays, size_t n_rays, grace_stream stream);
grace_status grace_trace_release_rays(void);
grace_status grace_trace_set_cache_validation(int enabled);
grace_status grace_trace_set_cache_auto(int enabled);

grace_status grace_trace_set_plan(int on);
grace_status grace_trace_set_plan_budget(size_t bytes);
grace_status grace_trace_plan_bytes(size_t* h_bytes);
grace_status grace_trace_last_plan_used(int* h_used);
grace_status grace_trace_plan_stats(unsigned long long* h_stats );

grace_status grace_trace_status(grace_stream stream);

grace_status grace_scan_exclusive_i32(const int* d_in, size_t n, int* d_out, long long* h_total,
                                      grace_stream stream);
grace_status grace_segscan_exclusive_f32(const int* d_segment_offsets, size_t n_segments,
                                         const float* d_data, size_t n, float* d_results,
                                         grace_stream stream);
grace_status grace_segscan_exclusive_f64(const int* d_segment_offsets, size_t n_segments,
                                         const double* d_data, size_t n, double* d_results,
                                         grace_stream stream);
grace_status grace_add_iota_i32(int* d_values, size_t n, grace_stream stream);
grace_status grace_fill_u32(void* d_values, size_t n, uint32_t bits, grace_stream stream);
grace_status grace_multiply_by_weights_f32(const float* d_unweighted, size_t n,
                                           const float* d_weights, const uint32_t* d_weight_map,
                                           float* d_weighted, grace_stream stream);
grace_status grace_multiply_by_weights_f64(const double* d_unweighted, size_t n,
                                           const double* d_weights, const uint32_t* d_weight_map,
                                           double* d_weighted, grace_stream stream);

grace_status grace_sort_by_distance_f32(float* d_distances, const int* d_ray_offsets,
                                        size_t n_rays, size_t n_hits, int* d_hit_indices,
                                        float* d_hit_data, grace_stream stream);

grace_status grace_sort_by_distance_f64(double* d_distances, const int* d_ray_offsets,
                                        size_t n_rays, size_t n_hits, int* d_hit_indices,
                                        double* d_hit_data, grace_stream stream);

grace_status grace_rays_orthogonal_z(int n_side, const float* h_mins4, const float* h_maxs4,
                                     void* d_rays, float* h_area, grace_stream stream);
grace_status grace_rays_pinhole(int res_x, int res_y, const float* h_camera, const float* h_look_at,
                                const float* h_view_up, float fovy, float length, void* d_rays,
                                grace_stream stream);
grace_status grace_rays_healpix(int nside, float ox, float oy, float oz, float length,
                                void* d_rays, grace_stream stream);
grace_status grace_rays_isotropic(size_t n_rays, float ox, float oy, float oz, float length,
                                  uint64_t seed, void* d_rays, grace_stream stream);

grace_status grace_rays_isotropic_octant(size_t n_rays, float ox, float oy, float oz, float length,
                                         int octant, uint64_t seed, void* d_rays,
                                         grace_stream stream);
grace_status grace_rays_one_to_many(size_t n_rays, float ox, float oy, float oz,
                                    const void* d_points, int is_double, int elems_per_point,
                                    int sort_type, const float* h_bot, const float* h_top,
                                    void* d_rays, grace_stream stream);
grace_status grace_rays_plane_parallel_random(int width, int height, const float* h_base,
                                              const float* h_w, const float* h_h, float length,
                                              uint64_t seed, void* d_rays, grace_stream stream);
grace_status grace_rays_orthographic_projection(int res_x, int res_y, const float* h_camera,
                                                const float* h_look_at, const float* h_view_up,
                                                float vertical_extent, float length,
                                                void* d_rays, grace_stream stream);

grace_status grace_deltas_euclid_d4(const double* d_spheres, size_t n, float* d_deltas,
                                    grace_stream stream);
grace_status grace_deltas_euclid_d4_f64(const double* d_spheres, size_t n, double* d_deltas,
                                        grace_stream stream);
grace_status grace_deltas_area_d4(const double* d_spheres, size_t n, float* d_deltas,
                                  grace_stream stream);
grace_status grace_deltas_area_d4_f64(const double* d_spheres, size_t n, double* d_deltas,
                                      grace_stream stream);
grace_status grace_albvh_build_f4_u64(const float* d_spheres, size_t n, const uint64_t* d_deltas,
                                      int max_per_leaf, int* d_nodes, int* d_leaves, int* d_root,
                                      size_t* h_n_leaves, grace_stream stream);
grace_status grace_albvh_build_f4_f64(const float* d_spheres, size_t n, const double* d_deltas,
                                      int max_per_leaf, int* d_nodes, int* d_leaves, int* d_root,
                                      size_t* h_n_leaves, grace_stream stream);
grace_status grace_albvh_build_d4_f64(const double* d_spheres, size_t n, const double* d_deltas,
                                      int max_per_leaf, int* d_nodes, int* d_leaves, int* d_root,
                                      size_t* h_n_leaves, grace_stream stream);
grace_status grace_albvh_build_d4_u32(const double* d_spheres, size_t n, const uint32_t* d_deltas,
                                      int max_per_leaf, int* d_nodes, int* d_leaves, int* d_root,
                                      size_t* h_n_leaves, grace_stream stream);
grace_status grace_albvh_build_d4_u64(const double* d_spheres, size_t n, const uint64_t* d_deltas,
                                      int max_per_leaf, int* d_nodes, int* d_leaves, int* d_root,
                                      size_t* h_n_leaves, grace_stream stream);
grace_status grace_albvh_build_d4(const double* d_spheres, size_t n, const float* d_deltas,
                                  int max_per_leaf, int* d_nodes, int* d_leaves, int* d_root,
                                  size_t* h_n_leaves, grace_stream stream);
grace_status grace_trace_hitcounts_d4(const void* d_rays, size_t n_rays, const double* d_spheres,
                                      size_t n_spheres, const int* d_nodes, size_t n_nodes,
                                      const int* d_leaves, const int* d_root, int* d_hit_counts,
                                      grace_stream stream);
grace_status grace_trace_cumulative_d4(const void* d_rays, size_t n_rays, const double* d_spheres,
                                       size_t n_spheres, const int* d_nodes, size_t n_nodes,
                                       const int* d_leaves, const int* d_root, double* d_sums,
                                       grace_stream stream);
grace_status grace_trace_hits_d4(const void* d_rays, size_t n_rays, const double* d_spheres,
                                 size_t n_spheres, const int* d_nodes, size_t n_nodes,
                                 const int* d_leaves, const int* d_root, const int* d_ray_offsets,
                                 int* d_hit_indices, double* d_hit_integrals,
                                 double* d_hit_distances, grace_stream stream);
grace_status grace_trace_status_d4(grace_stream stream);

grace_status grace_trace_hitcounts_f4_f64(const void* d_rays, size_t n_rays, const float* d_spheres,
                                          size_t n_spheres, const int* d_nodes, size_t n_nodes,
                                          const int* d_leaves, const int* d_root, int* d_hit_counts,
                                          grace_stream stream);
grace_status grace_trace_cumulative_f4_f64(const void* d_rays, size_t n_rays, const float* d_spheres,
                                           size_t n_spheres, const int* d_nodes, size_t n_nodes,
                                           const int* d_leaves, const int* d_root, double* d_sums,
                                           grace_stream stream);
grace_status grace_trace_hits_f4_f64(const void* d_rays, size_t n_rays, const float* d_spheres,
                                     size_t n_spheres, const int* d_nodes, size_t n_nodes,
                                     const int* d_leaves, const int* d_root, const int* d_ray_offsets,
                                     int* d_hit_indices, double* d_hit_integrals,
                                     double* d_hit_distances, grace_stream stream);

grace_status grace_interpolate_points_f4(const float* d_points, size_t n_points, int elems_per_point,
                                         const float* d_spheres, size_t n_spheres, const int* d_nodes,
                                         size_t n_nodes, const int* d_leaves, const int* d_root,
                                         const float* d_weights, int n_channels,
                                         float* d_out, int* d_counts, grace_stream stream);
grace_status grace_interpolate_grid_f4(const float* h_origin3, const float* h_uvw9, const int* h_dims3,
                                       const float* d_spheres, size_t n_spheres, const int* d_nodes,
                                       size_t n_nodes, const int* d_leaves, const int* d_root,
                                       const float* d_weights, int n_channels,
                                       float* d_out, int* d_counts, grace_stream stream);
grace_status grace_interpolate_enable_stats(int enabled);
grace_status grace_interpolate_last_stats(unsigned long long* h_survivor_tests);

grace_status grace_nearest_neighbours_f4(const float* d_points, size_t n_points, int elems_per_point,
                                         const float* d_spheres, size_t n_spheres, const int* d_nodes,
                                         size_t n_nodes, const int* d_leaves, const int* d_root,
                                         int k, int* d_indices, float* d_d2, grace_stream stream);
grace_status grace_smoothing_lengths_f4(const float* d_spheres, size_t n_spheres, const int* d_nodes,
                                        size_t n_nodes, const int* d_leaves, const int* d_root,
                                        int k, float eta, float* d_h, grace_stream stream);
grace_status grace_neighbours_enable_stats(int enabled);
grace_status grace_neighbours_last_stats(unsigned long long* h_candidate_tests, unsigned long long* h_packets,
                                         unsigned long long* h_insertion_steps);

grace_status grace_range_counts_f4(const float* d_points, size_t n_points, int elems_per_point,
                                   const float* d_radii, float radius,
                                   const float* d_spheres, size_t n_spheres, const int* d_nodes,
                                   size_t n_nodes, const int* d_leaves, const int* d_root,
                                   const float* d_weights, int n_channels,
                                   int* d_counts, float* d_sums, grace_stream stream);
grace_status grace_range_neighbours_f4(const float* d_points, size_t n_points, int elems_per_point,
                                       const float* d_radii, float radius,
                                       const float* d_spheres, size_t n_spheres, const int* d_nodes,
                                       size_t n_nodes, const int* d_leaves, const int* d_root,
                                       const int* d_offsets, int* d_indices, float* d_d2,
                                       grace_stream stream);

grace_status grace_fof_labels_f4(const float* d_spheres, size_t n_spheres, const int* d_nodes,
                                 size_t n_nodes, const int* d_leaves, const int* d_root,
                                 float linking_length, int* d_labels, grace_stream stream);
grace_status grace_fof_groups(const int* d_labels, size_t n, int min_members, int* d_group_of,
                              int* d_sizes, int* d_n_groups, grace_stream stream);
grace_status grace_fof_members(const int* d_group_of, size_t n, const int* d_sizes, size_t n_groups,
                               int* d_offsets, int* d_members, grace_stream stream);

// ... 103 lines not shown
```

Before: 575.6.

## Compact packet plan into index words and headers, fuse adjacent rounds

Replaces the per-entry uint4 packet plan, which carried a cluster id and a 64-bit mask, with a flat array of precomputed primitive indices plus one 32-bit header per round. The trace kernel can then read its gather index directly per lane instead of rebuilding it through LDS with ballot and mbcnt. For unweighted fast mode, consecutive compatible rounds are fused into loops of up to 128 primitives, so a second tile half is loaded and the inner loop runs over more work per trip. This cuts plan bandwidth and per-round overhead, but the recording pass becomes more complex and LDS tile use and register pressure rise.

```diff
diff --git a/grace-devel_amd/csrc/trace.hip b/grace-devel_amd/csrc/trace.hip
--- a/grace-devel_amd/csrc/trace.hip
+++ b/grace-devel_amd/csrc/trace.hip
@@ -407,9 +407,10 @@
             GRACE_TRY(plan_fill(ts, b.plan_key, a, stream));
         ts.last_plan_ctl = nullptr;
         if (b.plan_eligible && pp.valid && pp.key == b.plan_key) {
-            a.plan_entries = pp.entries; a.plan_spans = pp.spans; a.plan_counts = pp.counts;
+            a.plan_idx = pp.idx; a.plan_hdr = pp.hdr; a.plan_spans = pp.spans; a.plan_counts = pp.counts;
             a.plan_usable = &pp.ctl->usable;
             ts.last_plan_ctl = pp.ctl; ts.last_plan_stream = stream;
+            ts.last_plan_fuses = !weighted(MODE) && p.fast_b;
         }
     }
     return timed(ts, stream, [&] {
@@ -813,6 +814,23 @@
     return GRACE_OK;
 }
 
+grace_status grace_trace_plan_loops(unsigned long long* h_loops)
+{
+    GRACE_REQUIRE(h_loops, "null output");
+    h_loops[0] = h_loops[1] = 0;
+    GRACE_TRACE_STATE();
+    if (ts.last_plan_ctl) {
+        PlanCtl h = {};
+        GRACE_TRY_HIP(hipStreamSynchronize(ts.last_plan_stream));
+        GRACE_TRY_HIP(hipMemcpy(&h, ts.last_plan_ctl, sizeof(h), hipMemcpyDeviceToHost));
+        if (h.usable != 0u) {
+            h_loops[0] = ts.last_plan_fuses ? h.loops : h.stats[2];
+            h_loops[1] = ts.last_plan_fuses ? h.largest_loop : h.largest_round;
+        }
+    }
+    return GRACE_OK;
+}
+
 grace_status grace_trace_set_plan(int on)
 {
     GRACE_TRACE_STATE();
@@ -834,7 +852,7 @@
     GRACE_REQUIRE(h_bytes, "null output");
     GRACE_TRACE_STATE();
     const PacketPlan& pp = ts.plan;
-    *h_bytes = pp.valid ? (pp.n_entries + 4) * sizeof(uint4) + pp.n_lists * (sizeof(int) + sizeof(int2)) + sizeof(PlanCtl) : 0;
+    *h_bytes = pp.valid ? pp.bytes() : 0;
     return GRACE_OK;
 }
 
diff --git a/grace-devel_amd/csrc/trace_coherence.hip b/grace-devel_amd/csrc/trace_coherence.hip
--- a/grace-devel_amd/csrc/trace_coherence.hip
+++ b/grace-devel_amd/csrc/trace_coherence.hip
@@ -190,6 +190,7 @@
             pc.sig[2] = gate.rays->sig[0]; pc.sig[3] = gate.rays->sig[1];
             for (int k = 0; k < 6; ++k) pc.stats[k] = 0ull;
             pc.largest_round = 0u;
+            pc.loops = 0ull; pc.largest_loop = 0u;
         }
     }
 }
diff --git a/grace-devel_amd/csrc/trace_kernel.hpp b/grace-devel_amd/csrc/trace_kernel.hpp
--- a/grace-devel_amd/csrc/trace_kernel.hpp
+++ b/grace-devel_amd/csrc/trace_kernel.hpp
@@ -221,8 +221,8 @@
     }
 }
 
-typedef uint32_t plan_u32x4 __attribute__((ext_vector_type(4)));
-typedef int plan_i32x2 __attribute__((ext_vector_type(2)));
+typedef int plan_i32x4 __attribute__((ext_vector_type(4)));
+typedef uint32_t plan_u32x4 __attribute__((ext_vector_type(4), aligned(4)));
 template <typename T>
 __device__ __forceinline__ const __attribute__((address_space(4))) T* plan_const(const void* p)
 {
@@ -256,12 +256,14 @@
     constexpr bool WEIGHTED = weighted(MODE);
     constexpr int NW = channels(MODE), WP = WEIGHTED ? (NW + 1) / 2 : 0;
     using BRec = std::conditional_t<WEIGHTED, WeightedB<NW>, float2>;
+    constexpr bool FUSE = PLANNED && !WEIGHTED && FAST;
     __shared__ double2 s_lut[FAST ? 1 : N_TABLE];
     constexpr int LUTF_N = 256;
     __shared__ float2 s_lutf[FAST ? LUTF_N : 1];
     constexpr bool D4 = primitive(MODE) == PRIM_D4, F4D = primitive(MODE) == PRIM_F4D;
     constexpr bool LDS_TILE = primitive(MODE) == PRIM_F4;
-    __shared__ __align__(16) float2 s_tile[LDS_TILE ? TRACE_BLOCK / 64 : 1][LDS_TILE ? 3 + WP : 1][LDS_TILE ? 66 : 1];
+    __shared__ __align__(16) float2 s_tile[LDS_TILE ? TRACE_BLOCK / 64 : 1][LDS_TILE ? (FUSE ? 4 : 3 + WP) : 1][LDS_TILE ? 66 : 1];
+    static_assert(!FUSE || 4 * 66 * sizeof(float2) >= (PLAN_LOOP_MAX + 2) * sizeof(float4), "the fused loop's tile");
     __shared__ double s_tile_d[D4 ? TRACE_BLOCK / 64 : 1][D4 ? 64 : 1][D4 ? 6 : 1];
     __shared__ float4 s_tile_f[F4D ? TRACE_BLOCK / 64 : 1][F4D ? 64 : 1][F4D ? 2 : 1];
     const int lane = threadIdx.x & 63;
@@ -580,9 +582,10 @@
     constexpr int FLAT_MAX_GROUPS = 256;
     if (flat && groups_kept > FLAT_MAX_GROUPS) flat = false;
     if (!flat && !PLANNED) push(*a.root, ~0ull);
-    const __attribute__((address_space(4))) plan_u32x4* plan_at = nullptr;
+    const __attribute__((address_space(4))) uint32_t* plan_hdr_at = nullptr;
+    const uint32_t* plan_idx_at = nullptr;
     int plan_n = 0, plan_cls = own_lo;
-    (void)plan_at; (void)plan_n; (void)plan_cls;
+    (void)plan_hdr_at; (void)plan_idx_at; (void)plan_n; (void)plan_cls;
     unsigned long long st_walk = 0, st_cluster = 0, st_cull = 0, st_surv = 0, st_rounds = 0, st_nsurv = 0;
     const unsigned long long st_begin = STAMP_NOW();
     (void)st_walk; (void)st_cluster; (void)st_cull; (void)st_surv; (void)st_rounds; (void)st_nsurv; (void)st_begin;
@@ -594,9 +597,11 @@
         if constexpr (PLANNED) {
             if (plan_cls >= own_hi) break;
             const int list = packet * SUM_CLASSES + plan_cls++;
-            plan_n = plan_const<int>(a.plan_counts)[list];
+            plan_n = plan_const<plan_i32x4>(a.plan_counts)[list].x;
             if (plan_n <= 0) continue;
-            plan_at = plan_const<plan_u32x4>(a.plan_entries) + plan_const<plan_i32x2>(a.plan_spans)[list].x;
+            const plan_i32x4 span = plan_const<plan_i32x4>(a.plan_spans)[list];
+            plan_idx_at = a.plan_idx + span.x;
+            plan_hdr_at = plan_const<uint32_t>(a.plan_hdr) + span.y;
             enter_granule((plan_cls - 1) << GRANULE_SHIFT);
             sweep = true; sweep_count = a.n_prims;
         } else if (flat) {
@@ -741,45 +746,72 @@
                 if (cmask == 0ull) continue;
                 int cnext = cg + __builtin_ctzll(cmask);
                 cmask &= cmask - 1ull;
-                plan_u32x4 e0 = { 0u, 0u, 0u, 0u }, e1 = e0, e2 = e0, e3 = e0;
-                int plan_i = 0;
-                (void)plan_i;
-                if constexpr (PLANNED) { e0 = plan_at[0]; e1 = plan_at[1]; e2 = plan_at[2]; e3 = plan_at[3]; }
+                plan_u32x4 plan_h = { 0u, 0u, 0u, 0u };
+                uint32_t plan_word = 0u, plan_word2 = 0u;
+                int plan_i = 0, plan_w = 0, loop_n = 0, loop_bits = 0;
+                (void)plan_h; (void)plan_word; (void)plan_word2; (void)plan_i; (void)plan_w; (void)loop_n; (void)loop_bits;
+                const uint32_t lane4 = uint32_t(lane) << 2;
+                (void)lane4;
+                auto headers_at = [&](const int round) {
+                    return *reinterpret_cast<const __attribute__((address_space(4))) plan_u32x4*>(plan_hdr_at + round);
+                };
+                (void)headers_at;
+                auto form_loop = [&]() {
+                    if constexpr (PLANNED) {
+                        loop_n = 0;
+                        if (plan_i < plan_n) {
+                            loop_n = plan_header_count(plan_h.x);
+                            loop_bits = plan_header_bits(plan_h.x);
+                            ++plan_i;
+                            if constexpr (FUSE) {
+                                int k = 1;
+                                for (;;) {
+                                    if (k == 4) { plan_h = headers_at(plan_i); k = 0; }
+                                    const uint32_t next = k == 0 ? plan_h.x : k == 1 ? plan_h.y : k == 2 ? plan_h.z : plan_h.w;
+                                    if (!(plan_i < plan_n && planned_fuses(loop_n, loop_bits, next))) break;
+                                    loop_n += plan_header_count(next);
+                                    ++plan_i; ++k;
+                                }
+                            }
+                        }
+                        plan_h = headers_at(plan_i);
+                        const char* const base = reinterpret_cast<const char*>(plan_idx_at + plan_w);
+                        plan_word = *reinterpret_cast<const uint32_t*>(base + lane4);
+                        if constexpr (FUSE)
+                            if (loop_n > 64) plan_word2 = *reinterpret_cast<const uint32_t*>(base + 256 + lane4);
+                    }
+                };
+                if constexpr (PLANNED) {
+                    plan_h = headers_at(0);
+                    form_loop();
+                }
                 float4 mine_next;
                 float2 mineb_next = make_float2(0.f, 0.f);
                 int round_n_next = 0;
                 uint32_t round_bits_next = 0u;
-                (void)round_n_next; (void)round_bits_next;
+                float4 mine2_next = make_float4(0.f, 0.f, 0.f, 0.f);
+                float2 mine2b_next = make_float2(0.f, 0.f);
+                (void)round_n_next; (void)round_bits_next; (void)mine2_next; (void)mine2b_next;
                 auto gather_round = [&]() {
                     if constexpr (PLANNED) {
-                        float* const idx = &s_tile[wv][0][0].x;
-                        int p = 0;
-                        round_bits_next = e0.w;
-                        auto take = [&](const plan_u32x4 ent) {
-                            const uint32_t m_lo = uint32_t(__builtin_amdgcn_readfirstlane(int(ent.y)));
-                            const uint32_t m_hi = uint32_t(__builtin_amdgcn_readfirstlane(int(ent.z)));
-                            const unsigned long long m = (unsigned long long)m_lo | ((unsigned long long)m_hi << 32);
-                            const int n_e = __builtin_popcountll(m);
-                            if (p + n_e > 64) return false;
-                            if (__builtin_amdgcn_inverse_ballot_w64(m))
-                                idx[p + int(__builtin_amdgcn_mbcnt_hi(m_hi, __builtin_amdgcn_mbcnt_lo(m_lo, 0u)))] =
-                                    __uint_as_float((uint32_t(__builtin_amdgcn_readfirstlane(int(ent.x))) << 6) + uint32_t(lane));
-                            p += n_e;
-                            ++plan_i;
-                            return (uint32_t(__builtin_amdgcn_readfirstlane(int(ent.w))) & 4u) == 0u && plan_i < plan_n;
-                        };
-                        while (take(e0) && take(e1) && take(e2) && take(e3)) {
-                            e0 = plan_at[plan_i]; e1 = plan_at[plan_i + 1]; e2 = plan_at[plan_i + 2]; e3 = plan_at[plan_i + 3];
-                        }
-                        e0 = plan_at[plan_i]; e1 = plan_at[plan_i + 1]; e2 = plan_at[plan_i + 2]; e3 = plan_at[plan_i + 3];
-                        round_n_next = p;
-                        const int pj = int(min(__float_as_uint(idx[lane]), uint32_t(r_hi - 1)));
+                        round_n_next = loop_n;
+                        round_bits_next = uint32_t(loop_bits);
+                        const int pj = int(min(plan_word, uint32_t(r_hi - 1)));
                         mine_next = a.A[pj];
                         if (NEED_B) mineb_next = a.B[pj];
                         if constexpr (WEIGHTED) {
 #pragma unroll
                             for (int c = 0; c < NW; ++c) mw_next[c] = a.weights[size_t(pj) * a.w_stride + c];
                         }
+                        if constexpr (FUSE) {
+                            if (loop_n > 64) {
+                                const int pj2 = int(min(plan_word2, uint32_t(r_hi - 1)));
+                                mine2_next = a.A[pj2];
+                                mine2b_next = a.B[pj2];
+                            }
+                        }
+                        plan_w += loop_n;
+                        form_loop();
                     }
                 };
                 if constexpr (PLANNED) gather_round();
@@ -799,8 +831,11 @@
                     const int round_n = round_n_next;
                     const uint32_t round_bits = round_bits_next;
                     (void)round_n; (void)round_bits;
+                    const float4 mine2 = mine2_next;
+                    const float2 mine2b = mine2b_next;
+                    (void)mine2; (void)mine2b;
                     if constexpr (PLANNED) {
-                        more = plan_i < plan_n;
+                        more = loop_n > 0;
                         if (more) gather_round();
                     } else if (more) {
                         cnext = cg + __builtin_ctzll(cmask);
@@ -879,6 +914,11 @@
                             if (NW > 1 && keep) tile4[66 + slot] = make_float4(sw[1], sw[2], sw[3], 0.f);
                         } else {
                         if (keep) tile4[slot] = make_float4(s1, s2, mineb.x, mineb.y);
+                        if constexpr (FUSE) {
+                            if (round_n > 64 && lane < round_n - 64)
+                                tile4[64 + lane] = make_float4(AX == 0 ? mine2.y : mine2.x, AX == 2 ? mine2.y : mine2.z,
+                                                               mine2b.x, mine2b.y);
+                        }
                         }
                     } else if (!COMPACT || keep) {
                         s_tile[wv][0][slot] = make_float2(mine.x, mine.y);
@@ -1120,7 +1160,7 @@
                 auto run_lean4 = [&](auto fat_tag) {
                     constexpr bool FAT = decltype(fat_tag)::value;
                     float4 c0, c1, c2;
-                    int left = __builtin_popcountll(todo);
+                    int left = FUSE ? round_n : __builtin_popcountll(todo);
                     const float4* t4 = tile4;
                     if constexpr (WEIGHTED && NW > 1) {
                         float4 x0, x1;
diff --git a/grace-devel_amd/csrc/trace_planned.hip b/grace-devel_amd/csrc/trace_planned.hip
--- a/grace-devel_amd/csrc/trace_planned.hip
+++ b/grace-devel_amd/csrc/trace_planned.hip
@@ -7,9 +7,10 @@
 namespace {
 
 struct PlanRef {
-    uint4* entries;
-    const int2* spans;
-    int* counts;
+    uint32_t* idx;
+    uint32_t* hdr;
+    const int4* spans;
+    int4* counts;
     PlanCtl* ctl;
     int force;
 };
@@ -30,6 +31,15 @@
     int cnt = 0;
     int round_n = 0, round_bits = 0;
     int t_surv = 0, t_rounds = 0, t_full = 0, t_cap = 0, t_flag = 0, t_max = 0;
+    int loop_n = 0, loop_bits = 0, t_loops = 0, t_lmax = 0;
+    auto round_closed = [&](const int n, const int bits) {
+        if (FUSED && loop_n > 0 && planned_fuses(loop_n, loop_bits, plan_header(n, bits))) {
+            loop_n += n;
+        } else {
+            if (loop_n > 0) { t_loops += 1; t_lmax = max(t_lmax, loop_n); }
+            loop_n = n; loop_bits = bits;
+        }
+    };
     bool failed = axis < 0 || covered < 0;
     if (!failed) {
         const AxisRay ar = axis_ray(axis, ray);
@@ -116,13 +126,16 @@
                         const bool close_flag = n > 0 && !close_cap && open_bits != bits;
                         const bool close = close_cap || close_flag;
                         if (pl.spans) {
-                            const int2 span = pl.spans[packet * SUM_CLASSES + cls];
-                            if (n < span.y) {
-                                if (lane == 0) {
-                                    if (close) pl.entries[size_t(span.x) + n - 1].w = uint32_t(open_bits) | PLAN_ROUND_END;
-                                    pl.entries[size_t(span.x) + n] =
-                                        make_uint4(uint32_t(c), uint32_t(rest), uint32_t(rest >> 32), uint32_t(bits));
-                                }
+                            const int4 span = pl.spans[packet * SUM_CLASSES + cls];
+                            const int surv_at = __builtin_amdgcn_readlane(t_surv, cls);
+                            const int closed = __builtin_amdgcn_readlane(t_rounds, cls);
+                            if (surv_at + n_surv <= span.z && closed + (close ? 1 : 0) < span.w) {
+                                if (close && lane == 0) pl.hdr[size_t(span.y) + closed] = plan_header(open_n, open_bits);
+                                if ((rest >> lane) & 1ull)
+                                    pl.idx[size_t(span.x) + surv_at
+                                           + int(__builtin_amdgcn_mbcnt_hi(uint32_t(rest >> 32),
+                                                                           __builtin_amdgcn_mbcnt_lo(uint32_t(rest), 0u)))] =
+                                        uint32_t(pbase + lane);
                             } else {
                                 failed = true;
                             }
@@ -132,6 +145,7 @@
                                 t_rounds += 1; t_full += open_n == 64 ? 1 : 0;
                                 t_cap += close_cap ? 1 : 0; t_flag += close_flag ? 1 : 0;
                                 t_max = max(t_max, open_n);
+                                round_closed(open_n, open_bits);
                                 round_n = 0;
                             }
                             round_n += n_surv; round_bits = bits;
@@ -147,31 +161,32 @@
         cnt = 0;
         if (lane == 0) { pl.ctl->unusable = 1u; pl.ctl->usable = 0u; }
     }
-    if (lane < SUM_CLASSES) pl.counts[packet * SUM_CLASSES + lane] = cnt;
+    if (lane < SUM_CLASSES && cnt > 0) {
+        if (pl.spans && !failed)
+            pl.hdr[size_t(pl.spans[packet * SUM_CLASSES + lane].y) + t_rounds] = plan_header(round_n, round_bits);
+        t_rounds += 1; t_full += round_n == 64 ? 1 : 0;
+        t_max = max(t_max, round_n);
+        round_closed(round_n, round_bits);
+        t_loops += 1; t_lmax = max(t_lmax, loop_n);
+    }
+    if (lane < SUM_CLASSES) pl.counts[packet * SUM_CLASSES + lane] = failed ? make_int4(0, 0, 0, 0) : make_int4(t_rounds, t_surv, cnt, 0);
     if (pl.spans && !failed) {
-        for (int cls = 0; cls < SUM_CLASSES; ++cls) {
-            const int n = __builtin_amdgcn_readlane(cnt, cls);
-            const int open_bits = __builtin_amdgcn_readlane(round_bits, cls);
-            if (n > 0 && lane == 0)
-                pl.entries[size_t(pl.spans[packet * SUM_CLASSES + cls].x) + n - 1].w = uint32_t(open_bits) | PLAN_ROUND_END;
-        }
-        if (lane < SUM_CLASSES && cnt > 0) {
-            t_rounds += 1; t_full += round_n == 64 ? 1 : 0;
-            t_max = max(t_max, round_n);
-        }
         if (lane >= SUM_CLASSES) cnt = 0;
-        int tally[6] = { cnt, t_surv, t_rounds, t_full, t_cap, t_flag };
+        int tally[7] = { cnt, t_surv, t_rounds, t_full, t_cap, t_flag, t_loops };
 #pragma unroll
         for (int off = 1; off < SUM_CLASSES; off <<= 1) {
 #pragma unroll
-            for (int k = 0; k < 6; ++k) tally[k] += __shfl_xor(tally[k], off);
+            for (int k = 0; k < 7; ++k) tally[k] += __shfl_xor(tally[k], off);
             t_max = max(t_max, __shfl_xor(t_max, off));
+            t_lmax = max(t_lmax, __shfl_xor(t_lmax, off));
         }
         if (lane == 0) {
 #pragma unroll
             for (int k = 0; k < 6; ++k)
                 if (tally[k]) atomicAdd(&pl.ctl->stats[k], (unsigned long long)tally[k]);
+            if (tally[6]) atomicAdd(&pl.ctl->loops, (unsigned long long)tally[6]);
             atomicMax(&pl.ctl->largest_round, uint32_t(t_max));
+            atomicMax(&pl.ctl->largest_loop, uint32_t(t_lmax));
         }
     }
 }
@@ -188,15 +203,15 @@
 
 grace_status plan_free_buffers(PacketPlan& pp)
 {
-    void* bufs[] = { pp.entries, pp.spans, pp.counts, pp.ctl };
+    void* bufs[] = { pp.idx, pp.hdr, pp.spans, pp.counts, pp.ctl };
     bool any = false;
     for (void* b : bufs) any = any || b;
     if (any) GRACE_TRY_HIP(hipDeviceSynchronize());
     for (void* b : bufs)
         if (b) GRACE_TRY_HIP(hipFree(b));
-    pp.entries = nullptr; pp.spans = nullptr; pp.counts = nullptr; pp.ctl = nullptr;
+    pp.idx = nullptr; pp.hdr = nullptr; pp.spans = nullptr; pp.counts = nullptr; pp.ctl = nullptr;
     pp.valid = false;
-    pp.n_lists = pp.n_entries = pp.recorded = 0;
+    pp.n_lists = pp.n_words = pp.n_hdrs = pp.recorded = 0;
     return GRACE_OK;
 }
 
@@ -227,36 +242,40 @@
         ptr = nullptr;
         return false;
     };
-    if (n_lists * (sizeof(int) + sizeof(int2)) > ts.plan_budget) return GRACE_OK;
-    if (!alloc(pp.counts, n_lists * sizeof(int)) || !alloc(pp.spans, n_lists * sizeof(int2))
+    if (n_lists * (sizeof(int4) + sizeof(int4)) > ts.plan_budget) return GRACE_OK;
+    if (!alloc(pp.counts, n_lists * sizeof(int4)) || !alloc(pp.spans, n_lists * sizeof(int4))
         || !alloc(pp.ctl, sizeof(PlanCtl)))
         return plan_free_buffers(pp);
     GRACE_TRY_HIP(hipMemsetAsync(pp.ctl, 0, sizeof(PlanCtl), stream));
-    GRACE_TRY(launch_record(key.fast, a, PlanRef{ nullptr, nullptr, pp.counts, pp.ctl, 1 }, stream));
-    std::vector<int> counts(n_lists);
+    GRACE_TRY(launch_record(key.fast, a, PlanRef{ nullptr, nullptr, nullptr, pp.counts, pp.ctl, 1 }, stream));
+    std::vector<int4> counts(n_lists);
     PlanCtl seen = {};
-    GRACE_TRY_HIP(hipMemcpyAsync(counts.data(), pp.counts, n_lists * sizeof(int), hipMemcpyDeviceToHost, stream));
+    GRACE_TRY_HIP(hipMemcpyAsync(counts.data(), pp.counts, n_lists * sizeof(int4), hipMemcpyDeviceToHost, stream));
     GRACE_TRY_HIP(hipMemcpyAsync(&seen, pp.ctl, sizeof(seen), hipMemcpyDeviceToHost, stream));
     GRACE_TRY_HIP(hipStreamSynchronize(stream));
     if (seen.unusable) return plan_free_buffers(pp);
-    std::vector<int2> spans(n_lists);
-    size_t total = 0, used = 0;
+    std::vector<int4> spans(n_lists);
+    size_t words = 0, hdrs = 0, used = 0;
     for (size_t l = 0; l < n_lists; ++l) {
-        const size_t room = size_t(counts[l]) + size_t(counts[l]) / 8 + 2;
-        spans[l] = make_int2(int(total), int(room));
-        total += room;
-        used += size_t(counts[l]);
-        if (total >= (size_t(1) << 31)) return plan_free_buffers(pp);
-    }
-    const size_t bytes = (total + 4) * sizeof(uint4) + n_lists * (sizeof(int) + sizeof(int2));
-    if (bytes > ts.plan_budget || !alloc(pp.entries, (total + 4) * sizeof(uint4))) return plan_free_buffers(pp);
-    GRACE_TRY_HIP(hipMemcpy(pp.spans, spans.data(), n_lists * sizeof(int2), hipMemcpyHostToDevice));
-    GRACE_TRY_HIP(hipMemsetAsync(pp.entries + total, 0, 4 * sizeof(uint4), stream));
-    pp.n_lists = n_lists; pp.n_entries = total; pp.recorded = used;
+        const size_t surv = size_t(counts[l].y), entries = size_t(counts[l].z);
+        const size_t room_s = surv + surv / 8 + 2, room_r = entries + entries / 8 + 2;
+        spans[l] = make_int4(int(words), int(hdrs), int(room_s), int(room_r));
+        words += room_s;
+        hdrs += room_r;
+        used += surv;
+        if (words >= (size_t(1) << 31) - PLAN_IDX_PAD) return plan_free_buffers(pp);
+    }
+    pp.n_lists = n_lists; pp.n_words = words; pp.n_hdrs = hdrs; pp.recorded = used;
+    if (pp.bytes() > ts.plan_budget || !alloc(pp.idx, (words + PLAN_IDX_PAD) * sizeof(uint32_t))
+        || !alloc(pp.hdr, (hdrs + PLAN_HDR_PAD) * sizeof(uint32_t)))
+        return plan_free_buffers(pp);
+    GRACE_TRY_HIP(hipMemcpy(pp.spans, spans.data(), n_lists * sizeof(int4), hipMemcpyHostToDevice));
+    GRACE_TRY_HIP(hipMemsetAsync(pp.idx + words, 0, PLAN_IDX_PAD * sizeof(uint32_t), stream));
+    GRACE_TRY_HIP(hipMemsetAsync(pp.hdr + hdrs, 0, PLAN_HDR_PAD * sizeof(uint32_t), stream));
     GRACE_TRY_HIP(hipMemsetD32Async(reinterpret_cast<hipDeviceptr_t>(&pp.ctl->usable), 1, 1, stream));
     GRACE_TRY_HIP(hipMemcpyAsync(&pp.ctl->sig[0], ts.scene.ctl->sig, 16, hipMemcpyDeviceToDevice, stream));
     GRACE_TRY_HIP(hipMemcpyAsync(&pp.ctl->sig[2], ts.rays.ctl->sig, 16, hipMemcpyDeviceToDevice, stream));
-    GRACE_TRY(launch_record(key.fast, a, PlanRef{ pp.entries, pp.spans, pp.counts, pp.ctl, 1 }, stream));
+    GRACE_TRY(launch_record(key.fast, a, PlanRef{ pp.idx, pp.hdr, pp.spans, pp.counts, pp.ctl, 1 }, stream));
     pp.valid = true;
     pp.dead = false;
     return GRACE_OK;
@@ -265,7 +284,7 @@
 grace_status plan_record(const TraceState& ts, const TraceArgs& a, hipStream_t stream)
 {
     const PacketPlan& pp = ts.plan;
-    return launch_record(pp.key.fast, a, PlanRef{ pp.entries, pp.spans, pp.counts, pp.ctl, 0 }, stream);
+    return launch_record(pp.key.fast, a, PlanRef{ pp.idx, pp.hdr, pp.spans, pp.counts, pp.ctl, 0 }, stream);
 }
 
 grace_status launch_planned(const int mode, const bool fast, const int grid, const TraceArgs& a, hipStream_t stream)
diff --git a/grace-devel_amd/csrc/trace_state.hpp b/grace-devel_amd/csrc/trace_state.hpp
--- a/grace-devel_amd/csrc/trace_state.hpp
+++ b/grace-devel_amd/csrc/trace_state.hpp
@@ -139,11 +139,12 @@
     int w_stride;
     int out_stride;
     const double* kernel_table;
-    const uint4* plan_entries;
-    const int2* plan_spans;
-    const int* plan_counts;
+    const uint32_t* plan_idx;
+    const int4* plan_spans;
+    const int4* plan_counts;
     const uint32_t* plan_usable;
     const int* plan_split_dev;
+    const uint32_t* plan_hdr;
 };
 
 
@@ -198,9 +199,17 @@
     uint32_t largest_round;
     unsigned long long sig[4];
     unsigned long long stats[6];
-};
-constexpr uint32_t PLAN_ROUND_END = 4u;
-constexpr int PLAN_FORMAT = 2;
+    unsigned long long loops;
+    uint32_t largest_loop, pad;
+};
+constexpr int PLAN_FORMAT = 3;
+__host__ __device__ inline uint32_t plan_header(const int n_surv, const int bits)
+{
+    return uint32_t(n_surv) | (uint32_t(bits) << 8);
+}
+__host__ __device__ inline int plan_header_count(const uint32_t h) { return int(h & 0xffu) < 64 ? int(h & 0xffu) : 64; }
+__host__ __device__ inline int plan_header_bits(const uint32_t h) { return int((h >> 8) & 3u); }
+constexpr size_t PLAN_IDX_PAD = 128, PLAN_HDR_PAD = 8;
 
 struct PlanKey {
     int format = PLAN_FORMAT;
@@ -220,12 +229,18 @@
     bool valid = false;
     bool dead = false;
     PlanKey key;
-    uint4* entries = nullptr;
-    int2* spans = nullptr;
-    int* counts = nullptr;
+    uint32_t* idx = nullptr;
+    uint32_t* hdr = nullptr;
+    int4* spans = nullptr;
+    int4* counts = nullptr;
     PlanCtl* ctl = nullptr;
-    size_t n_lists = 0, n_entries = 0;
+    size_t n_lists = 0, n_words = 0, n_hdrs = 0;
     size_t recorded = 0;
+    size_t bytes() const
+    {
+        return (n_words + PLAN_IDX_PAD + n_hdrs + PLAN_HDR_PAD) * sizeof(uint32_t)
+            + n_lists * (sizeof(int4) + sizeof(int4)) + sizeof(PlanCtl);
+    }
 };
 
 struct PlanGate {
@@ -237,6 +252,13 @@
 __host__ __device__ inline int planned_split(const int n_packets)
 {
     return n_packets <= 8192 ? SUM_CLASSES : SUM_CLASSES / 2;
+}
+
+constexpr int PLAN_LOOP_MAX = 128;
+__host__ __device__ inline bool planned_fuses(const int loop_n, const int loop_bits, const uint32_t next)
+{
+    return (loop_bits & 1) != 0 && plan_header_bits(next) == loop_bits
+        && loop_n + plan_header_count(next) <= PLAN_LOOP_MAX;
 }
 
 struct HitsCache {
@@ -278,6 +300,7 @@
     PacketPlan plan;
     const PlanCtl* last_plan_ctl = nullptr;
     hipStream_t last_plan_stream = nullptr;
+    bool last_plan_fuses = false;
 };
 
 grace_status trace_state(TraceState** out);
diff --git a/grace-devel_amd/grace_hip/__init__.py b/grace-devel_amd/grace_hip/__init__.py
--- a/grace-devel_amd/grace_hip/__init__.py
+++ b/grace-devel_amd/grace_hip/__init__.py
@@ -363,6 +363,12 @@
     v = (C.c_ulonglong * 7)()
     _check(_lib.grace_trace_plan_stats(v))
     return PlanStats(*[int(x) for x in v])
+
+
+def plan_loops():
+    v = (C.c_ulonglong * 2)()
+    _check(_lib.grace_trace_plan_loops(v))
+    return int(v[0]), int(v[1])
 
 
 def set_lattice_split(k):
diff --git a/include/grace_hip.h b/include/grace_hip.h
--- a/include/grace_hip.h
+++ b/include/grace_hip.h
@@ -241,6 +241,7 @@
 grace_status grace_trace_plan_bytes(size_t* h_bytes);
 grace_status grace_trace_last_plan_used(int* h_used);
 grace_status grace_trace_plan_stats(unsigned long long* h_stats );
+grace_status grace_trace_plan_loops(unsigned long long* h_loops );
 
 grace_status grace_trace_status(grace_stream stream);
 
```

New measurement: 596.3 (median of 6 runs). 3.6% higher.
